# deepspeedai/DeepSpeed

Hardware: AMD Instinct MI355X
Metric: tokens/sec Llama-3-8B ZeRO-3 (higher is better)
Workload: dtype bf16; 1 GPU; model=llama3-8b, global_batch=8, seq_len=4096, parallelism=zero3_dp1, grad_accum=2

## Files before the change

### deepspeed_amd/models/llama.py

```python
from dataclasses import dataclass, field

import torch
import torch.nn as nn
import torch.nn.functional as F

from ..ops.attention import flash_attention
from ..ops.functional import (apply_rope, build_rope_cache,
                              fused_cross_entropy, rms_norm, swiglu)


@dataclass
class LlamaConfig:
    hidden_size: int = 4096
    intermediate_size: int = 14336
    num_hidden_layers: int = 32
    num_attention_heads: int = 32
    num_key_value_heads: int = 8
    vocab_size: int = 128256
    max_position_embeddings: int = 8192
    rope_theta: float = 500000.0
    rms_norm_eps: float = 1e-5
    tie_word_embeddings: bool = False
    initializer_range: float = 0.02
    activation_checkpointing: bool = True
    attention_bias: bool = False

    @property
    def head_dim(self):
        return self.hidden_size // self.num_attention_heads


LLAMA_CONFIGS = {
    "llama3-8b": LlamaConfig(),
    "llama3-70b": LlamaConfig(hidden_size=8192, intermediate_size=28672,
                              num_hidden_layers=80, num_attention_heads=64,
                              num_key_value_heads=8),
    "llama-tiny": LlamaConfig(hidden_size=256, intermediate_size=688,
                              num_hidden_layers=4, num_attention_heads=8,
                              num_key_value_heads=4, vocab_size=2048,
                              max_position_embeddings=512,
                              activation_checkpointing=False),
    "llama-small": LlamaConfig(hidden_size=1024, intermediate_size=2816,
                               num_hidden_layers=8, num_attention_heads=16,
                               num_key_value_heads=4, vocab_size=32000,
                               max_position_embeddings=4096),
    "qwen2-7b": LlamaConfig(hidden_size=3584, intermediate_size=18944,
                            num_hidden_layers=28, num_attention_heads=28,
                            num_key_value_heads=4, vocab_size=152064,
                            max_position_embeddings=32768,
                            rope_theta=1e6, rms_norm_eps=1e-6,
                            attention_bias=True),
    "qwen2-tiny": LlamaConfig(hidden_size=256, intermediate_size=688,
                              num_hidden_layers=4, num_attention_heads=8,
                              num_key_value_heads=4, vocab_size=2048,
                              max_position_embeddings=512,
                              attention_bias=True,
                              tie_word_embeddings=True,
                              activation_checkpointing=False),
}


class LlamaRMSNorm(nn.Module):
    def __init__(self, hidden_size, eps=1e-5):
        super().__init__()
        self.weight = nn.Parameter(torch.ones(hidden_size))
        self.eps = eps

    def forward(self, x):
        return rms_norm(x, self.weight, self.eps)


class LlamaAttention(nn.Module):
    def __init__(self, cfg: LlamaConfig):
        super().__init__()
        self.cfg = cfg
        h, d = cfg.hidden_size, cfg.head_dim
        ab = getattr(cfg, "attention_bias", False)
        self.q_proj = nn.Linear(h, cfg.num_attention_heads * d, bias=ab)
        self.k_proj = nn.Linear(h, cfg.num_key_value_heads * d, bias=ab)
        self.v_proj = nn.Linear(h, cfg.num_key_value_heads * d, bias=ab)
        self.o_proj = nn.Linear(cfg.num_attention_heads * d, h, bias=False)
        self.sp_group = None
        self._dist_attn = None

    def forward(self, x, cos, sin, kv_cache=None):
        B, S, _ = x.shape
        d = self.cfg.head_dim
        q = self.q_proj(x).view(B, S, -1, d)
        k = self.k_proj(x).view(B, S, -1, d)
        v = self.v_proj(x).view(B, S, -1, d)
        if getattr(kv_cache, "fuses_rope", False):
            q, k, v = kv_cache.rope_append(q, k, v)
        else:
            q = apply_rope(q, cos, sin)
            k = apply_rope(k, cos, sin)
            if kv_cache is not None:
                k, v = kv_cache.update(k, v)
        if kv_cache is not None:
            rg = getattr(kv_cache, "ragged", None)
            fb = getattr(kv_cache, "fused", None)
            if getattr(kv_cache, "fp8", False) and (fb is not None
                                                    or rg is not None):
                from ..ops import functional as Fops
                if fb is not None:
                    o = Fops.ragged_prefill_attention_fp8(
                        q[0], kv_cache.k, kv_cache.v, kv_cache.k_scale,
                        kv_cache.v_scale, fb)
                else:
                    o = Fops.ragged_decode_attention_fp8(q, *rg)
            elif fb is not None:
                from ..ops.functional import ragged_prefill_attention
                o = ragged_prefill_attention(q[0], kv_cache.k, kv_cache.v,
                                             fb)
            elif rg is not None:
                from ..ops.loader import get_ext
                o = get_ext(required=True).ragged_decode(
                    q.contiguous(), *rg)
            else:
                mask = getattr(kv_cache, "attn_mask", None)
                causal = S > 1
                o = flash_attention(q, k, v,
                                    causal=causal and mask is None,
                                    attn_mask=mask)
        elif self._dist_attn is not None:
            o = self._dist_attn(q, k, v, causal=True)
        else:
            o = flash_attention(q, k, v, causal=True)
        return self.o_proj(o.reshape(B, S, -1))


class StaticKVCache:

    def __init__(self, batch, max_seq, n_kv, head_dim, dtype, device):
        self.k = torch.zeros(batch, max_seq, n_kv, head_dim, dtype=dtype,
                             device=device)
        self.v = torch.zeros_like(self.k)
        self.max_seq = max_seq

    def prefill(self, k, v):
        S = k.shape[1]
        self.k[:, :S] = k
        self.v[:, :S] = v

    def decode_update(self, k1, v1, pos_idx):
        self.k.index_copy_(1, pos_idx, k1)
        self.v.index_copy_(1, pos_idx, v1)
        return self.k, self.v


def _linear_1t(lin, x):
    if x.is_cuda and x.dtype == torch.bfloat16:
        from ..ops.loader import get_ext
        ext = get_ext(required=False)
        if ext is not None:
            B = x.numel() // x.shape[-1]
            y = ext.gemv_bf16(lin.weight, x.reshape(B, -1).contiguous())
            return y.reshape(*x.shape[:-1], lin.weight.shape[0])
    return lin(x)


def llama_decode_step(model, ids, caches, pos_idx, attn_mask, cos_t, sin_t):
    core = model.model
    x = core.embed_tokens(ids)
    cos = cos_t.index_select(0, pos_idx)
    sin = sin_t.index_select(0, pos_idx)
    for layer, cache in zip(core.layers, caches):
        attn = layer.self_attn
        h = layer.input_layernorm(x)
        B = h.shape[0]
        d = attn.cfg.head_dim
        q = _linear_1t(attn.q_proj, h).view(B, 1, -1, d)
        k = _linear_1t(attn.k_proj, h).view(B, 1, -1, d)
        v = _linear_1t(attn.v_proj, h).view(B, 1, -1, d)
        q = apply_rope(q, cos, sin)
        k = apply_rope(k, cos, sin)
        kf, vf = cache.decode_update(k, v, pos_idx)
        o = F.scaled_dot_product_attention(
            q.transpose(1, 2), kf.transpose(1, 2), vf.transpose(1, 2),
            attn_mask=attn_mask,
            enable_gqa=(kf.shape[2] != q.shape[2]))
        x = x + _linear_1t(attn.o_proj, o.transpose(1, 2).reshape(B, 1, -1))
        h2 = layer.post_attention_layernorm(x)
        mlp = layer.mlp
        x = x + _linear_1t(mlp.down_proj,
                           swiglu(_linear_1t(mlp.gate_proj, h2),
                                  _linear_1t(mlp.up_proj, h2)))
    x = core.norm(x)
    return _linear_1t(model.lm_head, x)


def enable_ulysses(model, sp_group=None):
    from ..sequence.layer import DistributedAttention
    for mod in model.modules():
        if isinstance(mod, LlamaAttention):
            mod.sp_group = sp_group
            mod._dist_attn = DistributedAttention(flash_attention, sp_group)
    return model


class LlamaMLP(nn.Module):
    def __init__(self, cfg: LlamaConfig):
        super().__init__()
        self.gate_proj = nn.Linear(cfg.hidden_size, cfg.intermediate_size,
                                   bias=False)
        self.up_proj = nn.Linear(cfg.hidden_size, cfg.intermediate_size,
                                 bias=False)
        self.down_proj = nn.Linear(cfg.intermediate_size, cfg.hidden_size,
                                   bias=False)

    def forward(self, x):
        return self.down_proj(swiglu(self.gate_proj(x), self.up_proj(x)))


class LlamaDecoderLayer(nn.Module):
    def __init__(self, cfg: LlamaConfig):
        super().__init__()
        self.input_layernorm = LlamaRMSNorm(cfg.hidden_size, cfg.rms_norm_eps)
        self.self_attn = LlamaAttention(cfg)
        self.post_attention_layernorm = LlamaRMSNorm(cfg.hidden_size,
                                                     cfg.rms_norm_eps)
        self.mlp = LlamaMLP(cfg)

    def forward(self, x, cos, sin, kv_cache=None):
        x = x + self.self_attn(self.input_layernorm(x), cos, sin,
                               kv_cache=kv_cache)
        x = x + self.mlp(self.post_attention_layernorm(x))
        return x


class LlamaModel(nn.Module):
    def __init__(self, cfg: LlamaConfig):
        super().__init__()
        self.cfg = cfg
        self.embed_tokens = nn.Embedding(cfg.vocab_size, cfg.hidden_size)
        self.layers = nn.ModuleList(
            [LlamaDecoderLayer(cfg) for _ in range(cfg.num_hidden_layers)])
        self.norm = LlamaRMSNorm(cfg.hidden_size, cfg.rms_norm_eps)
        cos, sin = build_rope_cache(cfg.max_position_embeddings, cfg.head_dim,
                                    cfg.rope_theta)
        dev = self.embed_tokens.weight.device
        if dev.type != "meta":
            cos, sin = cos.to(dev), sin.to(dev)
        self.register_buffer("rope_cos", cos, persistent=False)
        self.register_buffer("rope_sin", sin, persistent=False)

    def forward(self, input_ids, seq_offset=0, kv_caches=None,
                positions=None):
        x = self.embed_tokens(input_ids)
        S = input_ids.shape[1]
        if positions is not None:
            cos = self.rope_cos[positions]
            sin = self.rope_sin[positions]
        else:
            cos = self.rope_cos[seq_offset:seq_offset + S]
            sin = self.rope_sin[seq_offset:seq_offset + S]
        for i, layer in enumerate(self.layers):
            if self.cfg.activation_checkpointing and self.training:
                x = torch.utils.checkpoint.checkpoint(
                    layer, x, cos, sin, use_reentrant=False)
            else:
                x = layer(x, cos, sin,
                          kv_cache=kv_caches[i] if kv_caches else None)
        return self.norm(x)


class LlamaForCausalLM(nn.Module):
    def __init__(self, cfg: LlamaConfig):
        super().__init__()
        self.cfg = cfg
        self.model = LlamaModel(cfg)
        self.lm_head = nn.Linear(cfg.hidden_size, cfg.vocab_size, bias=False)
        if cfg.tie_word_embeddings:
            self.lm_head.weight = self.model.embed_tokens.weight
        self.apply(self._init_weights)

    def _init_weights(self, module):
        std = self.cfg.initializer_range
        if isinstance(module, nn.Linear):
            module.weight.data.normal_(0.0, std)
            if module.bias is not None:
                module.bias.data.zero_()
        elif isinstance(module, nn.Embedding):
            module.weight.data.normal_(0.0, std)

    def forward(self, input_ids, labels=None, seq_offset=0, kv_caches=None,
                positions=None, logits_rows=None):
        h = self.model(input_ids, seq_offset=seq_offset, kv_caches=kv_caches,
                       positions=positions)
        if logits_rows is not None:
            h = h[:, logits_rows]
        logits = self.lm_head(h)
        if labels is None:
            return logits
        return fused_cross_entropy(logits[:, :-1, :], labels[:, 1:])
```

### deepspeed_amd/ops/attention.py

```python
import math
import os

import torch
import torch.nn.functional as F

from .loader import get_ext


class _FlashAttnFn(torch.autograd.Function):
    @staticmethod
    def forward(ctx, q, k, v, causal, scale, kvmask=None):
        ext = get_ext(required=True)
        out, lse = ext.flash_attn_fwd(q, k, v, causal, scale, kvmask)
        ctx.save_for_backward(q, k, v, out, lse,
                              kvmask if kvmask is not None
                              else torch.empty(0))
        ctx.causal = causal
        ctx.scale = scale
        return out

    @staticmethod
    def backward(ctx, dout):
        q, k, v, out, lse, kvmask = ctx.saved_tensors
        if kvmask.numel() == 0:
            kvmask = None
        causal, scale = ctx.causal, ctx.scale
        B, S, Hq, D = q.shape
        Hk = k.shape[2]
        G = Hq // Hk

        if os.environ.get("DSAMD_FLASH_BWD", "1") == "1":
            ext = get_ext(required=True)
            dq, dk, dv = ext.flash_attn_bwd(
                q, k, v, dout.contiguous(), out, lse, causal, scale, kvmask)
            return dq, dk, dv, None, None, None

        qh = q.permute(0, 2, 1, 3)
        kh = k.permute(0, 2, 1, 3)
        vh = v.permute(0, 2, 1, 3)
        doh = dout.permute(0, 2, 1, 3).contiguous()
        oh = out.permute(0, 2, 1, 3)

        drow = (doh.float() * oh.float()).sum(-1)

        qg = qh.reshape(B, Hk, G, S, D)
        dog = doh.reshape(B, Hk, G, S, D)
        lse_g = lse.reshape(B, Hk, G, S)
        drow_g = drow.reshape(B, Hk, G, S)

        dq = torch.zeros(B, Hk, G, S, D, device=q.device, dtype=torch.float32)
        dk = torch.empty_like(kh, dtype=torch.float32)
        dv = torch.empty_like(vh, dtype=torch.float32)

        CHUNK = 1024
        rows = torch.arange(S, device=q.device)
        for c0 in range(0, S, CHUNK):
            c1 = min(c0 + CHUNK, S)
            kc = kh[:, :, c0:c1]
            vc = vh[:, :, c0:c1]
            s_c = torch.einsum("bhgsd,bhcd->bhgsc", qg, kc).float() * scale
            if kvmask is not None:
                s_c = s_c + kvmask[:, c0:c1].view(B, 1, 1, 1, c1 - c0)
            p = torch.exp(s_c - lse_g.unsqueeze(-1))
            if causal:
                mask = rows.view(1, 1, 1, S, 1) >= (c0 + torch.arange(
                    c1 - c0, device=q.device)).view(1, 1, 1, 1, -1)
                p = p * mask
            p16 = p.to(q.dtype)
            dv[:, :, c0:c1] = torch.einsum("bhgsc,bhgsd->bhcd", p16,
                                           dog).float()
            dp = torch.einsum("bhgsd,bhcd->bhgsc", dog, vc).float()
            ds = (p * (dp - drow_g.unsqueeze(-1)) * scale).to(q.dtype)
            dq += torch.einsum("bhgsc,bhcd->bhgsd", ds, kc).float()
            dk[:, :, c0:c1] = torch.einsum("bhgsc,bhgsd->bhcd", ds,
                                           qg).float()

        dq_out = dq.reshape(B, Hq, S, D).permute(0, 2, 1, 3).to(q.dtype)
        dk_out = dk.permute(0, 2, 1, 3).to(k.dtype)
        dv_out = dv.permute(0, 2, 1, 3).to(v.dtype)
        return dq_out.contiguous(), dk_out.contiguous(), \
            dv_out.contiguous(), None, None, None


_USE_HIP_FLASH = os.environ.get("DSAMD_FLASH", "1") == "1"


def _as_kv_padding_mask(attn_mask, B, Sk):
    if attn_mask is None or attn_mask.dtype == torch.bool:
        return None
    m = attn_mask
    if m.dim() == 4 and m.shape[1] == 1 and m.shape[2] == 1:
        m = m[:, 0, 0]
    elif m.dim() == 3 and m.shape[1] == 1:
        m = m[:, 0]
    elif m.dim() != 2:
        return None
    if m.shape[-1] != Sk:
        return None
    if m.shape[0] == 1 and B > 1:
        m = m.expand(B, Sk)
    if m.shape[0] != B:
        return None
    return m.contiguous().float()


def flash_attention(q, k, v, causal=True, attn_mask=None):
    scale = 1.0 / math.sqrt(q.shape[-1])
    hip_ok = _USE_HIP_FLASH and q.is_cuda and q.dtype == torch.bfloat16 \
        and q.shape[-1] in (64, 128) and q.shape[1] == k.shape[1]
    if attn_mask is not None:
        kvm = _as_kv_padding_mask(attn_mask, q.shape[0], k.shape[1]) \
            if hip_ok else None
        if kvm is not None:
            return _FlashAttnFn.apply(q.contiguous(), k.contiguous(),
                                      v.contiguous(), causal, scale, kvm)
        out = F.scaled_dot_product_attention(
            q.transpose(1, 2), k.transpose(1, 2), v.transpose(1, 2),
            attn_mask=attn_mask, is_causal=False,
            enable_gqa=(k.shape[2] != q.shape[2]))
        return out.transpose(1, 2)
    if hip_ok:
        return _FlashAttnFn.apply(q.contiguous(), k.contiguous(),
                                  v.contiguous(), causal, scale)
    qt = q.transpose(1, 2)
    kt = k.transpose(1, 2)
    vt = v.transpose(1, 2)
    out = F.scaled_dot_product_attention(
        qt, kt, vt, is_causal=causal,
        enable_gqa=(k.shape[2] != q.shape[2]))
    return out.transpose(1, 2)
```

### deepspeed_amd/ops/csrc/attention_bwd.hip

```cpp
#include <torch/extension.h>

#include "common.h"

using bf16x8_t = __attribute__((ext_vector_type(8))) short;
using f32x4_t = __attribute__((ext_vector_type(4))) float;
using u32x4_t = __attribute__((ext_vector_type(4))) unsigned int;
using u32x2_t = __attribute__((ext_vector_type(2))) unsigned int;

#define MFMA_BF16_16x16x32 __builtin_amdgcn_mfma_f32_16x16x32_bf16

namespace bwd {

constexpr int BR = 128;
constexpr int WR = 32;
constexpr int KTW1 = 1;
constexpr int TS = 32;
constexpr int PT = 64;

DEV_INLINE unsigned int cvtpk2(float lo, float hi) {
  unsigned short a = __builtin_bit_cast(unsigned short, (__bf16)lo);
  unsigned short b = __builtin_bit_cast(unsigned short, (__bf16)hi);
  return (unsigned int)a | ((unsigned int)b << 16);
}

template <int DH>
__launch_bounds__(256)
__global__ void bwd_preprocess(
    const short* __restrict__ q, const short* __restrict__ k,
    const short* __restrict__ dout, const short* __restrict__ out,
    const float* __restrict__ lse,
    short* __restrict__ qT, short* __restrict__ doT, short* __restrict__ kT,
    float* __restrict__ drowP, float* __restrict__ lseP,
    int B, int S, int Sp, int Hq, int Hk) {
  constexpr int PPR = DH / 8;
  __shared__ unsigned int t[PT][DH / 2 + 1];

  const int z = blockIdx.z;
  const int H = (z == 2) ? Hk : Hq;
  const int bh = blockIdx.y;
  if (bh >= B * H) return;
  const int b = bh / H;
  const int h = bh % H;
  const int s0 = blockIdx.x * PT;
  const short* src = (z == 0) ? q : (z == 1) ? dout : k;
  short* dst = (z == 0) ? qT : (z == 1) ? doT : kT;

  for (int i = threadIdx.x; i < PT * PPR; i += 256) {
    const int row = i / PPR;
    const int c = i % PPR;
    const int s = s0 + row;
    const long long off = (((long long)b * S + s) * H + h) * DH + c * 8;
    u32x4_t x = {0u, 0u, 0u, 0u};
    if (s < S) x = *reinterpret_cast<const u32x4_t*>(src + off);
#pragma unroll
    for (int w = 0; w < 4; ++w) t[row][c * 4 + w] = x[w];
    if (z == 1) {
      u32x4_t o = {0u, 0u, 0u, 0u};
      if (s < S) o = *reinterpret_cast<const u32x4_t*>(out + off);
      float acc = 0.f;
#pragma unroll
      for (int w = 0; w < 4; ++w)
        acc += bf2f((short)(x[w] & 0xffff)) * bf2f((short)(o[w] & 0xffff)) +
               bf2f((short)(x[w] >> 16)) * bf2f((short)(o[w] >> 16));
#pragma unroll
      for (int m = PPR / 2; m > 0; m >>= 1) acc += __shfl_xor(acc, m, WAVE);
      if (c == 0) drowP[((long long)b * Hq + h) * Sp + s] = acc;
    } else if (z == 0 && c == 0) {
      float l = 0.f;
      if (s < S) {
        l = lse[((long long)b * Hq + h) * S + s];
        if (l == -INFINITY) l = INFINITY;
      }
      lseP[((long long)b * Hq + h) * Sp + s] = l;
    }
  }
  __syncthreads();
  for (int i = threadIdx.x; i < DH * (PT / 8); i += 256) {
    const int d = i / (PT / 8);
    const int pc = i % (PT / 8);
    const int sh = (d & 1) * 16;
    unsigned int e[8];
#pragma unroll
    for (int j = 0; j < 8; ++j) e[j] = (t[pc * 8 + j][d >> 1] >> sh) & 0xffffu;
    u32x4_t y = {e[0] | (e[1] << 16), e[2] | (e[3] << 16),
                 e[4] | (e[5] << 16), e[6] | (e[7] << 16)};
    *reinterpret_cast<u32x4_t*>(dst + (((long long)b * H + h) * DH + d) * Sp +
                                s0 + pc * 8) = y;
  }
}

template <int DH>
DEV_INLINE int rmswz(int row, int byte_off) {
  return row * (DH * 2) + (byte_off ^ ((row & 7) << 4));
}

DEV_INLINE void lds_dma16(const short* src, char* lds_wave_base) {
  __builtin_amdgcn_global_load_lds(
      reinterpret_cast<const unsigned int*>(src),
      reinterpret_cast<unsigned int*>(lds_wave_base), 16, 0, 0);
}

template <int DH>
DEV_INLINE void issue_rm(const short* base, long long rs, int r0, int S,
                         char* img, int sseg, int lane) {
  const int linear = sseg * 1024 + lane * 16;
  const int row = linear / (DH * 2);
  const int colbyte = linear % (DH * 2);
  const int src_col = colbyte ^ ((row & 7) << 4);
  const int grow = r0 + row;
  const int srow = grow < S ? grow : S - 1;
  lds_dma16(base + (long long)srow * rs + (src_col >> 1), img + sseg * 1024);
}

template <int DH>
DEV_INLINE void issue_tr(const short* baseT, int Sp, int c0, char* img,
                         int sseg, int lane) {
  const int linear = sseg * 1024 + lane * 16;
  const int d = linear >> 6;
  const int g = ((linear >> 4) & 3) ^ ((d >> 2) & 3);
  lds_dma16(baseT + (long long)d * Sp + c0 + g * 8, img + sseg * 1024);
}

template <int DH>
DEV_INLINE bf16x8_t read_rm(const char* img, int row, int ks, int l4) {
  return *reinterpret_cast<const bf16x8_t*>(
      img + rmswz<DH>(row, (l4 * 8 + 32 * ks) * 2));
}

DEV_INLINE bf16x8_t read_tr(const char* img, int d, int l4) {
  const int sw = (d >> 2) & 3;
  const char* rowp = img + d * 64 + (l4 & 1) * 8;
  u32x2_t lo = *reinterpret_cast<const u32x2_t*>(rowp + (((l4 >> 1) ^ sw) << 4));
  u32x2_t hi =
      *reinterpret_cast<const u32x2_t*>(rowp + (((2 + (l4 >> 1)) ^ sw) << 4));
  u32x4_t w = {lo[0], lo[1], hi[0], hi[1]};
  return __builtin_bit_cast(bf16x8_t, w);
}

DEV_INLINE bf16x8_t pack_pair(const f32x4_t& a, const f32x4_t& b) {
  u32x4_t w = {cvtpk2(a[0], a[1]), cvtpk2(a[2], a[3]), cvtpk2(b[0], b[1]),
               cvtpk2(b[2], b[3])};
  return __builtin_bit_cast(bf16x8_t, w);
}

DEV_INLINE void store4(short* p, const f32x4_t& a) {
  u32x2_t w = {cvtpk2(a[0], a[1]), cvtpk2(a[2], a[3])};
  *reinterpret_cast<u32x2_t*>(p) = w;
}

template <int DH, int KTW>
__launch_bounds__(512 / KTW, 1)
__global__ void flash_bwd_dkv_kernel(
    const short* __restrict__ q,
    const short* __restrict__ k,
    const short* __restrict__ v,
    const short* __restrict__ dout,
    const short* __restrict__ qT,
    const short* __restrict__ doT,
    const float* __restrict__ lseP,
    const float* __restrict__ drowP,
    const float* __restrict__ kvmask,
    short* __restrict__ dk,
    short* __restrict__ dv,
    int B, int S, int Sp, int Hq, int Hk, float scale, int causal) {
  constexpr int NKS = DH / 32;
  constexpr int NDT = DH / 16;
  constexpr int IMG = TS * DH * 2;
  constexpr int SPI = DH / 16;
  constexpr int NW = 8 / KTW;
  constexpr int WRK = 16 * KTW;
  constexpr int LD_OFF = 4 * IMG;
  constexpr int BUF = LD_OFF + 256;
  __shared__ __attribute__((aligned(16))) char smem[2 * BUF];

  const int lane = threadIdx.x & 63;
  const int wave = threadIdx.x >> 6;
  const int l15 = lane & 15;
  const int l4 = lane >> 4;

  const int bh = blockIdx.y;
  const int b = bh / Hk;
  const int hk = bh % Hk;
  const int G = Hq / Hk;
  const int kv_base = blockIdx.x * BR;
  const int wk = kv_base + wave * WRK;

  const long long qrs = (long long)Hq * DH;
  const long long kvrs = (long long)Hk * DH;
  const short* kp = k + ((long long)b * S) * kvrs + hk * DH;
  const short* vp = v + ((long long)b * S) * kvrs + hk * DH;

  bf16x8_t kfrag[KTW][NKS], vfrag[KTW][NKS];
  float maskv[KTW];
#pragma unroll
  for (int kt = 0; kt < KTW; ++kt) {
    const int krow = wk + 16 * kt + l15;
    const int srow = krow < S ? krow : S - 1;
    const short* ks = kp + (long long)srow * kvrs;
    const short* vs = vp + (long long)srow * kvrs;
#pragma unroll
    for (int ks_i = 0; ks_i < NKS; ++ks_i) {
      kfrag[kt][ks_i] =
          *reinterpret_cast<const bf16x8_t*>(ks + ks_i * 32 + l4 * 8);
      vfrag[kt][ks_i] =
          *reinterpret_cast<const bf16x8_t*>(vs + ks_i * 32 + l4 * 8);
    }
    maskv[kt] = (kvmask && krow < S) ? kvmask[(long long)b * S + krow] : 0.f;
  }

  f32x4_t dk_acc[NDT][KTW], dv_acc[NDT][KTW];
#pragma unroll
  for (int dt = 0; dt < NDT; ++dt)
#pragma unroll
    for (int kt = 0; kt < KTW; ++kt) {
      dk_acc[dt][kt] = f32x4_t{0.f, 0.f, 0.f, 0.f};
      dv_acc[dt][kt] = f32x4_t{0.f, 0.f, 0.f, 0.f};
    }

  const int q_start = causal ? kv_base : 0;
  const int nq = (S - q_start + TS - 1) / TS;
  const int total = G * nq;

  auto issue = [&](int g, int qb, int bufi) {
    const int h = hk * G + g;
    char* buf = smem + bufi * BUF;
    const short* qp = q + ((long long)b * S) * qrs + h * DH;
    const short* dop = dout + ((long long)b * S) * qrs + h * DH;
    const long long toff = ((long long)b * Hq + h) * DH * Sp;
    const long long roff = ((long long)b * Hq + h) * Sp;
#pragma unroll
    for (int sseg = wave; sseg < SPI; sseg += NW) {
      issue_rm<DH>(qp, qrs, qb, S, buf, sseg, lane);
      issue_rm<DH>(dop, qrs, qb, S, buf + IMG, sseg, lane);
      issue_tr<DH>(qT + toff, Sp, qb, buf + 2 * IMG, sseg, lane);
      issue_tr<DH>(doT + toff, Sp, qb, buf + 3 * IMG, sseg, lane);
    }
    if (wave == 0) {
      const float* s = (lane < 32 ? lseP : drowP) + roff + qb + (lane & 31);
      __builtin_amdgcn_global_load_lds(
          reinterpret_cast<const unsigned int*>(s),
          reinterpret_cast<unsigned int*>(buf + LD_OFF), 4, 0, 0);
    }
  };

  int g_nx = 0, qb_nx = q_start;
  issue(g_nx, qb_nx, 0);
  for (int it = 0; it < total; ++it) {
    const int qb = qb_nx;
    asm volatile("s_waitcnt vmcnt(0)" ::: "memory");
    __syncthreads();
    qb_nx += TS;
    if (qb_nx >= S) {
      qb_nx = q_start;
      ++g_nx;
    }
    if (it + 1 < total) issue(g_nx, qb_nx, (it + 1) & 1);

    if (wk >= S || (causal && qb + TS - 1 < wk)) continue;
    const bool interior = !kvmask && qb + TS <= S && wk + WRK <= S &&
                          (!causal || qb >= wk + WRK - 1);
    const char* buf = smem + (it & 1) * BUF;
    const float* ld = reinterpret_cast<const float*>(buf + LD_OFF);

    f32x4_t s_acc[2][KTW], dp_acc[2][KTW], lrow[2];
#pragma unroll
    for (int qt = 0; qt < 2; ++qt) {
      lrow[qt] = *reinterpret_cast<const f32x4_t*>(ld + 16 * qt + 4 * l4);
      f32x4_t dr = *reinterpret_cast<const f32x4_t*>(ld + 32 + 16 * qt + 4 * l4);
#pragma unroll
      for (int kt = 0; kt < KTW; ++kt) {
        s_acc[qt][kt] = f32x4_t{0.f, 0.f, 0.f, 0.f};
        dp_acc[qt][kt] = -dr;
      }
    }
    __builtin_amdgcn_s_setprio(1);
#pragma unroll
    for (int qt = 0; qt < 2; ++qt)
#pragma unroll
      for (int ks_i = 0; ks_i < NKS; ++ks_i) {
        bf16x8_t aq = read_rm<DH>(buf, l15 + 16 * qt, ks_i, l4);
        bf16x8_t ad = read_rm<DH>(buf + IMG, l15 + 16 * qt, ks_i, l4);
#pragma unroll
        for (int kt = 0; kt < KTW; ++kt) {
          s_acc[qt][kt] = MFMA_BF16_16x16x32(aq, kfrag[kt][ks_i],
                                             s_acc[qt][kt], 0, 0, 0);
          dp_acc[qt][kt] = MFMA_BF16_16x16x32(ad, vfrag[kt][ks_i],
                                              dp_acc[qt][kt], 0, 0, 0);
        }
      }
    __builtin_amdgcn_s_setprio(0);

    if (interior) {
#pragma unroll
      for (int qt = 0; qt < 2; ++qt)
#pragma unroll
        for (int kt = 0; kt < KTW; ++kt)
#pragma unroll
          for (int r = 0; r < 4; ++r) {
            float p = __expf(s_acc[qt][kt][r] * scale - lrow[qt][r]);
            s_acc[qt][kt][r] = p;
            dp_acc[qt][kt][r] = p * dp_acc[qt][kt][r] * scale;
          }
    } else {
#pragma unroll
      for (int qt = 0; qt < 2; ++qt)
#pragma unroll
        for (int kt = 0; kt < KTW; ++kt) {
          const int gkv = wk + 16 * kt + l15;
#pragma unroll
          for (int r = 0; r < 4; ++r) {
            const int gq = qb + 16 * qt + 4 * l4 + r;
            const bool valid = gq < S && gkv < S && (!causal || gq >= gkv);
            float sval = s_acc[qt][kt][r] * scale + maskv[kt];
            float p = valid ? __expf(sval - lrow[qt][r]) : 0.f;
            s_acc[qt][kt][r] = p;
            dp_acc[qt][kt][r] = p * dp_acc[qt][kt][r] * scale;
          }
        }
    }
    bf16x8_t pb[KTW], dsb[KTW];
#pragma unroll
    for (int kt = 0; kt < KTW; ++kt) {
      pb[kt] = pack_pair(s_acc[0][kt], s_acc[1][kt]);
      dsb[kt] = pack_pair(dp_acc[0][kt], dp_acc[1][kt]);
    }

    __builtin_amdgcn_s_setprio(1);
#pragma unroll
    for (int dt = 0; dt < NDT; ++dt) {
      bf16x8_t aqt = read_tr(buf + 2 * IMG, l15 + 16 * dt, l4);
      bf16x8_t adt = read_tr(buf + 3 * IMG, l15 + 16 * dt, l4);
#pragma unroll
      for (int kt = 0; kt < KTW; ++kt) {
        dv_acc[dt][kt] =
            MFMA_BF16_16x16x32(adt, pb[kt], dv_acc[dt][kt], 0, 0, 0);
        dk_acc[dt][kt] =
            MFMA_BF16_16x16x32(aqt, dsb[kt], dk_acc[dt][kt], 0, 0, 0);
      }
    }
    __builtin_amdgcn_s_setprio(0);
  }

#pragma unroll
  for (int kt = 0; kt < KTW; ++kt) {
    const int gkv = wk + 16 * kt + l15;
    if (gkv >= S) continue;
    short* dkr = dk + ((long long)b * S + gkv) * kvrs + hk * DH + 4 * l4;
    short* dvr = dv + ((long long)b * S + gkv) * kvrs + hk * DH + 4 * l4;
#pragma unroll
    for (int dt = 0; dt < NDT; ++dt) {
      store4(dkr + 16 * dt, dk_acc[dt][kt]);
      store4(dvr + 16 * dt, dv_acc[dt][kt]);
    }
  }
}

template <int DH>
__launch_bounds__(256, 2)
__global__ void flash_bwd_dq_kernel(
    const short* __restrict__ q, const short* __restrict__ k,
    const short* __restrict__ v, const short* __restrict__ dout,
    const short* __restrict__ kT,
    const float* __restrict__ lseP,
    const float* __restrict__ drowP,
    const float* __restrict__ kvmask,
    short* __restrict__ dq,
    int B, int S, int Sp, int Hq, int Hk, float scale, int causal) {
  constexpr int NKS = DH / 32;
  constexpr int NDT = DH / 16;
  constexpr int IMG = TS * DH * 2;
  constexpr int SPI = DH / 16;
  constexpr int IPI = SPI / 4;
  constexpr int BUF = 3 * IMG;
  __shared__ __attribute__((aligned(16))) char smem[2 * BUF];

  const int lane = threadIdx.x & 63;
  const int wave = threadIdx.x >> 6;
  const int l15 = lane & 15;
  const int l4 = lane >> 4;

  const int qtile = gridDim.x - 1 - blockIdx.x;
  const int bh = blockIdx.y;
  const int b = bh / Hq;
  const int h = bh % Hq;
  const int hk = h / (Hq / Hk);
  const int qbase = qtile * BR;
  const int wq = qbase + wave * WR;

  const long long qrs = (long long)Hq * DH;
  const long long kvrs = (long long)Hk * DH;
  const short* qp = q + ((long long)b * S) * qrs + h * DH;
  const short* dop = dout + ((long long)b * S) * qrs + h * DH;
  const short* kp = k + ((long long)b * S) * kvrs + hk * DH;
  const short* vp = v + ((long long)b * S) * kvrs + hk * DH;
  const short* ktp = kT + ((long long)b * Hk + hk) * DH * Sp;
  const float* mp = kvmask ? kvmask + (long long)b * S : nullptr;

  bf16x8_t qfrag[2][NKS], dofrag[2][NKS];
  float lse_l[2], dr_l[2];
#pragma unroll
  for (int qt = 0; qt < 2; ++qt) {
    const int qrow = wq + 16 * qt + l15;
    const int srow = qrow < S ? qrow : S - 1;
    const short* qs = qp + (long long)srow * qrs;
    const short* ds = dop + (long long)srow * qrs;
#pragma unroll
    for (int ks_i = 0; ks_i < NKS; ++ks_i) {
      qfrag[qt][ks_i] =
          *reinterpret_cast<const bf16x8_t*>(qs + ks_i * 32 + l4 * 8);
      dofrag[qt][ks_i] =
          *reinterpret_cast<const bf16x8_t*>(ds + ks_i * 32 + l4 * 8);
    }
    lse_l[qt] = lseP[((long long)b * Hq + h) * Sp + qrow];
    dr_l[qt] = drowP[((long long)b * Hq + h) * Sp + qrow];
  }

  f32x4_t dq_acc[NDT][2];
#pragma unroll
  for (int dt = 0; dt < NDT; ++dt)
#pragma unroll
    for (int qt = 0; qt < 2; ++qt) dq_acc[dt][qt] = f32x4_t{0.f, 0.f, 0.f, 0.f};

  const int kv_end = causal ? min(S, qbase + BR) : S;
  const int n_tiles = (kv_end + TS - 1) / TS;

  auto issue = [&](int kvb, int bufi) {
    char* buf = smem + bufi * BUF;
#pragma unroll
    for (int i = 0; i < IPI; ++i) {
      const int sseg = i * 4 + wave;
      issue_rm<DH>(kp, kvrs, kvb, S, buf, sseg, lane);
      issue_rm<DH>(vp, kvrs, kvb, S, buf + IMG, sseg, lane);
      issue_tr<DH>(ktp, Sp, kvb, buf + 2 * IMG, sseg, lane);
    }
  };

  issue(0, 0);
  for (int t = 0; t < n_tiles; ++t) {
    const int kvb = t * TS;
    asm volatile("s_waitcnt vmcnt(0)" ::: "memory");
    __syncthreads();
    if (t + 1 < n_tiles) issue(kvb + TS, (t + 1) & 1);

    if (wq >= S || (causal && kvb > wq + WR - 1)) continue;
    const bool interior = !mp && kvb + TS <= S && wq + WR <= S &&
                          (!causal || kvb + TS - 1 <= wq);
    const char* buf = smem + (t & 1) * BUF;

    f32x4_t s_acc[2][2], dp_acc[2][2];
#pragma unroll
    for (int kt = 0; kt < 2; ++kt)
#pragma unroll
      for (int qt = 0; qt < 2; ++qt) {
        s_acc[kt][qt] = f32x4_t{0.f, 0.f, 0.f, 0.f};
        dp_acc[kt][qt] =
            f32x4_t{-dr_l[qt], -dr_l[qt], -dr_l[qt], -dr_l[qt]};
      }
    __builtin_amdgcn_s_setprio(1);
#pragma unroll
    for (int kt = 0; kt < 2; ++kt)
#pragma unroll
      for (int ks_i = 0; ks_i < NKS; ++ks_i) {
        bf16x8_t ak = read_rm<DH>(buf, l15 + 16 * kt, ks_i, l4);
        bf16x8_t av = read_rm<DH>(buf + IMG, l15 + 16 * kt, ks_i, l4);
#pragma unroll
        for (int qt = 0; qt < 2; ++qt) {
          s_acc[kt][qt] = MFMA_BF16_16x16x32(ak, qfrag[qt][ks_i],
                                             s_acc[kt][qt], 0, 0, 0);
          dp_acc[kt][qt] = MFMA_BF16_16x16x32(av, dofrag[qt][ks_i],
                                              dp_acc[kt][qt], 0, 0, 0);
        }
      }
    __builtin_amdgcn_s_setprio(0);

    if (interior) {
#pragma unroll
      for (int kt = 0; kt < 2; ++kt)
#pragma unroll
        for (int qt = 0; qt < 2; ++qt)
#pragma unroll
          for (int r = 0; r < 4; ++r) {
            float p = __expf(s_acc[kt][qt][r] * scale - lse_l[qt]);
            dp_acc[kt][qt][r] = p * dp_acc[kt][qt][r] * scale;
          }
    } else {
#pragma unroll
      for (int kt = 0; kt < 2; ++kt)
#pragma unroll
        for (int r = 0; r < 4; ++r) {
          const int gkv = kvb + 16 * kt + 4 * l4 + r;
          const float mv = (mp && gkv < S) ? mp[gkv] : 0.f;
#pragma unroll
          for (int qt = 0; qt < 2; ++qt) {
            const int gq = wq + 16 * qt + l15;
            const bool valid = gq < S && gkv < S && (!causal || gkv <= gq);
            float sval = s_acc[kt][qt][r] * scale + mv;
            float p = valid ? __expf(sval - lse_l[qt]) : 0.f;
            dp_acc[kt][qt][r] = p * dp_acc[kt][qt][r] * scale;
          }
        }
    }
    bf16x8_t dsb[2];
#pragma unroll
    for (int qt = 0; qt < 2; ++qt)
      dsb[qt] = pack_pair(dp_acc[0][qt], dp_acc[1][qt]);

    __builtin_amdgcn_s_setprio(1);
#pragma unroll
    for (int dt = 0; dt < NDT; ++dt) {
      bf16x8_t akt = read_tr(buf + 2 * IMG, l15 + 16 * dt, l4);
#pragma unroll
      for (int qt = 0; qt < 2; ++qt)
        dq_acc[dt][qt] =
            MFMA_BF16_16x16x32(akt, dsb[qt], dq_acc[dt][qt], 0, 0, 0);
    }
    __builtin_amdgcn_s_setprio(0);
  }

#pragma unroll
  for (int qt = 0; qt < 2; ++qt) {
    const int gq = wq + 16 * qt + l15;
    if (gq >= S) continue;
    short* dqr = dq + ((long long)b * S + gq) * qrs + h * DH + 4 * l4;
#pragma unroll
    for (int dt = 0; dt < NDT; ++dt) store4(dqr + 16 * dt, dq_acc[dt][qt]);
  }
}

}

template <int DH>
static void launch_bwd(at::Tensor& q, at::Tensor& k, at::Tensor& v,
                       at::Tensor& dout, at::Tensor& out, at::Tensor& lse,
                       at::Tensor& dq, at::Tensor& dk, at::Tensor& dv,
                       const float* mp, int B, int S, int Hq, int Hk,
                       float scale, int causal) {
  auto stream = c10::hip::getCurrentHIPStream();
  const int Sp = (S + bwd::BR - 1) / bwd::BR * bwd::BR;
  auto qT = at::empty({B, Hq, DH, Sp}, q.options());
  auto doT = at::empty({B, Hq, DH, Sp}, q.options());
  auto kT = at::empty({B, Hk, DH, Sp}, q.options());
  auto drow = at::empty({B, Hq, Sp}, q.options().dtype(at::kFloat));
  auto lseP = at::empty({B, Hq, Sp}, q.options().dtype(at::kFloat));
  auto sp = [](const at::Tensor& t) {
    return reinterpret_cast<const short*>(t.data_ptr());
  };
  auto spm = [](at::Tensor& t) {
    return reinterpret_cast<short*>(t.data_ptr());
  };
  dim3 grid0(Sp / bwd::PT, B * Hq, 3);
  hipLaunchKernelGGL(bwd::bwd_preprocess<DH>, grid0, dim3(256), 0,
                     stream.stream(), sp(q), sp(k), sp(dout), sp(out),
                     lse.data_ptr<float>(), spm(qT), spm(doT), spm(kT),
                     drow.data_ptr<float>(), lseP.data_ptr<float>(), B, S,
                     Sp, Hq, Hk);
  HIP_CHECK_KERNEL();
  dim3 grid1(Sp / bwd::BR, B * Hk);
  hipLaunchKernelGGL((bwd::flash_bwd_dkv_kernel<DH, bwd::KTW1>), grid1,
                     dim3(512 / bwd::KTW1), 0, stream.stream(), sp(q), sp(k),
                     sp(v), sp(dout), sp(qT), sp(doT), lseP.data_ptr<float>(),
                     drow.data_ptr<float>(), mp, spm(dk), spm(dv), B, S, Sp,
                     Hq, Hk, scale, causal);
  HIP_CHECK_KERNEL();
  dim3 grid2(Sp / bwd::BR, B * Hq);
  hipLaunchKernelGGL(bwd::flash_bwd_dq_kernel<DH>, grid2, dim3(256), 0,
                     stream.stream(), sp(q), sp(k), sp(v), sp(dout), sp(kT),
                     lseP.data_ptr<float>(), drow.data_ptr<float>(), mp,
                     spm(dq), B, S, Sp, Hq, Hk, scale, causal);
  HIP_CHECK_KERNEL();
}

void flash_check_qkv(const at::Tensor& q, const at::Tensor& k,
                     const at::Tensor& v, const char* who);
const float* flash_check_kvmask(const c10::optional<at::Tensor>& kvmask,
                                const at::Tensor& q);

std::vector<at::Tensor> flash_attn_bwd(at::Tensor q, at::Tensor k,
                                       at::Tensor v, at::Tensor dout,
                                       at::Tensor out, at::Tensor lse,
                                       bool causal, double scale,
                                       c10::optional<at::Tensor> kvmask) {
  flash_check_qkv(q, k, v, "flash_attn_bwd");
  CHECK_ARG(dout, at::kBFloat16);
  CHECK_ARG(out, at::kBFloat16);
  CHECK_ARG(lse, at::kFloat);
  CHECK_ON(dout, q);
  CHECK_ON(out, q);
  CHECK_ON(lse, q);
  TORCH_CHECK(dout.sizes() == q.sizes() && out.sizes() == q.sizes(),
              "flash_attn_bwd: dout and out must have q's shape");
  int B = q.size(0), S = q.size(1), Hq = q.size(2), D = q.size(3);
  int Hk = k.size(2);
  TORCH_CHECK(lse.dim() == 3 && lse.size(0) == B && lse.size(1) == Hq &&
                  lse.size(2) == S,
              "flash_attn_bwd: lse must be [B,Hq,S]");
  const float* mp = flash_check_kvmask(kvmask, q);
  const float fscale =
      scale == 0.0 ? 1.0f / std::sqrt((float)D) : (float)scale;
  auto dq = at::empty_like(q);
  auto dk = at::empty_like(k);
  auto dv = at::empty_like(v);
  if (D == 128)
    launch_bwd<128>(q, k, v, dout, out, lse, dq, dk, dv, mp, B, S, Hq, Hk,
                    fscale, causal ? 1 : 0);
  else
    launch_bwd<64>(q, k, v, dout, out, lse, dq, dk, dv, mp, B, S, Hq, Hk,
                   fscale, causal ? 1 : 0);
  return {dq, dk, dv};
}
```

### deepspeed_amd/ops/csrc/bindings.cpp

```cpp
#include <torch/extension.h>

void multi_tensor_adam(std::vector<at::Tensor> params,
                       std::vector<at::Tensor> grads,
                       std::vector<at::Tensor> exp_avgs,
                       std::vector<at::Tensor> exp_avg_sqs, double lr,
                       double beta1, double beta2, double eps, long step,
                       long adamw_mode, long bias_correction,
                       double weight_decay, std::vector<at::Tensor> out16,
                       double grad_scale);
void accum_bf16_to_f32(at::Tensor dst, at::Tensor src, double scale);
at::Tensor l2norm_sq(std::vector<at::Tensor> tensors);
at::Tensor fp8_amax(at::Tensor x);
at::Tensor ragged_decode(at::Tensor q, at::Tensor kpool, at::Tensor vpool,
                         at::Tensor rows, at::Tensor lens, long chunk);
at::Tensor ragged_prefill(at::Tensor q, at::Tensor kpool, at::Tensor vpool,
                          at::Tensor desc, long max_qlen, long max_kvlen);
at::Tensor ragged_rope_append(at::Tensor q, at::Tensor k, at::Tensor v,
                              at::Tensor cos, at::Tensor sin,
                              at::Tensor tok_slot, at::Tensor tok_pos,
                              at::Tensor kpool, at::Tensor vpool,
                              c10::optional<at::Tensor> lens);
at::Tensor ragged_decode_fp8(at::Tensor q, at::Tensor kpool, at::Tensor vpool,
                             at::Tensor k_scale, at::Tensor v_scale,
                             at::Tensor rows, at::Tensor lens, long chunk);
at::Tensor ragged_prefill_fp8(at::Tensor q, at::Tensor kpool,
                              at::Tensor vpool, at::Tensor k_scale,
                              at::Tensor v_scale, at::Tensor desc,
                              long max_qlen, long max_kvlen);
at::Tensor ragged_rope_append_fp8(at::Tensor q, at::Tensor k, at::Tensor v,
                                  at::Tensor cos, at::Tensor sin,
                                  at::Tensor tok_slot, at::Tensor tok_pos,
                                  at::Tensor kpool, at::Tensor vpool,
                                  at::Tensor k_scale, at::Tensor v_scale,
                                  c10::optional<at::Tensor> lens);
at::Tensor fp8_cast(at::Tensor x, at::Tensor scale, bool e5m2);
std::vector<at::Tensor> fp8_cast_transpose(at::Tensor x, at::Tensor scale,
                                           bool e5m2);
std::vector<at::Tensor> flash_attn_fwd(at::Tensor q, at::Tensor k,
                                       at::Tensor v, bool causal,
                                       double scale,
                                       c10::optional<at::Tensor> kvmask);
std::vector<at::Tensor> flash_attn_bwd(at::Tensor q, at::Tensor k,
                                       at::Tensor v, at::Tensor dout,
                                       at::Tensor out, at::Tensor lse,
                                       bool causal, double scale,
                                       c10::optional<at::Tensor> kvmask);
void multi_tensor_adagrad(std::vector<at::Tensor> params,
                          std::vector<at::Tensor> grads,
                          std::vector<at::Tensor> sq_accums, double lr,
                          double eps, double weight_decay,
                          std::vector<at::Tensor> out16);
void multi_tensor_lamb(std::vector<at::Tensor> params,
                       std::vector<at::Tensor> grads,
                       std::vector<at::Tensor> updates,
                       std::vector<at::Tensor> exp_avgs,
                       std::vector<at::Tensor> exp_avg_sqs,
                       at::Tensor workspace, double lr, double beta1,
                       double beta2, double eps, long step,
                       long bias_correction, double weight_decay,
                       std::vector<at::Tensor> out16, double grad_scale);
void cpu_lion_step(at::Tensor p, at::Tensor g, at::Tensor m,
                   c10::optional<at::Tensor> out16, double lr, double beta1,
                   double beta2, double wd);
void cpu_adagrad_step(at::Tensor p, at::Tensor g, at::Tensor h,
                      c10::optional<at::Tensor> out16, double lr, double eps,
                      double wd);
void cpu_adam_step(at::Tensor p, at::Tensor g, at::Tensor m, at::Tensor v,
                   c10::optional<at::Tensor> out16, double lr, double beta1,
                   double beta2, double eps, long step, long adamw,
                   long bias_correction, double wd, double grad_scale);
void multi_tensor_lion(std::vector<at::Tensor> params,
                       std::vector<at::Tensor> grads,
                       std::vector<at::Tensor> exp_avgs, double lr,
                       double beta1, double beta2, double weight_decay,
                       std::vector<at::Tensor> out16);
std::vector<at::Tensor> rmsnorm_fwd(at::Tensor x, at::Tensor w, double eps);
std::vector<at::Tensor> rmsnorm_bwd(at::Tensor dy, at::Tensor x, at::Tensor w,
                                    at::Tensor rstd);
std::vector<at::Tensor> layernorm_fwd(at::Tensor x, at::Tensor w,
                                      c10::optional<at::Tensor> b, double eps);
std::vector<at::Tensor> layernorm_bwd(at::Tensor dy, at::Tensor x,
                                      at::Tensor w, at::Tensor mean,
                                      at::Tensor rstd);
void rope(at::Tensor dst, at::Tensor src, at::Tensor cos, at::Tensor sin,
          long pos0, bool backward);
void rope_inplace(at::Tensor t, at::Tensor cos, at::Tensor sin, long pos0,
                  bool backward);
at::Tensor swiglu_fwd(at::Tensor g, at::Tensor u);
std::vector<at::Tensor> swiglu_bwd(at::Tensor dy, at::Tensor g, at::Tensor u);
std::vector<at::Tensor> cross_entropy_fwd(at::Tensor logits,
                                          at::Tensor targets,
                                          long ignore_index);
at::Tensor cross_entropy_bwd(at::Tensor logits, at::Tensor targets,
                             at::Tensor lse, at::Tensor dloss,
                             long ignore_index);

void bind_aio(py::module_& m);
at::Tensor gemv_bf16(at::Tensor W, at::Tensor x);
at::Tensor spatial_bias_add(at::Tensor a, at::Tensor bias,
                            c10::optional<at::Tensor> other);
std::vector<at::Tensor> quantize_int8(at::Tensor x, long group_size);
at::Tensor dequantize_int8(at::Tensor q, at::Tensor scales, long group_size);
std::vector<at::Tensor> quantize_fp8(at::Tensor x, long group_size);
at::Tensor dequantize_fp8(at::Tensor q, at::Tensor scales, long group_size);
std::vector<at::Tensor> quantize_int4(at::Tensor x, long group);
at::Tensor dequantize_int4(at::Tensor q, at::Tensor scales, long group,
                           long numel);
std::vector<at::Tensor> quantize_fp_em(at::Tensor x, long qbits, long group);
at::Tensor dequantize_fp_em(at::Tensor q, at::Tensor scales, long qbits,
                            long group, std::vector<long> shape);

PYBIND11_MODULE(TORCH_EXTENSION_NAME, m) {
  bind_aio(m);
  m.def("multi_tensor_adam", &multi_tensor_adam, "fused AdamW (gfx950)",
        py::arg("params"), py::arg("grads"), py::arg("exp_avgs"),
        py::arg("exp_avg_sqs"), py::arg("lr"), py::arg("beta1"),
        py::arg("beta2"), py::arg("eps"), py::arg("step"),
        py::arg("adamw_mode"), py::arg("bias_correction"),
        py::arg("weight_decay"), py::arg("out16") = std::vector<at::Tensor>(),
        py::arg("grad_scale") = 1.0);
  m.def("accum_bf16_to_f32", &accum_bf16_to_f32, py::arg("dst"),
        py::arg("src"), py::arg("scale") = 1.0);
  m.def("l2norm_sq", &l2norm_sq);
  m.def("fp8_amax", &fp8_amax);
  m.def("ragged_decode", &ragged_decode, py::arg("q"), py::arg("kpool"),
        py::arg("vpool"), py::arg("rows"), py::arg("lens"),
        py::arg("chunk") = 512);
  m.def("ragged_prefill", &ragged_prefill, py::arg("q"), py::arg("kpool"),
        py::arg("vpool"), py::arg("desc"), py::arg("max_qlen"),
        py::arg("max_kvlen"));
  m.def("ragged_rope_append", &ragged_rope_append, py::arg("q"),
        py::arg("k"), py::arg("v"), py::arg("cos"), py::arg("sin"),
        py::arg("tok_slot"), py::arg("tok_pos"), py::arg("kpool"),
        py::arg("vpool"), py::arg("lens") = c10::nullopt);
  m.def("ragged_decode_fp8", &ragged_decode_fp8, py::arg("q"),
        py::arg("kpool"), py::arg("vpool"), py::arg("k_scale"),
        py::arg("v_scale"), py::arg("rows"), py::arg("lens"),
        py::arg("chunk") = 512);
  m.def("ragged_prefill_fp8", &ragged_prefill_fp8, py::arg("q"),
        py::arg("kpool"), py::arg("vpool"), py::arg("k_scale"),
        py::arg("v_scale"), py::arg("desc"), py::arg("max_qlen"),
        py::arg("max_kvlen"));
  m.def("ragged_rope_append_fp8", &ragged_rope_append_fp8, py::arg("q"),
        py::arg("k"), py::arg("v"), py::arg("cos"), py::arg("sin"),
        py::arg("tok_slot"), py::arg("tok_pos"), py::arg("kpool"),
        py::arg("vpool"), py::arg("k_scale"), py::arg("v_scale"),
        py::arg("lens") = c10::nullopt);
  m.def("fp8_cast", &fp8_cast, py::arg("x"), py::arg("scale"),
        py::arg("e5m2") = false);
  m.def("fp8_cast_transpose", &fp8_cast_transpose, py::arg("x"),
        py::arg("scale"), py::arg("e5m2") = false);
  m.def("gemv_bf16", &gemv_bf16);
  m.def("spatial_bias_add", &spatial_bias_add, py::arg("a"), py::arg("bias"),
        py::arg("other") = c10::nullopt);
  m.def("quantize_int8", &quantize_int8);
  m.def("dequantize_int8", &dequantize_int8);
  m.def("quantize_fp8", &quantize_fp8);
  m.def("dequantize_fp8", &dequantize_fp8);
  m.def("quantize_int4", &quantize_int4, py::arg("x"),
        py::arg("group") = 2048);
  m.def("dequantize_int4", &dequantize_int4, py::arg("q"),
        py::arg("scales"), py::arg("group"), py::arg("numel"));
  m.def("quantize_fp_em", &quantize_fp_em, py::arg("x"), py::arg("qbits"),
        py::arg("group") = 512);
  m.def("dequantize_fp_em", &dequantize_fp_em, py::arg("q"),
        py::arg("scales"), py::arg("qbits"), py::arg("group"),
        py::arg("shape"));
  m.def("flash_attn_fwd", &flash_attn_fwd, py::arg("q"), py::arg("k"),
        py::arg("v"), py::arg("causal") = true, py::arg("scale") = 0.0,
        py::arg("kvmask") = c10::nullopt);
  m.def("flash_attn_bwd", &flash_attn_bwd, py::arg("q"), py::arg("k"),
        py::arg("v"), py::arg("dout"), py::arg("out"), py::arg("lse"),
        py::arg("causal") = true, py::arg("scale") = 0.0,
        py::arg("kvmask") = c10::nullopt);
  m.def("multi_tensor_adagrad", &multi_tensor_adagrad, py::arg("params"),
        py::arg("grads"), py::arg("sq_accums"), py::arg("lr"),
        py::arg("eps") = 1e-8, py::arg("weight_decay") = 0.0,
        py::arg("out16") = std::vector<at::Tensor>{});
  m.def("multi_tensor_lamb", &multi_tensor_lamb, py::arg("params"),
        py::arg("grads"), py::arg("updates"), py::arg("exp_avgs"),
        py::arg("exp_avg_sqs"),
        py::arg("workspace"), py::arg("lr"), py::arg("beta1") = 0.9,
        py::arg("beta2") = 0.999, py::arg("eps") = 1e-6, py::arg("step") = 1,
        py::arg("bias_correction") = 1, py::arg("weight_decay") = 0.0,
        py::arg("out16") = std::vector<at::Tensor>{},
        py::arg("grad_scale") = 1.0);
  m.def("cpu_lion_step", &cpu_lion_step, py::arg("p"), py::arg("g"),
        py::arg("m"), py::arg("out16") = c10::nullopt, py::arg("lr") = 1e-4,
        py::arg("beta1") = 0.9, py::arg("beta2") = 0.99, py::arg("wd") = 0.0,
        py::call_guard<py::gil_scoped_release>());
  m.def("cpu_adagrad_step", &cpu_adagrad_step, py::arg("p"), py::arg("g"),
        py::arg("h"), py::arg("out16") = c10::nullopt, py::arg("lr") = 1e-2,
        py::arg("eps") = 1e-8, py::arg("wd") = 0.0,
        py::call_guard<py::gil_scoped_release>());
  m.def("cpu_adam_step", &cpu_adam_step, py::arg("p"), py::arg("g"),
        py::arg("m"), py::arg("v"), py::arg("out16") = c10::nullopt,
        py::arg("lr") = 1e-3, py::arg("beta1") = 0.9, py::arg("beta2") = 0.999,
        py::arg("eps") = 1e-8, py::arg("step") = 1, py::arg("adamw") = 1,
        py::arg("bias_correction") = 1, py::arg("wd") = 0.0,
        py::arg("grad_scale") = 1.0);
  m.def("multi_tensor_lion", &multi_tensor_lion, "fused Lion (gfx950)",
        py::arg("params"), py::arg("grads"), py::arg("exp_avgs"),
        py::arg("lr"), py::arg("beta1"), py::arg("beta2"),
        py::arg("weight_decay"), py::arg("out16") = std::vector<at::Tensor>());
  m.def("rmsnorm_fwd", &rmsnorm_fwd);
  m.def("rmsnorm_bwd", &rmsnorm_bwd);
  m.def("layernorm_fwd", &layernorm_fwd);
  m.def("layernorm_bwd", &layernorm_bwd);
  m.def("rope", &rope);
  m.def("rope_inplace", &rope_inplace);
  m.def("swiglu_fwd", &swiglu_fwd);
  m.def("swiglu_bwd", &swiglu_bwd);
  m.def("cross_entropy_fwd", &cross_entropy_fwd);
  m.def("cross_entropy_bwd", &cross_entropy_bwd);
}
```

### deepspeed_amd/ops/csrc/elementwise.hip

```cpp
#include <torch/extension.h>

#include "common.h"

__global__ void rope_kernel(short* __restrict__ dst,
                            const short* __restrict__ src,
                            const float* __restrict__ cs,
                            const float* __restrict__ sn,
                            long long total_vec, int S, int H, int D,
                            int pos0, int backward) {
  int half = D / 2;
  int half8 = half / 8;
  long long i0 = (long long)blockIdx.x * blockDim.x + threadIdx.x;
  long long stride = (long long)gridDim.x * blockDim.x;
  for (long long i = i0; i < total_vec; i += stride) {
    int d8 = (int)(i % half8);
    long long rem = i / half8;
    int h = (int)(rem % H);
    long long rem2 = rem / H;
    int s = (int)(rem2 % S);
    long long b = rem2 / S;
    long long base = ((b * S + s) * (long long)H + h) * D + d8 * 8;
    const float* crow = cs + (long long)(s + pos0) * half + d8 * 8;
    const float* srow = sn + (long long)(s + pos0) * half + d8 * 8;
    bf16x8 x1 = *reinterpret_cast<const bf16x8*>(src + base);
    bf16x8 x2 = *reinterpret_cast<const bf16x8*>(src + base + half);
    f32x4 c0 = *reinterpret_cast<const f32x4*>(crow);
    f32x4 c1 = *reinterpret_cast<const f32x4*>(crow + 4);
    f32x4 s0 = *reinterpret_cast<const f32x4*>(srow);
    f32x4 s1 = *reinterpret_cast<const f32x4*>(srow + 4);
    float sgn = backward ? -1.f : 1.f;
    bf16x8 o1, o2;
#pragma unroll
    for (int k = 0; k < 8; ++k) {
      float c = (k < 4 ? c0.v[k] : c1.v[k - 4]);
      float sv = (k < 4 ? s0.v[k] : s1.v[k - 4]) * sgn;
      float a = bf2f(x1.v[k]);
      float bb = bf2f(x2.v[k]);
      o1.v[k] = f2bf(a * c - bb * sv);
      o2.v[k] = f2bf(bb * c + a * sv);
    }
    *reinterpret_cast<bf16x8*>(dst + base) = o1;
    *reinterpret_cast<bf16x8*>(dst + base + half) = o2;
  }
}

__global__ void rope_kernel_scalar(short* __restrict__ dst,
                                   const short* __restrict__ src,
                                   const float* __restrict__ cs,
                                   const float* __restrict__ sn,
                                   long long total_pairs, int S, int H,
                                   int D, int pos0, int backward) {
  int half = D / 2;
  long long i0 = (long long)blockIdx.x * blockDim.x + threadIdx.x;
  long long stride = (long long)gridDim.x * blockDim.x;
  for (long long i = i0; i < total_pairs; i += stride) {
    int d = (int)(i % half);
    long long rem = i / half;
    int h = (int)(rem % H);
    long long rem2 = rem / H;
    int s = (int)(rem2 % S);
    long long b = rem2 / S;
    long long base = ((b * S + s) * (long long)H + h) * D;
    float c = cs[(long long)(s + pos0) * half + d];
    float sv = sn[(long long)(s + pos0) * half + d];
    if (backward) sv = -sv;
    float x1 = bf2f(src[base + d]);
    float x2 = bf2f(src[base + d + half]);
    dst[base + d] = f2bf(x1 * c - x2 * sv);
    dst[base + d + half] = f2bf(x2 * c + x1 * sv);
  }
}

void rope(at::Tensor dst, at::Tensor src, at::Tensor cos, at::Tensor sin,
          long pos0, bool backward) {
  CHECK_ARG(src, at::kBFloat16);
  CHECK_ARG(dst, at::kBFloat16);
  CHECK_LIKE(dst, src);
  TORCH_CHECK(src.dim() == 4, "rope expects [B,S,H,D]");
  int B = src.size(0), S = src.size(1), H = src.size(2), D = src.size(3);
  TORCH_CHECK(D % 2 == 0, "rope: D must be even");
  if (src.numel() == 0) return;
  TORCH_CHECK(cos.device() == src.device() && sin.device() == src.device() &&
                  dst.device() == src.device(),
              "rope: cos/sin/dst must be on the same device as src");
  TORCH_CHECK(cos.scalar_type() == at::kFloat && cos.is_contiguous() &&
                  sin.scalar_type() == at::kFloat && sin.is_contiguous(),
              "rope: cos/sin must be contiguous fp32");
  TORCH_CHECK(pos0 >= 0, "rope: pos0 must be >= 0");
  TORCH_CHECK((long long)(pos0 + S) * (D / 2) <= cos.numel() &&
                  (long long)(pos0 + S) * (D / 2) <= sin.numel(),
              "rope: cos/sin table shorter than [pos0 + S, D/2]");
  auto stream = c10::hip::getCurrentHIPStream();
  int block = 256;
  bool vec = (D / 2) % 8 == 0 && ptr_aligned(src.data_ptr(), 16) &&
             ptr_aligned(dst.data_ptr(), 16) &&
             ptr_aligned(cos.data_ptr(), 16) &&
             ptr_aligned(sin.data_ptr(), 16);
  if (vec) {
    long long total_vec = (long long)B * S * H * (D / 16);
    int grid = grid_for(total_vec, block);
    hipLaunchKernelGGL(rope_kernel, dim3(grid), dim3(block), 0,
                       stream.stream(),
                       reinterpret_cast<short*>(dst.data_ptr()),
                       reinterpret_cast<const short*>(src.data_ptr()),
                       cos.data_ptr<float>(), sin.data_ptr<float>(),
                       total_vec, S, H, D, (int)pos0, backward ? 1 : 0);
  } else {
    long long total_pairs = (long long)B * S * H * (D / 2);
    int grid = grid_for(total_pairs, block);
    hipLaunchKernelGGL(rope_kernel_scalar, dim3(grid), dim3(block), 0,
                       stream.stream(),
                       reinterpret_cast<short*>(dst.data_ptr()),
                       reinterpret_cast<const short*>(src.data_ptr()),
                       cos.data_ptr<float>(), sin.data_ptr<float>(),
                       total_pairs, S, H, D, (int)pos0, backward ? 1 : 0);
  }
  HIP_CHECK_KERNEL();
}

void rope_inplace(at::Tensor t, at::Tensor cos, at::Tensor sin, long pos0,
                  bool backward) {
  rope(t, t, cos, sin, pos0, backward);
}

__global__ void swiglu_fwd_kernel(const short* __restrict__ g,
                                  const short* __restrict__ u,
                                  short* __restrict__ y, long long n,
                                  int vec_ok) {
  long long i0 = (long long)blockIdx.x * blockDim.x + threadIdx.x;
  long long stride = (long long)gridDim.x * blockDim.x;
  long long n8 = vec_ok ? n / 8 : 0;
  for (long long i = i0; i < n8; i += stride) {
    bf16x8 gv = reinterpret_cast<const bf16x8*>(g)[i];
    bf16x8 uv = reinterpret_cast<const bf16x8*>(u)[i];
    bf16x8 o;
#pragma unroll
    for (int k = 0; k < 8; ++k) {
      float gf = bf2f(gv.v[k]);
      float s = gf / (1.f + __expf(-gf));
      o.v[k] = f2bf(s * bf2f(uv.v[k]));
    }
    reinterpret_cast<bf16x8*>(y)[i] = o;
  }
  for (long long i = n8 * 8 + i0; i < n; i += stride) {
    float gf = bf2f(g[i]);
    float s = gf / (1.f + __expf(-gf));
    y[i] = f2bf(s * bf2f(u[i]));
  }
}

__global__ void swiglu_bwd_kernel(const short* __restrict__ dy,
                                  const short* __restrict__ g,
                                  const short* __restrict__ u,
                                  short* __restrict__ dg,
                                  short* __restrict__ du, long long n,
                                  int vec_ok) {
  long long i0 = (long long)blockIdx.x * blockDim.x + threadIdx.x;
  long long stride = (long long)gridDim.x * blockDim.x;
  long long n8 = vec_ok ? n / 8 : 0;
  for (long long i = i0; i < n8; i += stride) {
    bf16x8 dv = reinterpret_cast<const bf16x8*>(dy)[i];
    bf16x8 gv = reinterpret_cast<const bf16x8*>(g)[i];
    bf16x8 uv = reinterpret_cast<const bf16x8*>(u)[i];
    bf16x8 og, ou;
#pragma unroll
    for (int k = 0; k < 8; ++k) {
      float gf = bf2f(gv.v[k]);
      float d = bf2f(dv.v[k]);
      float sig = 1.f / (1.f + __expf(-gf));
      float silu = gf * sig;
      og.v[k] = f2bf(d * bf2f(uv.v[k]) * (sig + silu * (1.f - sig)));
      ou.v[k] = f2bf(d * silu);
    }
    reinterpret_cast<bf16x8*>(dg)[i] = og;
    reinterpret_cast<bf16x8*>(du)[i] = ou;
  }
  for (long long i = n8 * 8 + i0; i < n; i += stride) {
    float gf = bf2f(g[i]);
    float d = bf2f(dy[i]);
    float sig = 1.f / (1.f + __expf(-gf));
    float silu = gf * sig;
    dg[i] = f2bf(d * bf2f(u[i]) * (sig + silu * (1.f - sig)));
    du[i] = f2bf(d * silu);
  }
}

at::Tensor swiglu_fwd(at::Tensor g, at::Tensor u) {
  CHECK_ARG(g, at::kBFloat16);
  CHECK_ARG(u, at::kBFloat16);
  CHECK_LIKE(u, g);
  auto y = at::empty_like(g);
  long long n = g.numel();
  if (n == 0) return y;
  int vec_ok = ptr_aligned(g.data_ptr(), 16) && ptr_aligned(u.data_ptr(), 16) &&
               ptr_aligned(y.data_ptr(), 16);
  auto stream = c10::hip::getCurrentHIPStream();
  int block = 256;
  int grid = grid_for(vec_ok ? n / 8 + 1 : n, block);
  hipLaunchKernelGGL(swiglu_fwd_kernel, dim3(grid), dim3(block), 0,
                     stream.stream(),
                     reinterpret_cast<const short*>(g.data_ptr()),
                     reinterpret_cast<const short*>(u.data_ptr()),
                     reinterpret_cast<short*>(y.data_ptr()), n, vec_ok);
  HIP_CHECK_KERNEL();
  return y;
}

std::vector<at::Tensor> swiglu_bwd(at::Tensor dy, at::Tensor g, at::Tensor u) {
  CHECK_ARG(g, at::kBFloat16);
  CHECK_ARG(u, at::kBFloat16);
  CHECK_ARG(dy, at::kBFloat16);
  CHECK_LIKE(u, g);
  CHECK_LIKE(dy, g);
  auto dg = at::empty_like(g);
  auto du = at::empty_like(u);
  long long n = g.numel();
  if (n == 0) return {dg, du};
  int vec_ok = ptr_aligned(dy.data_ptr(), 16) &&
               ptr_aligned(g.data_ptr(), 16) &&
               ptr_aligned(u.data_ptr(), 16) &&
               ptr_aligned(dg.data_ptr(), 16) &&
               ptr_aligned(du.data_ptr(), 16);
  auto stream = c10::hip::getCurrentHIPStream();
  int block = 256;
  int grid = grid_for(vec_ok ? n / 8 + 1 : n, block);
  hipLaunchKernelGGL(swiglu_bwd_kernel, dim3(grid), dim3(block), 0,
                     stream.stream(),
                     reinterpret_cast<const short*>(dy.data_ptr()),
                     reinterpret_cast<const short*>(g.data_ptr()),
                     reinterpret_cast<const short*>(u.data_ptr()),
                     reinterpret_cast<short*>(dg.data_ptr()),
                     reinterpret_cast<short*>(du.data_ptr()), n, vec_ok);
  HIP_CHECK_KERNEL();
  return {dg, du};
}
```

### deepspeed_amd/ops/csrc/misc.hip

```cpp
#include <torch/extension.h>

#include "common.h"

__global__ void accum_bf16_f32_kernel(float* __restrict__ dst,
                                      const short* __restrict__ src,
                                      long long n, float scale,
                                      int vec_ok) {
  long long i0 = (long long)blockIdx.x * blockDim.x + threadIdx.x;
  long long stride = (long long)gridDim.x * blockDim.x;
  long long n4 = vec_ok ? n / 4 : 0;
  for (long long i = i0; i < n4; i += stride) {
    uint2 sv = reinterpret_cast<const uint2*>(src)[i];
    const short* s = reinterpret_cast<const short*>(&sv);
    f32x4 d = reinterpret_cast<f32x4*>(dst)[i];
#pragma unroll
    for (int k = 0; k < 4; ++k) d.v[k] += bf2f(s[k]) * scale;
    reinterpret_cast<f32x4*>(dst)[i] = d;
  }
  for (long long i = n4 * 4 + i0; i < n; i += stride)
    dst[i] += bf2f(src[i]) * scale;
}

void accum_bf16_to_f32(at::Tensor dst, at::Tensor src, double scale) {
  CHECK_ARG(dst, at::kFloat);
  CHECK_ARG(src, at::kBFloat16);
  CHECK_LIKE(src, dst);
  long long n = dst.numel();
  if (n == 0) return;
  int vec_ok = ptr_aligned(dst.data_ptr(), 16) && ptr_aligned(src.data_ptr(), 8);
  auto stream = c10::hip::getCurrentHIPStream();
  int block = 256;
  int grid = grid_for(n / 4 + 1, block);
  hipLaunchKernelGGL(accum_bf16_f32_kernel, dim3(grid), dim3(block), 0,
                     stream.stream(), dst.data_ptr<float>(),
                     reinterpret_cast<const short*>(src.data_ptr()), n,
                     (float)scale, vec_ok);
  HIP_CHECK_KERNEL();
}

template <int BLOCK>
__global__ void l2norm_sq_kernel(const float* __restrict__ x, long long n,
                                 float* __restrict__ out ,
                                 int vec_ok) {
  __shared__ float lds[BLOCK / WAVE];
  long long i0 = (long long)blockIdx.x * blockDim.x + threadIdx.x;
  long long stride = (long long)gridDim.x * blockDim.x;
  float acc = 0.f;
  long long n4 = vec_ok ? n / 4 : 0;
  for (long long i = i0; i < n4; i += stride) {
    f32x4 v = reinterpret_cast<const f32x4*>(x)[i];
#pragma unroll
    for (int k = 0; k < 4; ++k) acc += v.v[k] * v.v[k];
  }
  for (long long i = n4 * 4 + i0; i < n; i += stride) acc += x[i] * x[i];
  acc = block_reduce_sum<BLOCK>(acc, lds);
  if (threadIdx.x == 0) atomicAdd(out, acc);
}

at::Tensor l2norm_sq(std::vector<at::Tensor> tensors) {
  TORCH_CHECK(!tensors.empty());
  for (auto& t : tensors) {
    CHECK_ARG(t, at::kFloat);
    CHECK_ON(t, tensors[0]);
  }
  auto out = at::zeros({1}, tensors[0].options().dtype(at::kFloat));
  auto stream = c10::hip::getCurrentHIPStream();
  constexpr int BLOCK = 256;
  for (auto& t : tensors) {
    long long n = t.numel();
    if (n == 0) continue;
    int vec_ok = ptr_aligned(t.data_ptr(), 16);
    int grid = grid_for(n / 4 + 1, BLOCK);
    hipLaunchKernelGGL(l2norm_sq_kernel<BLOCK>, dim3(grid), dim3(BLOCK), 0,
                       stream.stream(), t.data_ptr<float>(), n,
                       out.data_ptr<float>(), vec_ok);
    HIP_CHECK_KERNEL();
  }
  return out;
}
```

### deepspeed_amd/ops/csrc/norms.hip

```cpp
#include <torch/extension.h>

#include "common.h"

static inline int row_vec_ok(int H, std::initializer_list<const void*> ptrs) {
  if (H % 8 != 0) return 0;
  for (const void* p : ptrs)
    if (!ptr_aligned(p, 16)) return 0;
  return 1;
}

static inline void check_norm_args(const at::Tensor& x, const at::Tensor& w) {
  CHECK_ARG(x, at::kBFloat16);
  CHECK_ARG(w, at::kBFloat16);
  CHECK_ON(w, x);
  TORCH_CHECK(x.dim() >= 1 && x.size(-1) > 0 && w.numel() == x.size(-1),
              "weight must have x.size(-1) elements");
}

template <int BLOCK>
__global__ void rmsnorm_fwd_kernel(const short* __restrict__ x,
                                   const short* __restrict__ w,
                                   short* __restrict__ y,
                                   float* __restrict__ rstd_out, int H,
                                   float eps, int vec) {
  __shared__ float lds[BLOCK / WAVE];
  const long long row = blockIdx.x;
  const short* xr = x + row * (long long)H;
  short* yr = y + row * (long long)H;
  int H8 = vec ? H / 8 : 0;
  float ss = 0.f;
  for (int i = threadIdx.x; i < H8; i += BLOCK) {
    bf16x8 v = reinterpret_cast<const bf16x8*>(xr)[i];
#pragma unroll
    for (int k = 0; k < 8; ++k) {
      float f = bf2f(v.v[k]);
      ss += f * f;
    }
  }
  for (int i = H8 * 8 + threadIdx.x; i < H; i += BLOCK) {
    float f = bf2f(xr[i]);
    ss += f * f;
  }
  ss = block_reduce_sum<BLOCK>(ss, lds);
  float rstd = rsqrtf(ss / H + eps);
  if (threadIdx.x == 0 && rstd_out) rstd_out[row] = rstd;
  for (int i = threadIdx.x; i < H8; i += BLOCK) {
    bf16x8 v = reinterpret_cast<const bf16x8*>(xr)[i];
    bf16x8 wv = reinterpret_cast<const bf16x8*>(w)[i];
    bf16x8 o;
#pragma unroll
    for (int k = 0; k < 8; ++k)
      o.v[k] = f2bf(bf2f(v.v[k]) * rstd * bf2f(wv.v[k]));
    reinterpret_cast<bf16x8*>(yr)[i] = o;
  }
  for (int i = H8 * 8 + threadIdx.x; i < H; i += BLOCK)
    yr[i] = f2bf(bf2f(xr[i]) * rstd * bf2f(w[i]));
}

template <int BLOCK>
__global__ void rmsnorm_bwd_dx_kernel(const short* __restrict__ dy,
                                      const short* __restrict__ x,
                                      const short* __restrict__ w,
                                      const float* __restrict__ rstd,
                                      short* __restrict__ dx, int H,
                                      int vec) {
  __shared__ float lds[BLOCK / WAVE];
  const long long row = blockIdx.x;
  const short* dyr = dy + row * (long long)H;
  const short* xr = x + row * (long long)H;
  short* dxr = dx + row * (long long)H;
  float rs = rstd[row];
  int H8 = vec ? H / 8 : 0;
  float dot = 0.f;
  for (int i = threadIdx.x; i < H8; i += BLOCK) {
    bf16x8 dv = reinterpret_cast<const bf16x8*>(dyr)[i];
    bf16x8 xv = reinterpret_cast<const bf16x8*>(xr)[i];
    bf16x8 wv = reinterpret_cast<const bf16x8*>(w)[i];
#pragma unroll
    for (int k = 0; k < 8; ++k)
      dot += bf2f(dv.v[k]) * bf2f(wv.v[k]) * bf2f(xv.v[k]);
  }
  for (int i = H8 * 8 + threadIdx.x; i < H; i += BLOCK)
    dot += bf2f(dyr[i]) * bf2f(w[i]) * bf2f(xr[i]);
  dot = block_reduce_sum<BLOCK>(dot, lds);
  float c = dot * rs * rs / H;
  for (int i = threadIdx.x; i < H8; i += BLOCK) {
    bf16x8 dv = reinterpret_cast<const bf16x8*>(dyr)[i];
    bf16x8 xv = reinterpret_cast<const bf16x8*>(xr)[i];
    bf16x8 wv = reinterpret_cast<const bf16x8*>(w)[i];
    bf16x8 o;
#pragma unroll
    for (int k = 0; k < 8; ++k)
      o.v[k] = f2bf(rs * (bf2f(dv.v[k]) * bf2f(wv.v[k]) -
                          bf2f(xv.v[k]) * c));
    reinterpret_cast<bf16x8*>(dxr)[i] = o;
  }
  for (int i = H8 * 8 + threadIdx.x; i < H; i += BLOCK)
    dxr[i] = f2bf(rs * (bf2f(dyr[i]) * bf2f(w[i]) - bf2f(xr[i]) * c));
}

__global__ void rmsnorm_bwd_dw_kernel(const short* __restrict__ dy,
                                      const short* __restrict__ x,
                                      const float* __restrict__ rstd,
                                      float* __restrict__ dw, long long rows,
                                      int H) {
  int c = blockIdx.x * blockDim.x + threadIdx.x;
  if (c >= H) return;
  float acc = 0.f;
  for (long long r = blockIdx.y; r < rows; r += gridDim.y) {
    long long idx = r * H + c;
    acc += bf2f(dy[idx]) * bf2f(x[idx]) * rstd[r];
  }
  if (gridDim.y == 1)
    dw[c] = acc;
  else
    atomicAdd(dw + c, acc);
}

std::vector<at::Tensor> rmsnorm_fwd(at::Tensor x, at::Tensor w, double eps) {
  check_norm_args(x, w);
  int H = x.size(-1);
  long long rows = x.numel() / H;
  auto y = at::empty_like(x);
  auto rstd = at::empty({rows}, x.options().dtype(at::kFloat));
  if (rows == 0) return {y, rstd};
  auto stream = c10::hip::getCurrentHIPStream();
  constexpr int BLOCK = 256;
  int vec = row_vec_ok(H, {x.data_ptr(), w.data_ptr(), y.data_ptr()});
  hipLaunchKernelGGL(rmsnorm_fwd_kernel<BLOCK>, dim3(rows), dim3(BLOCK), 0,
                     stream.stream(),
                     reinterpret_cast<const short*>(x.data_ptr()),
                     reinterpret_cast<const short*>(w.data_ptr()),
                     reinterpret_cast<short*>(y.data_ptr()),
                     rstd.data_ptr<float>(), H, (float)eps, vec);
  HIP_CHECK_KERNEL();
  return {y, rstd};
}

std::vector<at::Tensor> rmsnorm_bwd(at::Tensor dy, at::Tensor x, at::Tensor w,
                                    at::Tensor rstd) {
  check_norm_args(x, w);
  CHECK_ARG(dy, at::kBFloat16);
  CHECK_LIKE(dy, x);
  CHECK_ARG(rstd, at::kFloat);
  CHECK_ON(rstd, x);
  int H = x.size(-1);
  long long rows = x.numel() / H;
  TORCH_CHECK(rstd.numel() == rows, "rstd must have one entry per row");
  auto dx = at::empty_like(x);
  auto dw = at::zeros({H}, x.options().dtype(at::kFloat));
  if (rows == 0) return {dx, dw};
  auto stream = c10::hip::getCurrentHIPStream();
  constexpr int BLOCK = 256;
  int vec = row_vec_ok(
      H, {dy.data_ptr(), x.data_ptr(), w.data_ptr(), dx.data_ptr()});
  hipLaunchKernelGGL(rmsnorm_bwd_dx_kernel<BLOCK>, dim3(rows), dim3(BLOCK), 0,
                     stream.stream(),
                     reinterpret_cast<const short*>(dy.data_ptr()),
                     reinterpret_cast<const short*>(x.data_ptr()),
                     reinterpret_cast<const short*>(w.data_ptr()),
                     rstd.data_ptr<float>(),
                     reinterpret_cast<short*>(dx.data_ptr()), H, vec);
  HIP_CHECK_KERNEL();
  int gy = rows > 4096 ? 64 : (rows > 512 ? 16 : 1);
  hipLaunchKernelGGL(rmsnorm_bwd_dw_kernel, dim3((H + 255) / 256, gy),
                     dim3(256), 0, stream.stream(),
                     reinterpret_cast<const short*>(dy.data_ptr()),
                     reinterpret_cast<const short*>(x.data_ptr()),
                     rstd.data_ptr<float>(), dw.data_ptr<float>(), rows, H);
  HIP_CHECK_KERNEL();
  return {dx, dw};
}

template <int BLOCK>
__global__ void layernorm_fwd_kernel(const short* __restrict__ x,
                                     const short* __restrict__ w,
                                     const short* __restrict__ b,
                                     short* __restrict__ y,
                                     float* __restrict__ mean_out,
                                     float* __restrict__ rstd_out, int H,
                                     float eps) {
  __shared__ float lds[BLOCK / WAVE];
  const long long row = blockIdx.x;
  const short* xr = x + row * (long long)H;
  short* yr = y + row * (long long)H;
  float s = 0.f;
  for (int i = threadIdx.x; i < H; i += BLOCK) s += bf2f(xr[i]);
  s = block_reduce_sum<BLOCK>(s, lds);
  float mean = s / H;
  float ss = 0.f;
  for (int i = threadIdx.x; i < H; i += BLOCK) {
    float d = bf2f(xr[i]) - mean;
    ss += d * d;
  }
  ss = block_reduce_sum<BLOCK>(ss, lds);
  float var = ss / H;
  float rstd = rsqrtf(var + eps);
  if (threadIdx.x == 0) {
    if (mean_out) mean_out[row] = mean;
    if (rstd_out) rstd_out[row] = rstd;
  }
  for (int i = threadIdx.x; i < H; i += BLOCK) {
    float xhat = (bf2f(xr[i]) - mean) * rstd;
    float o = xhat * bf2f(w[i]) + (b ? bf2f(b[i]) : 0.f);
    yr[i] = f2bf(o);
  }
}

template <int BLOCK>
__global__ void layernorm_bwd_dx_kernel(
    const short* __restrict__ dy, const short* __restrict__ x,
    const short* __restrict__ w, const float* __restrict__ mean,
    const float* __restrict__ rstd, short* __restrict__ dx, int H) {
  __shared__ float lds[BLOCK / WAVE];
  const long long row = blockIdx.x;
  const short* dyr = dy + row * (long long)H;
  const short* xr = x + row * (long long)H;
  short* dxr = dx + row * (long long)H;
  float mu = mean[row], rs = rstd[row];
  float c1 = 0.f, c2 = 0.f;
  for (int i = threadIdx.x; i < H; i += BLOCK) {
    float g = bf2f(dyr[i]) * bf2f(w[i]);
    float xhat = (bf2f(xr[i]) - mu) * rs;
    c1 += g;
    c2 += g * xhat;
  }
  c1 = block_reduce_sum<BLOCK>(c1, lds) / H;
  c2 = block_reduce_sum<BLOCK>(c2, lds) / H;
  for (int i = threadIdx.x; i < H; i += BLOCK) {
    float g = bf2f(dyr[i]) * bf2f(w[i]);
    float xhat = (bf2f(xr[i]) - mu) * rs;
    dxr[i] = f2bf((g - c1 - xhat * c2) * rs);
  }
}

__global__ void layernorm_bwd_dwdb_kernel(const short* __restrict__ dy,
                                          const short* __restrict__ x,
                                          const float* __restrict__ mean,
                                          const float* __restrict__ rstd,
                                          float* __restrict__ dw,
                                          float* __restrict__ db,
                                          long long rows, int H) {
  int c = blockIdx.x * blockDim.x + threadIdx.x;
  if (c >= H) return;
  float accw = 0.f, accb = 0.f;
  for (long long r = blockIdx.y; r < rows; r += gridDim.y) {
    long long idx = r * H + c;
    float d = bf2f(dy[idx]);
    accw += d * (bf2f(x[idx]) - mean[r]) * rstd[r];
    accb += d;
  }
  if (gridDim.y == 1) {
    dw[c] = accw;
    db[c] = accb;
  } else {
    atomicAdd(dw + c, accw);
    atomicAdd(db + c, accb);
  }
}

std::vector<at::Tensor> layernorm_fwd(at::Tensor x, at::Tensor w,
                                      c10::optional<at::Tensor> b,
                                      double eps) {
  check_norm_args(x, w);
  if (b.has_value()) {
    CHECK_ARG(*b, at::kBFloat16);
    CHECK_LIKE(*b, w);
  }
  int H = x.size(-1);
  long long rows = x.numel() / H;
  auto y = at::empty_like(x);
  auto mean = at::empty({rows}, x.options().dtype(at::kFloat));
  auto rstd = at::empty({rows}, x.options().dtype(at::kFloat));
  if (rows == 0) return {y, mean, rstd};
  auto stream = c10::hip::getCurrentHIPStream();
  constexpr int BLOCK = 256;
  hipLaunchKernelGGL(
      layernorm_fwd_kernel<BLOCK>, dim3(rows), dim3(BLOCK), 0,
      stream.stream(), reinterpret_cast<const short*>(x.data_ptr()),
      reinterpret_cast<const short*>(w.data_ptr()),
      b.has_value() ? reinterpret_cast<const short*>(b->data_ptr()) : nullptr,
      reinterpret_cast<short*>(y.data_ptr()), mean.data_ptr<float>(),
      rstd.data_ptr<float>(), H, (float)eps);
  HIP_CHECK_KERNEL();
  return {y, mean, rstd};
}

std::vector<at::Tensor> layernorm_bwd(at::Tensor dy, at::Tensor x,
                                      at::Tensor w, at::Tensor mean,
                                      at::Tensor rstd) {
  check_norm_args(x, w);
  CHECK_ARG(dy, at::kBFloat16);
  CHECK_LIKE(dy, x);
  CHECK_ARG(mean, at::kFloat);
  CHECK_ARG(rstd, at::kFloat);
  CHECK_ON(mean, x);
  CHECK_ON(rstd, x);
  int H = x.size(-1);
  long long rows = x.numel() / H;
  TORCH_CHECK(mean.numel() == rows && rstd.numel() == rows,
              "mean/rstd must have one entry per row");
  auto dx = at::empty_like(x);
  auto dw = at::zeros({H}, x.options().dtype(at::kFloat));
  auto db = at::zeros({H}, x.options().dtype(at::kFloat));
  if (rows == 0) return {dx, dw, db};
  auto stream = c10::hip::getCurrentHIPStream();
  constexpr int BLOCK = 256;
  hipLaunchKernelGGL(layernorm_bwd_dx_kernel<BLOCK>, dim3(rows), dim3(BLOCK),
                     0, stream.stream(),
                     reinterpret_cast<const short*>(dy.data_ptr()),
                     reinterpret_cast<const short*>(x.data_ptr()),
                     reinterpret_cast<const short*>(w.data_ptr()),
                     mean.data_ptr<float>(), rstd.data_ptr<float>(),
                     reinterpret_cast<short*>(dx.data_ptr()), H);
  HIP_CHECK_KERNEL();
  int gy = rows > 4096 ? 64 : (rows > 512 ? 16 : 1);
  hipLaunchKernelGGL(layernorm_bwd_dwdb_kernel, dim3((H + 255) / 256, gy),
                     dim3(256), 0, stream.stream(),
                     reinterpret_cast<const short*>(dy.data_ptr()),
                     reinterpret_cast<const short*>(x.data_ptr()),
                     mean.data_ptr<float>(), rstd.data_ptr<float>(),
                     dw.data_ptr<float>(), db.data_ptr<float>(), rows, H);
  HIP_CHECK_KERNEL();
  return {dx, dw, db};
}
```

### deepspeed_amd/runtime/zenflow.py

```python
from typing import Optional

import threading

import torch
from pydantic import BaseModel

from .. import comm as dist
from ..utils.logging import log_dist
from .zero.stage_1_and_2 import ZeroStage12Optimizer
from .zero.stage3 import ZeroStage3Optimizer


class ZenFlowConfig(BaseModel):
    topk_ratio: float = 0.01
    update_interval: int = 4
    select_interval: int = 16
    select_strategy: str = "auto"
    full_warm_up_rounds: int = 0
    overlap_step: bool = False


class ZenFlowZeroOptimizer(ZeroStage12Optimizer):
    def __init__(self, init_optimizer, zenflow_config: Optional[dict] = None,
                 **kw):
        super().__init__(init_optimizer, **kw)
        zf = zenflow_config or {}
        self.zf = zf if isinstance(zf, ZenFlowConfig) else ZenFlowConfig(**zf)
        self._zf_step = 0
        pin = torch.cuda.is_available()
        self._zf = []
        for b in self.buckets:
            cpu = b.master32.detach().to("cpu")
            st = dict(master_cpu=cpu.pin_memory() if pin else cpu,
                      acc_steps=0, hot_idx=None, hot_master=None,
                      hot_m=None, hot_v=None)
            st["m_cpu"] = torch.zeros_like(st["master_cpu"])
            st["v_cpu"] = torch.zeros_like(st["master_cpu"])
            st["acc_cpu"] = torch.zeros_like(st["master_cpu"])
            st["acc_snap"] = torch.zeros_like(st["master_cpu"]) \
                if self.zf.overlap_step else None
            st["thread"] = None
            self._zf.append(st)
            b.master32 = None
        for group in self.optimizer.param_groups:
            group["params"] = []
        log_dist(f"ZenFlow: topk={self.zf.topk_ratio}, "
                 f"update_interval={self.zf.update_interval}", ranks=[0])

    def _writeback_hot(self, st):
        if st["hot_idx"] is None:
            return
        idx = st["hot_idx"].cpu()
        st["master_cpu"][idx] = st["hot_master"].cpu()
        st["m_cpu"][idx] = st["hot_m"].cpu()
        st["v_cpu"][idx] = st["hot_v"].cpu()

    def _select_hot(self, st, g):
        k = max(1, int(self.zf.topk_ratio * g.numel()))
        self._writeback_hot(st)
        st["hot_idx"] = g.abs().topk(k).indices
        idx_cpu = st["hot_idx"].cpu()
        dev = g.device
        st["hot_master"] = st["master_cpu"][idx_cpu].to(dev,
                                                        non_blocking=True)
        st["hot_m"] = st["m_cpu"][idx_cpu].to(dev, non_blocking=True)
        st["hot_v"] = st["v_cpu"][idx_cpu].to(dev, non_blocking=True)

    @torch.no_grad()
    def step(self, closure=None):
        assert closure is None, "closure not supported"
        self._sync_comm()
        if self.dtype == torch.float16:
            self.overflow = self.has_overflow()
            self.loss_scaler.update_scale(self.overflow)
            if self.overflow:
                log_dist("ZenFlow: OVERFLOW, skipping step", ranks=[0])
                self._clear_grads()
                return
        self._zf_step += 1
        combined = self._combined_scale()
        group = self.optimizer.param_groups[0]
        lr = group["lr"]
        beta1, beta2 = group.get("betas", (0.9, 0.999))
        eps = group.get("eps", 1e-8)
        wd = group.get("weight_decay", 0.0)
        t = self._zf_step
        bc1 = 1 - beta1 ** t
        bc2 = 1 - beta2 ** t

        lazy = (self._zf_step % self.zf.update_interval) == 0
        for b, st in zip(self.buckets, self._zf):
            if st["thread"] is not None and not st["thread"].is_alive():
                self._publish_cpu_step(b, st)
            g = b.grad32
            if combined != 1.0:
                g.mul_(1.0 / combined)
            if st["hot_idx"] is None or \
                    (self._zf_step % self.zf.select_interval) == 1:
                self._select_hot(st, g)
            idx = st["hot_idx"]
            gh = g[idx]
            st["hot_m"].mul_(beta1).add_(gh, alpha=1 - beta1)
            st["hot_v"].mul_(beta2).addcmul_(gh, gh, value=1 - beta2)
            if wd:
                st["hot_master"].mul_(1 - lr * wd)
            denom = (st["hot_v"] / bc2).sqrt().add_(eps)
            st["hot_master"].addcdiv_(st["hot_m"] / bc1, denom, value=-lr)
            flat_shard = b.shard16.view(-1)
            flat_shard[idx] = st["hot_master"].to(b.shard16.dtype)
            g.index_fill_(0, idx, 0.0)
            st["acc_cpu"].add_(g.to("cpu"))
            st["acc_steps"] += 1
            if lazy:
                if st["thread"] is not None:
                    st["thread"].join()
                    self._publish_cpu_step(b, st)
                self._writeback_hot(st)
                idx_cpu = st["hot_idx"].cpu()
                hot_restore = (idx_cpu, st["master_cpu"][idx_cpu].clone(),
                               st["m_cpu"][idx_cpu].clone(),
                               st["v_cpu"][idx_cpu].clone())
                st["acc_cpu"].div_(max(st["acc_steps"], 1))
                if self.zf.overlap_step:
                    st["acc_cpu"], st["acc_snap"] = (st["acc_snap"],
                                                     st["acc_cpu"])
                    args = (st["master_cpu"], st["acc_snap"], st["m_cpu"],
                            st["v_cpu"], lr, beta1, beta2, eps, t, wd,
                            bc1, bc2) + hot_restore
                    st["thread"] = threading.Thread(
                        target=self._host_adam, args=args, daemon=True)
                    st["thread"].start()
                else:
                    self._host_adam(st["master_cpu"], st["acc_cpu"],
                                    st["m_cpu"], st["v_cpu"], lr, beta1,
                                    beta2, eps, t, wd, bc1, bc2,
                                    *hot_restore)
                    st["acc_cpu"].zero_()
                    self._publish_cpu_step(b, st)
                st["acc_steps"] = 0

        for b in self.buckets:
            dist.all_gather_into_tensor(
                b.flat16, b.shard16,
                group=b.pg if b.pg is not None else self.dp_group)
        self._clear_grads()

    @staticmethod
    def _host_adam(master, grad, m, v, lr, beta1, beta2, eps, t, wd,
                   bc1, bc2, hot_idx=None, hot_master=None, hot_m=None,
                   hot_v=None):
        from ..ops.loader import has_ext, get_ext
        if has_ext():
            get_ext().cpu_adam_step(master, grad, m, v, None, lr, beta1,
                                    beta2, eps, t, 1, 1, wd, 1.0)
        else:
            m.mul_(beta1).add_(grad, alpha=1 - beta1)
            v.mul_(beta2).addcmul_(grad, grad, value=1 - beta2)
            master.mul_(1 - lr * wd)
            master.addcdiv_(m / bc1, (v / bc2).sqrt().add_(eps), value=-lr)
        if hot_idx is not None:
            master[hot_idx] = hot_master
            m[hot_idx] = hot_m
            v[hot_idx] = hot_v

    def _publish_cpu_step(self, b, st):
        st["thread"] = None
        if st["acc_snap"] is not None:
            st["acc_snap"].zero_()
        b.shard16.copy_(
            st["master_cpu"].to(b.shard16.device, non_blocking=True)
            .to(b.shard16.dtype))
        if st["hot_idx"] is not None:
            idx_cpu = st["hot_idx"].cpu()
            dev = b.shard16.device
            st["hot_master"] = st["master_cpu"][idx_cpu].to(dev)
            st["hot_m"] = st["m_cpu"][idx_cpu].to(dev)
            st["hot_v"] = st["v_cpu"][idx_cpu].to(dev)

    def _drain_threads(self):
        for b, st in zip(self.buckets, self._zf):
            if st["thread"] is not None:
                st["thread"].join()
                self._publish_cpu_step(b, st)

    def state_dict(self):
        self._drain_threads()
        return {
            "zf_step": self._zf_step,
            "single_partition_of_fp32_groups":
                [st["master_cpu"] for st in self._zf],
            "m": [st["m_cpu"] for st in self._zf],
            "v": [st["v_cpu"] for st in self._zf],
            "loss_scaler": self.loss_scaler.state_dict()
            if hasattr(self.loss_scaler, "state_dict") else None,
        }

    def load_state_dict(self, sd):
        self._zf_step = sd.get("zf_step", 0)
        for b, st, mc, m, v in zip(self.buckets, self._zf,
                                   sd["single_partition_of_fp32_groups"],
                                   sd["m"], sd["v"]):
            st["master_cpu"].copy_(mc)
            st["m_cpu"].copy_(m)
            st["v_cpu"].copy_(v)
            st["hot_idx"] = None
            b.shard16.copy_(st["master_cpu"].to(b.shard16.device)
                            .to(b.shard16.dtype))
        for b in self.buckets:
            dist.all_gather_into_tensor(
                b.flat16, b.shard16,
                group=b.pg if b.pg is not None else self.dp_group)


class ZenFlowZeroStage3Optimizer(ZeroStage3Optimizer):

    def __init__(self, init_optimizer, zenflow_config=None, **kw):
        super().__init__(init_optimizer, **kw)
        assert self.param_swapper is None, \
            "ZenFlow manages its own host state; combine it with " \
            "offload_param cpu, not the NVMe parameter tier"
        zf = zenflow_config or {}
        self.zf = zf if isinstance(zf, ZenFlowConfig) else ZenFlowConfig(**zf)
        self._zf_step = 0
        pin = torch.cuda.is_available()
        self._zf = []
        for sg in self.sub_groups:
            cpu = sg.master32.detach().to("cpu")
            st = dict(master_cpu=cpu.pin_memory() if pin else cpu,
                      acc_steps=0, hot_idx=None, hot_master=None,
                      hot_m=None, hot_v=None, thread=None)
            st["m_cpu"] = torch.zeros_like(st["master_cpu"])
            st["v_cpu"] = torch.zeros_like(st["master_cpu"])
            st["acc_cpu"] = torch.zeros_like(st["master_cpu"])
            st["acc_snap"] = torch.zeros_like(st["master_cpu"]) \
                if self.zf.overlap_step else None
            self._zf.append(st)
            sg.master32 = st["master_cpu"]
        for group in self.optimizer.param_groups:
            group["params"] = []
        log_dist(f"ZenFlow(stage3): topk={self.zf.topk_ratio}, "
                 f"update_interval={self.zf.update_interval}", ranks=[0])

    @torch.no_grad()
    def step(self, closure=None):
        assert closure is None
        self._flush_ipg()
        self._sync_comm_streams()
        self._drain_inflight()
        self._cached_norm_sq = None
        if self.dtype == torch.float16:
            self.overflow = self.has_overflow()
            self.loss_scaler.update_scale(self.overflow)
            if self.overflow:
                log_dist("ZenFlow(stage3): OVERFLOW, skipping step",
                         ranks=[0])
                self._clear_grads()
                return
        self._zf_step += 1
        combined = self._combined_scale()
        group = self.optimizer.param_groups[0]
        lr = group["lr"]
        beta1, beta2 = group.get("betas", (0.9, 0.999))
        eps = group.get("eps", 1e-8)
        wd = group.get("weight_decay", 0.0)
        t = self._zf_step
        bc1 = 1 - beta1 ** t
        bc2 = 1 - beta2 ** t
        lazy = (self._zf_step % self.zf.update_interval) == 0

        for sg, st in zip(self.sub_groups, self._zf):
            if st["thread"] is not None and not st["thread"].is_alive():
                self._publish_sg(sg, st)
            g = sg.grad32
            if combined != 1.0:
                g.mul_(1.0 / combined)
            if st["hot_idx"] is None or \
                    (self._zf_step % self.zf.select_interval) == 1:
                self._select_hot_sg(sg, st, g)
            idx = st["hot_idx"]
            gh = g[idx]
            st["hot_m"].mul_(beta1).add_(gh, alpha=1 - beta1)
            st["hot_v"].mul_(beta2).addcmul_(gh, gh, value=1 - beta2)
            if wd:
                st["hot_master"].mul_(1 - lr * wd)
            denom = (st["hot_v"] / bc2).sqrt().add_(eps)
            st["hot_master"].addcdiv_(st["hot_m"] / bc1, denom, value=-lr)
            sg.flat16.view(-1)[idx] = st["hot_master"].to(sg.flat16.dtype)
            g.index_fill_(0, idx, 0.0)
            st["acc_cpu"].add_(g.to("cpu"))
            st["acc_steps"] += 1
            if lazy:
                if st["thread"] is not None:
                    st["thread"].join()
                    self._publish_sg(sg, st)
                self._writeback_hot_sg(st)
                idx_cpu = st["hot_idx"].cpu()
                hot_restore = (idx_cpu, st["master_cpu"][idx_cpu].clone(),
                               st["m_cpu"][idx_cpu].clone(),
                               st["v_cpu"][idx_cpu].clone())
                st["acc_cpu"].div_(max(st["acc_steps"], 1))
                if self.zf.overlap_step:
                    st["acc_cpu"], st["acc_snap"] = (st["acc_snap"],
                                                     st["acc_cpu"])
                    args = (st["master_cpu"], st["acc_snap"], st["m_cpu"],
                            st["v_cpu"], lr, beta1, beta2, eps, t, wd,
                            bc1, bc2) + hot_restore
                    st["thread"] = threading.Thread(
                        target=ZenFlowZeroOptimizer._host_adam, args=args,
                        daemon=True)
                    st["thread"].start()
                else:
                    ZenFlowZeroOptimizer._host_adam(
                        st["master_cpu"], st["acc_cpu"], st["m_cpu"],
                        st["v_cpu"], lr, beta1, beta2, eps, t, wd, bc1,
                        bc2, *hot_restore)
                    st["acc_cpu"].zero_()
                    self._publish_sg(sg, st)
                st["acc_steps"] = 0
        self._clear_grads()
        self._refresh_persistent_params()

    def _writeback_hot_sg(self, st):
        if st["hot_idx"] is None:
            return
        idx = st["hot_idx"].cpu()
        st["master_cpu"][idx] = st["hot_master"].cpu()
        st["m_cpu"][idx] = st["hot_m"].cpu()
        st["v_cpu"][idx] = st["hot_v"].cpu()

    def _select_hot_sg(self, sg, st, g):
        k = max(1, int(self.zf.topk_ratio * g.numel()))
        self._writeback_hot_sg(st)
        st["hot_idx"] = g.abs().topk(k).indices
        idx_cpu = st["hot_idx"].cpu()
        dev = g.device
        st["hot_master"] = st["master_cpu"][idx_cpu].to(dev,
                                                        non_blocking=True)
        st["hot_m"] = st["m_cpu"][idx_cpu].to(dev, non_blocking=True)
        st["hot_v"] = st["v_cpu"][idx_cpu].to(dev, non_blocking=True)

    def _publish_sg(self, sg, st):
        st["thread"] = None
        if st["acc_snap"] is not None:
            st["acc_snap"].zero_()
        sg.flat16.copy_(
            st["master_cpu"].to(sg.flat16.device, non_blocking=True)
            .to(sg.flat16.dtype))
        if st["hot_idx"] is not None:
            idx_cpu = st["hot_idx"].cpu()
            dev = sg.flat16.device
            st["hot_master"] = st["master_cpu"][idx_cpu].to(dev)
            st["hot_m"] = st["m_cpu"][idx_cpu].to(dev)
            st["hot_v"] = st["v_cpu"][idx_cpu].to(dev)

    def _drain_threads(self):
        for sg, st in zip(self.sub_groups, self._zf):
            if st["thread"] is not None:
                st["thread"].join()
                self._publish_sg(sg, st)

    def state_dict(self):
        self._drain_threads()
        sd = super().state_dict()
        sd["zf_step"] = self._zf_step
        sd["zf_m"] = [st["m_cpu"] for st in self._zf]
        sd["zf_v"] = [st["v_cpu"] for st in self._zf]
        return sd

    def load_state_dict(self, sd, load_optimizer_states=True):
        super().load_state_dict(sd, load_optimizer_states)
        self._zf_step = sd.get("zf_step", 0)
        if load_optimizer_states and "zf_m" in sd:
            for st, m, v in zip(self._zf, sd["zf_m"], sd["zf_v"]):
                st["m_cpu"].copy_(m)
                st["v_cpu"].copy_(v)
                st["hot_idx"] = None

    def destroy(self):
        self._drain_threads()
        super().destroy()
```

### deepspeed_amd/runtime/zero/stage3.py

```python
from collections import OrderedDict

import torch

from ... import comm as dist
from ...utils.logging import log_dist, logger
from ..loss_scaler import CreateLossScaler
from .stage3_params import (ZeroParamStatus, all_gather_params,
                            convert_to_zero_param, free_param, is_zero_param)

ALIGN = 64


def _pad_to(n, m):
    return (n + m - 1) // m * m


class SubGroup:

    __slots__ = ("params", "offsets", "master32", "grad32", "flat16",
                 "flat16_cpu", "grad_stage", "group_idx", "numel", "offload",
                 "param_offload", "dtype16")

    def __init__(self, params, offsets, numel, group_idx, device,
                 offload=False, param_offload=False, pin_opt=True,
                 pin_param=True):
        self.params = params
        self.offsets = offsets
        self.numel = numel
        self.group_idx = group_idx
        self.offload = offload
        self.param_offload = param_offload
        dtype16 = params[0].ds_tensor.dtype if params else torch.bfloat16
        self.dtype16 = dtype16
        pin = torch.cuda.is_available()
        host = torch.device("cpu")
        state_dev = host if offload else device
        slab_dev = host if param_offload else device
        self.flat16 = torch.empty(numel, dtype=dtype16, device=slab_dev,
                                  pin_memory=pin and param_offload
                                  and pin_param)
        self.master32 = torch.empty(numel, dtype=torch.float32,
                                    device=state_dev,
                                    pin_memory=pin and offload and pin_opt)
        for p in params:
            off = offsets[p]
            n = p.ds_shard_numel
            self.flat16[off:off + n].copy_(p.ds_tensor)
            p.ds_tensor = self.flat16[off:off + n]
            self.master32[off:off + n].copy_(p.ds_tensor.float())
        self.master32 = self.master32.detach().requires_grad_(True)
        self.grad32 = torch.zeros(numel, dtype=torch.float32,
                                  device=state_dev,
                                  pin_memory=pin and offload and pin_opt)
        if offload:
            if param_offload:
                self.flat16_cpu = self.flat16
            else:
                self.flat16_cpu = torch.empty(numel, dtype=dtype16,
                                              device=host,
                                              pin_memory=pin and pin_opt)
            self.grad_stage = torch.empty(numel, dtype=dtype16, device=host,
                                          pin_memory=pin and pin_opt)
        else:
            self.flat16_cpu = None
            self.grad_stage = None

    def grad_shard_view(self, p):
        off = self.offsets[p]
        return self.grad32[off:off + p.ds_shard_numel]

    def accumulate_grad(self, p, shard16_gpu):
        dst = self.grad_shard_view(p)[:shard16_gpu.numel()]
        if self.offload:
            off = self.offsets[p]
            stage = self.grad_stage[off:off + shard16_gpu.numel()]
            stage.copy_(shard16_gpu, non_blocking=True)
            if shard16_gpu.is_cuda:
                torch.cuda.synchronize()
            dst.add_(stage.float())
        elif shard16_gpu.is_cuda and shard16_gpu.dtype == torch.bfloat16:
            from ...ops.loader import get_ext
            get_ext(required=True).accum_bf16_to_f32(dst, shard16_gpu, 1.0)
        else:
            dst.add_(shard16_gpu.float())

    def copy_master_to_shards(self):
        if self.offload:
            self.flat16_cpu.copy_(self.master32.detach().to(self.dtype16)
                                  if self.flat16_cpu.dtype != torch.float32
                                  else self.master32.detach())
            if self.flat16_cpu is not self.flat16:
                self.flat16.copy_(self.flat16_cpu, non_blocking=True)
        else:
            self.flat16.copy_(self.master32.detach())

    def publish_flat16(self):
        if self.flat16_cpu is not self.flat16:
            self.flat16.copy_(self.flat16_cpu, non_blocking=True)


class ZeroStage3Optimizer:
    def __init__(self,
                 init_optimizer,
                 module,
                 engine=None,
                 dp_process_group=None,
                 reduce_bucket_size=int(5e8),
                 prefetch_bucket_size=int(5e7),
                 param_persistence_threshold=int(1e5),
                 model_persistence_threshold=int(1e14),
                 max_live_parameters=int(1e9),
                 max_reuse_distance=int(1e9),
                 sub_group_size=int(1e9),
                 overlap_comm=True,
                 offload_optimizer=None,
                 offload_param=None,
                 zero_quantized_weights=False,
                 zero_quantized_gradients=False,
                 zero_quantized_nontrainable_weights=False,
                 leaf_module_names=None,
                 clip_grad=0.0,
                 static_loss_scale=1.0,
                 dynamic_loss_scale=False,
                 dynamic_loss_args=None,
                 dtype=torch.bfloat16,
                 gradient_accumulation_steps=1,
                 replica_group=None):
        self.optimizer = init_optimizer
        self.module = module
        self.dp_group = dp_process_group
        self.replica_group = replica_group
        self.replica_world = (dist.get_world_size(replica_group)
                              if replica_group is not None else 1)
        self.world = dist.get_world_size(self.dp_group)
        self.rank = dist.get_rank(self.dp_group)
        self.dtype = dtype
        self.clip_grad = clip_grad
        self.reduce_bucket_size = int(reduce_bucket_size)
        self.prefetch_bucket_size = int(prefetch_bucket_size)
        self.persist_threshold = int(param_persistence_threshold)
        self.model_persistence_threshold = int(model_persistence_threshold)
        self.max_live_parameters = int(max_live_parameters)
        self.max_reuse_distance = int(max_reuse_distance)
        self.sub_group_size = int(sub_group_size)
        self.gradient_accumulation_steps = gradient_accumulation_steps
        self.micro_step = 0
        self.overlap_comm = overlap_comm
        self.quantized_weights = bool(zero_quantized_weights)
        self.quantized_gradients = bool(zero_quantized_gradients)
        self.quantized_nontrainable = bool(
            zero_quantized_nontrainable_weights)
        self.leaf_module_names = list(leaf_module_names or [])

        self.device = (torch.device("cuda", torch.cuda.current_device())
                       if torch.cuda.is_available() else torch.device("cpu"))
        self.offload_device = getattr(offload_optimizer, "device", "none") \
            if offload_optimizer is not None else "none"
        self.offload_optimizer = self.offload_device in ("cpu", "nvme")
        self.offload_ratio = float(getattr(offload_optimizer, "ratio",
                                           1.0)) \
            if offload_optimizer is not None else 1.0
        self.param_offload_device = getattr(offload_param, "device", "none") \
            if offload_param is not None else "none"
        self._pin_opt = getattr(offload_optimizer, "pin_memory", True) \
            if offload_optimizer is not None else True
        self._pin_param = getattr(offload_param, "pin_memory", True) \
            if offload_param is not None else True
        self.param_offload = self.param_offload_device in ("cpu", "nvme")
        self.param_swapper = None
        if self.param_offload_device == "nvme":
            from ..swap_tensor.param_swapper import ParamSlabSwapper
            import os as _os
            ppath = getattr(offload_param, "nvme_path", None) \
                or "/tmp/dsamd_nvme_swap"
            ppath = _os.path.join(ppath, f"param_rank{self.rank}")
            self.param_swapper = ParamSlabSwapper(
                ppath,
                max_in_cpu=getattr(offload_param, "max_in_cpu", int(1e9)),
                pin_memory=getattr(offload_param, "pin_memory", True))
        self.nvme_swapper = None
        if self.offload_device == "nvme":
            from ..swap_tensor.optimizer_swapper import OptimizerStateSwapper
            import os as _os
            nvme_path = getattr(offload_optimizer, "nvme_path", None) \
                or "/tmp/dsamd_nvme_swap"
            nvme_path = _os.path.join(nvme_path, f"rank{self.rank}")
            self.nvme_swapper = OptimizerStateSwapper(nvme_path)

        self.loss_scaler = CreateLossScaler(dtype, static_loss_scale,
                                            dynamic_loss_scale,
                                            dynamic_loss_args)
        self.overflow = False

        from ...comm import groups as grp
        self._expert_pg = {}
        for p in module.parameters():
            gn = getattr(p, "group_name", None)
            if gn is None:
                continue
            if gn not in self._expert_pg:
                if gn not in grp.get_expert_parallel_group_dict():
                    try:
                        grp.create_expert_and_data_parallel(
                            int(gn.rsplit("_", 1)[1]))
                    except (ValueError, AssertionError):
                        pass
                try:
                    self._expert_pg[gn] = \
                        grp.get_expert_data_parallel_group(gn)
                except KeyError:
                    self._expert_pg[gn] = None
        if self._expert_pg and self.replica_world > 1:
            raise NotImplementedError("MiCS + expert parallelism")
        self._shard_module_params()
        if self.quantized_nontrainable:
            from .stage3_params import quantize_frozen_param
            nq = 0
            for p in self._all_params:
                if not p.requires_grad and not p.ds_persist \
                        and p.ds_tensor is not None:
                    quantize_frozen_param(p)
                    nq += 1
            log_dist(f"ZeRO-3: {nq} frozen params int8-quantized",
                     ranks=[0])
        self._build_sub_groups()
        if self.param_swapper is not None:
            for i, sg in enumerate(self.sub_groups):
                self.param_swapper.register(i, sg)
                for p in sg.params:
                    p.ds_swap = (self.param_swapper, i)
            self._sg_index = {id(sg): i for i, sg in
                              enumerate(self.sub_groups)}
        if self.nvme_swapper is not None:
            self._init_nvme_state()
        self._gather_persistent_params()
        self._install_module_hooks()
        self._install_grad_hooks()

        import os as _os
        use_streams = torch.cuda.is_available() and self.overlap_comm \
            and (self.world > 1
                 or _os.environ.get("DSAMD_FORCE_STREAMS") == "1")
        self.ag_stream = torch.cuda.Stream() if use_streams else None
        self.rs_stream = torch.cuda.Stream() if use_streams else None
        self._rs_refs = []

        self._ipg_params = []
        self._ipg_numel = 0
        self._reduce_works = []

        self._trace = []
        self._trace_complete = False
        self._trace_pos = 0
        self._inflight = {}
        self._hooks_paused = False
        self._partition_stats = {"fetches": 0, "prefetch_hits": 0,
                                 "demand_gathers": 0, "gathered_numel": 0,
                                 "releases": 0}

        self._global_grad_norm = 0.0
        self._cached_norm_sq = None
        self._sanity = _os.environ.get("DSAMD_SANITY") == "1"
        log_dist(
            f"ZeRO-3: {sum(p.ds_numel for p in self._all_params)/1e9:.2f}B "
            f"params, {len(self.sub_groups)} sub-groups, world {self.world}",
            ranks=[0])

    def _shard_module_params(self):
        params = list(self.module.parameters())
        bcast_group = None if self.replica_world > 1 else self.dp_group
        bcast_world = dist.get_world_size(bcast_group) \
            if dist.is_initialized() else 1
        src = (dist.get_global_rank(bcast_group, 0)
               if bcast_group is not None and bcast_world > 1 else 0)
        shard_dev = torch.device("cpu") if self.param_offload else self.device
        for p in params:
            if not is_zero_param(p):
                p.data = p.data.to(self.device, self.dtype)
                gn = getattr(p, "group_name", None)
                pg = self._expert_pg.get(gn) if gn is not None else None
                if pg is not None:
                    if dist.get_world_size(pg) > 1:
                        dist.broadcast(p.data,
                                       dist.get_global_rank(pg, 0),
                                       group=pg)
                    convert_to_zero_param(p, pg, shard_dev, self.dtype,
                                          self.persist_threshold)
                    continue
                if bcast_world > 1:
                    dist.broadcast(p.data, src, group=bcast_group)
                convert_to_zero_param(p, self.dp_group, shard_dev,
                                      self.dtype, self.persist_threshold)
        for b in self.module.buffers():
            b.data = b.data.to(self.device)
        self._all_params = [p for p in self.module.parameters()]
        for i, p in enumerate(self._all_params):
            p.ds_param_index = i
        budget = self.model_persistence_threshold // max(self.world, 1)
        persisted = 0
        for p in self._all_params:
            if p.ds_persist:
                if persisted + p.ds_numel > budget:
                    p.ds_persist = False
                else:
                    persisted += p.ds_numel

    def _build_sub_groups(self):
        param_to_group = {}
        for gi, g in enumerate(self.optimizer.param_groups):
            for p in g["params"]:
                param_to_group[p] = gi
        self.sub_groups = []
        for gi in range(len(self.optimizer.param_groups)):
            gparams = [p for p in self._all_params
                       if param_to_group.get(p, 0) == gi and p.requires_grad]
            cur, offsets, numel = [], OrderedDict(), 0
            for p in gparams:
                if numel >= self.sub_group_size and cur:
                    self.sub_groups.append(
                        SubGroup(cur, offsets, numel, gi, self.device,
                                 offload=self._sg_offload(numel),
                                 param_offload=self.param_offload,
                                 pin_opt=self._pin_opt,
                                 pin_param=self._pin_param))
                    cur, offsets, numel = [], OrderedDict(), 0
                offsets[p] = numel
                cur.append(p)
                numel += p.ds_shard_numel
            if cur:
                self.sub_groups.append(
                    SubGroup(cur, offsets, numel, gi, self.device,
                             offload=self._sg_offload(numel),
                             param_offload=self.param_offload,
                             pin_opt=self._pin_opt,
                             pin_param=self._pin_param))
        self.param_to_subgroup = {}
        for sg in self.sub_groups:
            for p in sg.params:
                self.param_to_subgroup[p] = sg
        for gi, g in enumerate(self.optimizer.param_groups):
            g["params"] = [sg.master32 for sg in self.sub_groups
                           if sg.group_idx == gi]

    def _sg_offload(self, numel):
        if not self.offload_optimizer:
            return False
        if self.offload_ratio >= 1.0:
            return True
        if self.offload_ratio <= 0.0:
            return False
        if not hasattr(self, "_off_elems"):
            self._off_elems = 0
            self._tot_elems = 0
        behind = self._off_elems <= self.offload_ratio * self._tot_elems
        self._tot_elems += numel
        if behind:
            self._off_elems += numel
            return True
        return False

    def _init_nvme_state(self):
        for i, sg in enumerate(self.sub_groups):
            buf = self.nvme_swapper._buffer(i, "master", sg.numel)
            buf.copy_(sg.master32.detach().cpu())
            self.nvme_swapper._buffer(i, "exp_avg", sg.numel)
            self.nvme_swapper._buffer(i, "exp_avg_sq", sg.numel)
            self.nvme_swapper.swap_out(i)
            self.nvme_swapper.release_buffers(i)
            sg.master32 = None
        for g in self.optimizer.param_groups:
            g["params"] = []

    def _nvme_step(self, combined_scale):
        from ...ops.loader import get_ext
        ext = get_ext(required=False)
        for g in self.optimizer.param_groups:
            g["step"] = g.get("step", 0) + 1
        for i, sg in enumerate(self.sub_groups):
            if self.param_swapper is not None:
                self.param_swapper.ensure_resident(i)
            group = self.optimizer.param_groups[sg.group_idx]
            beta1, beta2 = group.get("betas", (0.9, 0.999))
            master, ea, eas = self.nvme_swapper.swap_in(i, sg.numel)
            grad = sg.grad32 if not sg.grad32.is_cuda else sg.grad32.cpu()
            if ext is not None:
                ext.cpu_adam_step(master, grad, ea, eas,
                                  sg.flat16_cpu, group["lr"], beta1, beta2,
                                  group.get("eps", 1e-8), group["step"], 1, 1,
                                  group.get("weight_decay", 0.0),
                                  1.0 / combined_scale)
            else:
                g32 = grad * (1.0 / combined_scale)
                step = group["step"]
                bc1 = 1 - beta1**step
                bc2 = 1 - beta2**step
                master.mul_(1.0 - group["lr"] *
                            group.get("weight_decay", 0.0))
                ea.mul_(beta1).add_(g32, alpha=1 - beta1)
                eas.mul_(beta2).addcmul_(g32, g32, value=1 - beta2)
                denom = (eas / bc2).sqrt().add_(group.get("eps", 1e-8))
                master.addcdiv_(ea, denom, value=-group["lr"] / bc1)
                sg.flat16_cpu.copy_(master.to(sg.flat16_cpu.dtype))
            self.nvme_swapper.swap_out(i)
            self.nvme_swapper.release_buffers(i)
            sg.publish_flat16()
            if self.param_swapper is not None:
                self.param_swapper.mark_dirty(i)
                self.param_swapper.evict_to_budget()

    def _flush_ipg_quant(self, params, world, pg):
        from .stage3_params import dequantize_gathered, quantize_shard
        for p in params:
            sn = p.ds_shard_numel
            if sn * world == p.ds_numel:
                padded = p.grad.reshape(-1)
            else:
                padded = torch.empty(sn * world, dtype=p.grad.dtype,
                                     device=p.grad.device)
                padded[:p.ds_numel].copy_(p.grad.reshape(-1))
                padded[p.ds_numel:].zero_()
            q, sc = quantize_shard(padded)
            qr = torch.empty_like(q)
            sr = torch.empty_like(sc)
            dist.all_to_all_single(qr, q, group=pg)
            dist.all_to_all_single(sr, sc, group=pg)
            deq = dequantize_gathered(qr, sr, world, torch.float32)
            shard = deq.view(world, sn).sum(0).div_(world)
            sg = self.param_to_subgroup[p]
            if self.replica_world > 1:
                from .stage_1_and_2 import _avg_op
                op = _avg_op(self.replica_world, shard)
                dist.all_reduce(shard, op=op, group=self.replica_group)
            sg.accumulate_grad(p, shard.to(p.grad.dtype))
            p.grad = None

    def _partial_offload_step(self, combined):
        if not hasattr(self, "_gpu_adam"):
            from ...ops.adam import FusedAdam
            g0 = self.optimizer.param_groups[0]
            dev_masters = [sg.master32 for sg in self.sub_groups
                           if not sg.offload]
            self._gpu_adam = FusedAdam(
                dev_masters, lr=g0["lr"],
                betas=g0.get("betas", (0.9, 0.999)),
                eps=g0.get("eps", 1e-8),
                weight_decay=g0.get("weight_decay", 0.0)) \
                if dev_masters else None
        if self._gpu_adam is not None:
            self._gpu_adam.param_groups[0]["lr"] = \
                self.optimizer.param_groups[0]["lr"]
        for which, opt in (("host", self.optimizer),
                           ("dev", self._gpu_adam)):
            if opt is None:
                continue
            fused = hasattr(opt, "set_grad_scale")
            sel = [sg for sg in self.sub_groups
                   if sg.offload == (which == "host")]
            if not sel:
                continue
            if fused:
                opt.set_grad_scale(1.0 / combined)
                opt.set_fused_out16(
                    {sg.master32: (sg.flat16_cpu if sg.offload
                                   else sg.flat16) for sg in sel})
            elif combined != 1.0:
                for sg in sel:
                    sg.grad32.mul_(1.0 / combined)
            for sg in sel:
                sg.master32.grad = sg.grad32
            opt.step()
            for sg in sel:
                sg.master32.grad = None
                if not fused:
                    sg.copy_master_to_shards()
                elif sg.offload:
                    sg.publish_flat16()
            if fused:
                opt.set_grad_scale(1.0)
                opt.set_fused_out16({})

    def _param_offload_step(self, combined, fused):
        bases = [g.get("step", 0) for g in self.optimizer.param_groups]
        if fused:
            self.optimizer.set_grad_scale(1.0 / combined)
        for i, sg in enumerate(self.sub_groups):
            self.param_swapper.ensure_resident(i)
            for g, b in zip(self.optimizer.param_groups, bases):
                g["step"] = b
            if fused:
                self.optimizer.set_fused_out16(
                    {sg.master32: (sg.flat16_cpu if sg.offload
                                   else sg.flat16)})
            elif combined != 1.0:
                sg.grad32.mul_(1.0 / combined)
            sg.master32.grad = sg.grad32
            self.optimizer.step()
            sg.master32.grad = None
            if not fused:
                sg.copy_master_to_shards()
            elif sg.offload:
                sg.publish_flat16()
            self.param_swapper.mark_dirty(i)
            self.param_swapper.evict_to_budget()
        if fused:
            self.optimizer.set_grad_scale(1.0)
            self.optimizer.set_fused_out16({})

    @torch.no_grad()
    def _muon_step(self, combined):
        from ...ops.muon import zeropower_via_newtonschulz5
        inv = 1.0 / combined
        if not hasattr(self, "_muon_state"):
            self._muon_state = {}
        for sg in self.sub_groups:
            group = self.optimizer.param_groups[sg.group_idx]
            group["step"] = group.get("step", 0) + 1
            mom = group["momentum"]
            for p in sg.params:
                sn = p.ds_shard_numel
                off = sg.offsets[p]
                gs = sg.grad32[off:off + sn]
                master = sg.master32[off:off + sn]
                st = self._muon_state.setdefault(p.ds_id, {})
                use_muon = len(p.ds_shape) == 2 and min(p.ds_shape) > 1
                if use_muon:
                    g = gs * inv
                    buf = st.setdefault("momentum_buffer",
                                        torch.zeros_like(gs))
                    buf.mul_(mom).add_(g)
                    eff = g.add(buf, alpha=mom) if group["nesterov"]                         else buf.clone()
                    pg = self._param_pg(p)
                    world = dist.get_world_size(pg)
                    eff_dev = eff.to(self.device)
                    if world > 1:
                        full = torch.empty(world * sn, dtype=eff_dev.dtype,
                                           device=eff_dev.device)
                        dist.all_gather_into_tensor(full, eff_dev, group=pg)
                    else:
                        full = eff_dev
                    mat = full[:p.ds_numel].view(p.ds_shape)
                    u = zeropower_via_newtonschulz5(
                        mat, group["ns_steps"]).reshape(-1)
                    rank = dist.get_rank(pg)
                    start = rank * sn
                    end = min(start + sn, p.ds_numel)
                    scale = max(1.0, p.ds_shape[0] / p.ds_shape[1]) ** 0.5
                    if group["weight_decay"]:
                        master.mul_(1 - group["lr"] *
                                    group["weight_decay"])
                    if end > start:
                        master[:end - start].add_(
                            u[start:end].to(master.device),
                            alpha=-group["lr"] * scale)
                else:
                    g = gs * inv
                    if "exp_avg" not in st:
                        st["exp_avg"] = torch.zeros_like(g)
                        st["exp_avg_sq"] = torch.zeros_like(g)
                    b1, b2 = group["adamw_betas"]
                    t = group["step"]
                    m, v = st["exp_avg"], st["exp_avg_sq"]
                    m.mul_(b1).add_(g, alpha=1 - b1)
                    v.mul_(b2).addcmul_(g, g, value=1 - b2)
                    denom = (v / (1 - b2 ** t)).sqrt_()                         .add_(group["adamw_eps"])
                    master.addcdiv_(m, denom,
                                    value=-group["adamw_lr"] /
                                    (1 - b1 ** t))
            if self.param_swapper is not None:
                i = self._sg_index[id(sg)]
                self.param_swapper.ensure_resident(i)
                sg.copy_master_to_shards()
                self.param_swapper.mark_dirty(i)
                self.param_swapper.evict_to_budget()
            else:
                sg.copy_master_to_shards()

    def _param_pg(self, p):
        return getattr(p, "ds_group", None) or self.dp_group

    def _gather_grouped(self, params, async_op=True, stream=None):
        if self.param_swapper is not None:
            need_ids = []
            for pm in params:
                sg = self.param_to_subgroup.get(pm)
                if sg is not None and self._sg_index[id(sg)] not in need_ids:
                    need_ids.append(self._sg_index[id(sg)])
            for i in need_ids:
                self.param_swapper.ensure_resident(i, exclude=need_ids)
        by_pg = {}
        for p in params:
            by_pg.setdefault(id(self._param_pg(p)), []).append(p)
        handles = [all_gather_params(ps, self._param_pg(ps[0]),
                                     async_op=async_op, stream=stream,
                                     quantized=self.quantized_weights)
                   for ps in by_pg.values()]
        if len(handles) == 1:
            return handles[0]

        class _Multi:
            def __init__(self, hs):
                self._hs = hs
                self.params = [p for h in hs for p in h.params]

            def wait(self):
                for h in self._hs:
                    h.wait()
        return _Multi(handles)

    def _gather_persistent_params(self):
        persist = [p for p in self._all_params if p.ds_persist]
        if persist:
            self._gather_grouped(persist, async_op=False).wait()

    def _leaf_module_classes(self):
        return set(getattr(self, "leaf_module_names", []) or [])

    def _install_module_hooks(self):
        self._module_hooks = []
        leaf_names = self._leaf_module_classes()
        leaf_descendants = set()
        for mod in self.module.modules():
            if type(mod).__name__ in leaf_names:
                for sub in mod.modules():
                    if sub is not mod:
                        leaf_descendants.add(id(sub))
        for mod in self.module.modules():
            if id(mod) in leaf_descendants:
                continue
            if type(mod).__name__ in leaf_names:
                direct = [p for p in mod.parameters(recurse=True)
                          if is_zero_param(p)]
            else:
                direct = [p for p in mod.parameters(recurse=False)
                          if is_zero_param(p)]
            external = [p for p in getattr(mod, "_ds_external_params", [])
                        if is_zero_param(p)]
            if not direct and not external:
                continue
            mod._ds_direct_params = direct + external
            self._module_hooks.append(mod.register_forward_pre_hook(
                self._pre_forward_hook))
            self._module_hooks.append(mod.register_forward_hook(
                self._post_forward_hook))
            self._module_hooks.append(mod.register_full_backward_pre_hook(
                self._pre_backward_hook))
            self._module_hooks.append(mod.register_full_backward_hook(
                self._post_backward_hook))
        self._module_hooks.append(self.module.register_forward_pre_hook(
            self._root_pre_forward))

    def _root_pre_forward(self, mod, inputs):
        self._trace_pos = 0
        if self._trace and not self._trace_complete:
            self._trace_complete = True
            self._compute_reuse_keep()

    def _compute_reuse_keep(self):
        sizes = [sum(p.ds_numel for p in m._ds_direct_params)
                 for m in self._trace]
        suffix = 0
        for i in range(len(self._trace) - 1, -1, -1):
            self._trace[i]._ds_keep_for_backward =                 2 * suffix < self.max_reuse_distance
            suffix += sizes[i]

    def _pre_forward_hook(self, mod, inputs):
        if self._hooks_paused:
            return
        self.fetch_sub_module(mod, forward=True)

    def _post_forward_hook(self, mod, inputs, output):
        if self._hooks_paused:
            return
        self.release_sub_module(mod)

    def _pre_backward_hook(self, mod, grad_output):
        self.fetch_sub_module(mod, forward=False)

    def _post_backward_hook(self, mod, grad_input, grad_output):
        for p in mod._ds_direct_params:
            p.ds_active_sub_modules.discard(id(mod))

    def fetch_sub_module(self, mod, forward=True):
        params = mod._ds_direct_params
        st = self._partition_stats
        st["fetches"] += 1
        for p in params:
            p.ds_active_sub_modules.add(id(mod))
        if forward and not self._trace_complete:
            self._trace.append(mod)
        h = self._inflight.pop(mod, None)
        if h is not None:
            st["prefetch_hits"] += 1
            h.wait()
        need = [p for p in params
                if p.ds_status == ZeroParamStatus.NOT_AVAILABLE]
        if need:
            st["demand_gathers"] += 1
            st["gathered_numel"] += sum(p.ds_numel for p in need)
            self._gather_grouped(need,
                              stream=self.ag_stream).wait()
        pending = [p for p in params
                   if p.ds_status == ZeroParamStatus.INFLIGHT]
        if pending:
            for key, handle in list(self._inflight.items()):
                if any(p in handle.params for p in pending):
                    handle.wait()
                    self._inflight.pop(key, None)
        for p in params:
            assert p.ds_status == ZeroParamStatus.AVAILABLE, \
                f"param {p.ds_id} not available after fetch"
        if self._trace_complete:
            self._prefetch(forward=forward, current_mod=mod)

    def _prefetch(self, forward=True, current_mod=None):
        budget = self.prefetch_bucket_size
        live = sum(p.ds_numel for p in self._all_params
                   if p.ds_status != ZeroParamStatus.NOT_AVAILABLE
                   and not p.ds_persist)
        budget = min(budget, max(0, self.max_live_parameters - live))
        n = len(self._trace)
        launched = 0
        if forward:
            pos = self._trace_pos
            step = 1
        else:
            if not hasattr(self, "_trace_index"):
                self._trace_index = {id(m): i
                                     for i, m in enumerate(self._trace)}
            pos = self._trace_index.get(id(current_mod), 0) - 1
            step = -1
        while 0 <= pos < n and budget > 0:
            mod = self._trace[pos]
            pos += step
            if mod in self._inflight:
                continue
            need = [p for p in mod._ds_direct_params
                    if p.ds_status == ZeroParamStatus.NOT_AVAILABLE]
            if not need:
                continue
            budget -= sum(p.ds_numel for p in need)
            self._inflight[mod] = self._gather_grouped(need,
                                                    stream=self.ag_stream)
            launched += 1
            if launched >= 8:
                break
        if forward:
            self._trace_pos = min(max(pos, 0), n)

    def release_sub_module(self, mod):
        keep = getattr(mod, "_ds_keep_for_backward", False)
        for p in mod._ds_direct_params:
            p.ds_active_sub_modules.discard(id(mod))
            if not keep and not p.ds_active_sub_modules \
                    and not p.ds_persist:
                self._partition_stats["releases"] += 1
                free_param(p)

    def partition_stats(self):
        return dict(self._partition_stats)

    def _install_grad_hooks(self):
        self._grad_hooks = []
        for p in self._all_params:
            if p.requires_grad:
                self._grad_hooks.append(
                    p.register_post_accumulate_grad_hook(self._on_grad_ready))

    def _on_grad_ready(self, p):
        self._ipg_params.append(p)
        self._ipg_numel += p.ds_numel
        if not p.ds_active_sub_modules and not p.ds_persist:
            free_param(p)
        if self._ipg_numel >= self.reduce_bucket_size:
            self._flush_ipg()

    def _flush_ipg(self):
        if not self._ipg_params:
            return
        params = self._ipg_params
        self._ipg_params = []
        self._ipg_numel = 0
        if self._sanity:
            from ..utils import assert_ints_same_as_other_ranks
            assert_ints_same_as_other_ranks(
                [p.ds_id for p in params], group=self.dp_group,
                tag="ipg_flush")
        by_pg = {}
        for p in params:
            by_pg.setdefault(id(self._param_pg(p)), []).append(p)
        if self.rs_stream is not None:
            self.rs_stream.wait_stream(torch.cuda.current_stream())
            for p in params:
                if p.grad is not None:
                    p.grad.record_stream(self.rs_stream)
            with torch.cuda.stream(self.rs_stream):
                for ps in by_pg.values():
                    pg = self._param_pg(ps[0])
                    self._flush_ipg_body(ps, dist.get_world_size(pg), pg)
            return
        for ps in by_pg.values():
            pg = self._param_pg(ps[0])
            self._flush_ipg_body(ps, dist.get_world_size(pg), pg)

    def _flush_ipg_body(self, params, world, pg=None):
        if pg is None:
            pg = self.dp_group
        use_coalescing = (torch.cuda.is_available() and world > 1
                          and len(params) > 1)
        shards = []
        if world == 1:
            for p in params:
                sg = self.param_to_subgroup[p]
                g = p.grad.reshape(-1)
                if self.replica_world > 1:
                    from .stage_1_and_2 import _avg_op
                    op = _avg_op(self.replica_world, g)
                    dist.all_reduce(g, op=op, group=self.replica_group)
                sg.accumulate_grad(p, g)
                p.grad = None
            return
        if self.quantized_gradients:
            self._flush_ipg_quant(params, world, pg)
            return
        from .stage_1_and_2 import _avg_op
        inputs = []
        for p in params:
            shard_numel = p.ds_shard_numel
            if shard_numel * world == p.ds_numel:
                padded = p.grad.reshape(-1)
            else:
                padded = torch.empty(shard_numel * world, dtype=p.grad.dtype,
                                     device=p.grad.device)
                padded[:p.ds_numel].copy_(p.grad.reshape(-1))
                padded[p.ds_numel:].zero_()
            inputs.append(padded)
            shards.append(torch.empty(shard_numel, dtype=p.grad.dtype,
                                      device=p.grad.device))
            p.grad = None
        if use_coalescing:
            try:
                from torch.distributed.distributed_c10d import \
                    _coalescing_manager
                from .stage_1_and_2 import _premul_avg_op
                op = _premul_avg_op(world) if inputs[0].is_cuda else None
                if op is None:
                    if world > 1:
                        for inp in inputs:
                            inp.div_(world)
                    op = dist.ReduceOp.SUM
                with _coalescing_manager(pg, self.device,
                                         async_ops=True) as cm:
                    for out, inp in zip(shards, inputs):
                        dist.reduce_scatter_tensor(out, inp, op=op,
                                                   group=pg)
                cm.wait()
            except Exception as e:
                from .stage3_params import _COALESCE_OK
                import deepspeed_amd.runtime.zero.stage3_params as s3p
                s3p._COALESCE_OK = False
                logger.warning(f"coalesced reduce-scatter failed ({e}); "
                               "falling back to per-param calls")
                use_coalescing = False
        if not use_coalescing:
            for out, inp in zip(shards, inputs):
                op = _avg_op(world, inp)
                dist.reduce_scatter_tensor(out, inp, op=op,
                                           group=pg)
        if self.replica_world > 1:
            from .stage_1_and_2 import _avg_op
            for shard in shards:
                op = _avg_op(self.replica_world, shard)
                dist.all_reduce(shard, op=op, group=self.replica_group)
        for p, shard in zip(params, shards):
            sg = self.param_to_subgroup[p]
            sg.accumulate_grad(p, shard)

    def backward(self, loss, retain_graph=False):
        self.micro_step += 1
        self.loss_scaler.backward(loss.float(), retain_graph=retain_graph)
        self._flush_ipg()

    def is_gradient_accumulation_boundary(self):
        return self.micro_step % self.gradient_accumulation_steps == 0

    def _grad_norm_sq(self):
        grads = [sg.grad32 for sg in self.sub_groups]
        if grads and grads[0].is_cuda:
            from ...ops.loader import get_ext
            total_sq = get_ext(required=True).l2norm_sq(grads).double()
        else:
            total_sq = torch.zeros(1, dtype=torch.float64)
            for g in grads:
                s = g.double()
                total_sq += torch.dot(s, s)
        total_sq = total_sq.reshape(1)
        if dist.is_initialized():
            total_sq = total_sq.to(self.device)
            dist.all_reduce(total_sq, group=self.dp_group)
        return total_sq

    def has_overflow(self):
        total_sq = self._cached_norm_sq if self._cached_norm_sq is not None \
            else self._grad_norm_sq()
        self._cached_norm_sq = total_sq
        return not bool(torch.isfinite(total_sq).item())

    def _combined_scale(self):
        scale = self.loss_scaler.loss_scale
        combined = scale
        if self.clip_grad > 0.0:
            total_sq = self._cached_norm_sq \
                if self._cached_norm_sq is not None else self._grad_norm_sq()
            norm = total_sq.sqrt().item() / scale
            self._global_grad_norm = norm
            clip = norm / self.clip_grad
            if clip > 1.0:
                combined = scale * clip
        return combined

    def _sync_comm_streams(self):
        if self.rs_stream is not None:
            torch.cuda.current_stream().wait_stream(self.rs_stream)
        if self.ag_stream is not None:
            torch.cuda.current_stream().wait_stream(self.ag_stream)
        self._rs_refs = []

    def _drain_inflight(self):
        for mod, h in list(self._inflight.items()):
            h.wait()
            for p in h.params:
                if not p.ds_persist:
                    free_param(p)
        self._inflight.clear()

    def step(self, closure=None):
        assert closure is None
        self._flush_ipg()
        self._sync_comm_streams()
        self._drain_inflight()
        self._cached_norm_sq = None

        if self.dtype == torch.float16:
            self.overflow = self.has_overflow()
            self.loss_scaler.update_scale(self.overflow)
            if self.overflow:
                log_dist("OVERFLOW: skipping step, new scale "
                         f"{self.loss_scaler.loss_scale}", ranks=[0])
                self._clear_grads()
                return

        combined = self._combined_scale()

        if self.nvme_swapper is not None:
            self._nvme_step(combined)
            self._clear_grads()
            self._refresh_persistent_params()
            return

        from ...ops.muon import Muon as _Muon
        if isinstance(self.optimizer, _Muon):
            self._muon_step(combined)
            self._clear_grads()
            self._refresh_persistent_params()
            return

        fused = hasattr(self.optimizer, "set_grad_scale")
        if getattr(self, "offload_ratio", 1.0) < 1.0 \
                and self.offload_optimizer:
            if self.param_swapper is not None:
                raise NotImplementedError(
                    "offload_optimizer.ratio < 1 with offload_param nvme "
                    "is unsupported: use ratio 1.0 (full offload) with "
                    "the NVMe parameter tier")
            self._partial_offload_step(combined)
            self._clear_grads()
            self._refresh_persistent_params()
            return
        if self.param_swapper is not None:
            self._param_offload_step(combined, fused)
            self._clear_grads()
            self._refresh_persistent_params()
            return
        if fused:
            self.optimizer.set_grad_scale(1.0 / combined)
            self.optimizer.set_fused_out16(
                {sg.master32: (sg.flat16_cpu if sg.offload else sg.flat16)
                 for sg in self.sub_groups})
        elif combined != 1.0:
            for sg in self.sub_groups:
                sg.grad32.mul_(1.0 / combined)

        for sg in self.sub_groups:
            sg.master32.grad = sg.grad32
        self.optimizer.step()
        for sg in self.sub_groups:
            sg.master32.grad = None
            if not fused:
                sg.copy_master_to_shards()
            elif sg.offload:
                sg.publish_flat16()
        if fused:
            self.optimizer.set_grad_scale(1.0)
            self.optimizer.set_fused_out16({})
        self._clear_grads()
        self._refresh_persistent_params()

    def _refresh_persistent_params(self):
        persist = [p for p in self._all_params if p.ds_persist]
        for p in persist:
            p.ds_status = ZeroParamStatus.NOT_AVAILABLE
        if persist:
            self._gather_grouped(persist, async_op=False).wait()

    def _clear_grads(self):
        for sg in self.sub_groups:
            sg.grad32.zero_()

    def zero_grad(self, set_to_none=True):
        pass

    @property
    def loss_scale(self):
        return self.loss_scaler.loss_scale

    def get_global_grad_norm(self):
        return self._global_grad_norm

    @property
    def param_groups(self):
        return self.optimizer.param_groups

    def shard_layout(self):
        names = {id(p): n for n, p in self.module.named_parameters()}
        subgroups = []
        for i, sg in enumerate(self.sub_groups):
            subgroups.append({
                "group_idx": sg.group_idx,
                "numel": sg.numel,
                "params": [(names.get(id(p), f"param_{p.ds_id}"),
                            sg.offsets[p], p.ds_shard_numel, p.ds_numel,
                            list(p.ds_shape),
                            dist.get_world_size(p.ds_group))
                           for p in sg.params],
            })
        return {"stage": 3, "world": self.world, "kind": "subgroup",
                "subgroups": subgroups}

    def state_dict(self):
        if self.nvme_swapper is not None:
            masters, eas, eass = [], [], []
            for i, sg in enumerate(self.sub_groups):
                m, ea, eas_ = self.nvme_swapper.swap_in(i, sg.numel)
                masters.append(m.clone())
                eas.append(ea.clone())
                eass.append(eas_.clone())
                self.nvme_swapper.release_buffers(i)
            return {
                "loss_scaler": self.loss_scaler,
                "base_optimizer_state": self.optimizer.state_dict(),
                "fp32_flat_groups": masters,
                "nvme_exp_avg": eas,
                "nvme_exp_avg_sq": eass,
                "param_shapes": self._param_shapes(),
                "zero_stage": 3,
                "partition_count": self.world,
                "shard_layout": self.shard_layout(),
            }
        sd = {
            "loss_scaler": self.loss_scaler,
            "base_optimizer_state": self.optimizer.state_dict(),
            "fp32_flat_groups": [sg.master32 for sg in self.sub_groups],
            "param_shapes": self._param_shapes(),
            "zero_stage": 3,
            "partition_count": self.world,
            "shard_layout": self.shard_layout(),
        }
        if getattr(self, "_muon_state", None):
            sd["muon_state"] = {
                k: {n: v for n, v in st.items()}
                for k, st in self._muon_state.items()}
        return sd

    def _param_shapes(self):
        shapes = OrderedDict()
        pmap = {id(p): n for n, p in self.module.named_parameters()}
        for sg in self.sub_groups:
            for p in sg.params:
                shapes[pmap.get(id(p), f"param_{p.ds_id}")] = {
                    "shape": p.ds_shape, "numel": p.ds_numel,
                    "shard_numel": p.ds_shard_numel,
                    "subgroup_offset": sg.offsets[p]}
        return shapes

    def load_state_dict(self, sd, load_optimizer_states=True):
        if "loss_scaler" in sd:
            self.loss_scaler = sd["loss_scaler"]
        if load_optimizer_states and "base_optimizer_state" in sd:
            self.optimizer.load_state_dict(sd["base_optimizer_state"])
        if load_optimizer_states and "muon_state" in sd:
            self._muon_state = {k: dict(st)
                                for k, st in sd["muon_state"].items()}
        saved = sd.get("fp32_flat_groups", [])
        assert len(saved) == len(self.sub_groups)
        if self.nvme_swapper is not None:
            eas = sd.get("nvme_exp_avg")
            eass = sd.get("nvme_exp_avg_sq")
            for i, (sg, m) in enumerate(zip(self.sub_groups, saved)):
                if self.param_swapper is not None:
                    self.param_swapper.ensure_resident(i)
                mb, eab, easb = self.nvme_swapper.swap_in(i, sg.numel)
                mb.copy_(m.cpu())
                if eas is not None:
                    eab.copy_(eas[i].cpu())
                    easb.copy_(eass[i].cpu())
                sg.flat16_cpu.copy_(mb.to(sg.flat16_cpu.dtype))
                self.nvme_swapper.swap_out(i)
                self.nvme_swapper.release_buffers(i)
                sg.publish_flat16()
                if self.param_swapper is not None:
                    self.param_swapper.mark_dirty(i)
                    self.param_swapper.evict_to_budget()
            self._refresh_persistent_params()
            return
        for i, (sg, s) in enumerate(zip(self.sub_groups, saved)):
            if self.param_swapper is not None:
                self.param_swapper.ensure_resident(i)
            sg.master32.data.copy_(s.data.to(sg.master32.device))
            sg.copy_master_to_shards()
            if self.param_swapper is not None:
                self.param_swapper.mark_dirty(i)
                self.param_swapper.evict_to_budget()
        self._refresh_persistent_params()

    @torch.no_grad()
    def offload_states(self, include=None, device="cpu",
                       pin_memory=False, non_blocking=False):
        inc = set(include or ("lp_params", "hp_params", "lp_grads",
                              "optim_states"))
        dev = torch.device(device)

        def _move(t):
            if t is None or t.device == dev:
                return t
            new = torch.empty_like(t, device=dev,
                                   pin_memory=pin_memory and
                                   dev.type == "cpu")
            new.copy_(t, non_blocking=non_blocking)
            return new

        for sg in self.sub_groups:
            if "lp_params" in inc and sg.flat16 is not None:
                sg.flat16 = _move(sg.flat16)
                for p in sg.params:
                    off = sg.offsets[p]
                    p.ds_tensor = sg.flat16[off:off + p.ds_shard_numel]
            if "hp_params" in inc:
                sg.master32.data = _move(sg.master32.data)
            if "lp_grads" in inc:
                sg.grad32 = _move(sg.grad32)
        if "optim_states" in inc:
            for st in self.optimizer.state.values():
                for k, v in list(st.items()):
                    if torch.is_tensor(v):
                        st[k] = _move(v)
        if torch.cuda.is_available():
            torch.cuda.empty_cache()

    def reload_states(self, non_blocking=False):
        self.offload_states(device=self.device,
                            non_blocking=non_blocking)

    def empty_partition_cache(self):
        self._drain_inflight()
        for p in self._all_params:
            if not p.ds_persist:
                free_param(p)
        if torch.cuda.is_available():
            torch.cuda.empty_cache()

    def destroy(self):
        for h in self._grad_hooks + self._module_hooks:
            h.remove()
        self._grad_hooks, self._module_hooks = [], []
```

### deepspeed_amd/utils/tensor_fragment.py

```python
import torch

from .. import comm as dist


def _find_owner(optimizer, param):
    if hasattr(optimizer, "param_to_bucket"):
        b = optimizer.param_to_bucket.get(param)
        if b is not None:
            return "bucket", b, b.offsets[param], None
    if hasattr(optimizer, "param_to_subgroup"):
        sg = optimizer.param_to_subgroup.get(param)
        if sg is not None:
            return "subgroup", sg, sg.offsets[param], param.ds_shard_numel
    return None, None, None, None


def _gather_flat(optimizer, kind, container, source32):
    pg = getattr(container, "pg", None) or optimizer.dp_group
    world = dist.get_world_size(pg)
    if world == 1:
        return source32.detach().float()
    out = torch.empty(source32.numel() * world, dtype=torch.float32,
                      device=source32.device)
    dist.all_gather_into_tensor(out, source32.detach().float().contiguous(),
                                group=pg)
    return out


def safe_get_full_fp32_param(param, optimizer=None):
    opt = optimizer
    if opt is None:
        return None
    kind, container, off, shard_numel = _find_owner(opt, param)
    if kind == "bucket":
        full = _gather_flat(opt, kind, container, container.master32)
        return full[off:off + param.numel()].reshape(param.shape)
    if kind == "subgroup":
        if container.master32 is None:
            return None
        pg = opt.dp_group
        world = dist.get_world_size(pg)
        shard = container.master32.detach().float()[off:off + shard_numel]
        if world == 1:
            return shard[:param.ds_numel].reshape(param.ds_shape)
        out = torch.empty(shard_numel * world, dtype=torch.float32,
                          device=shard.device)
        dist.all_gather_into_tensor(out, shard.contiguous(), group=pg)
        return out[:param.ds_numel].reshape(param.ds_shape)
    return None


def safe_set_full_fp32_param(param, value, optimizer=None):
    opt = optimizer
    if opt is None:
        return False
    kind, container, off, shard_numel = _find_owner(opt, param)
    flat = value.reshape(-1).float()
    if kind == "bucket":
        pg = getattr(container, "pg", None) or opt.dp_group
        rank = dist.get_rank(pg)
        lo = rank * container.shard_numel
        hi = lo + container.shard_numel
        s = max(lo, off)
        e = min(hi, off + param.numel())
        if e > s:
            container.master32.data[s - lo:e - lo].copy_(
                flat[s - off:e - off])
            container.shard16[s - lo:e - lo].copy_(
                flat[s - off:e - off].to(container.shard16.dtype))
        dist.all_gather_into_tensor(container.flat16, container.shard16,
                                    group=pg)
        return True
    if kind == "subgroup":
        pg = opt.dp_group
        rank = dist.get_rank(pg)
        lo = rank * shard_numel
        hi = min(lo + shard_numel, param.ds_numel)
        if hi > lo and container.master32 is not None:
            container.master32.data[off:off + hi - lo].copy_(flat[lo:hi])
            container.flat16[off:off + hi - lo].copy_(
                flat[lo:hi].to(container.flat16.dtype))
        return True
    return False


def safe_get_full_optimizer_state(param, optim_state_key, optimizer=None):
    opt = optimizer
    if opt is None:
        return None
    kind, container, off, shard_numel = _find_owner(opt, param)
    if container is None:
        return None
    base = opt.optimizer
    st = base.state.get(container.master32)
    if not st or optim_state_key not in st:
        return None
    state32 = st[optim_state_key]
    if kind == "bucket":
        full = _gather_flat(opt, kind, container, state32)
        return full[off:off + param.numel()].reshape(param.shape)
    pg = opt.dp_group
    world = dist.get_world_size(pg)
    shard = state32.detach().float()[off:off + shard_numel]
    if world == 1:
        return shard[:param.ds_numel].reshape(param.ds_shape)
    out = torch.empty(shard_numel * world, dtype=torch.float32,
                      device=shard.device)
    dist.all_gather_into_tensor(out, shard.contiguous(), group=pg)
    return out[:param.ds_numel].reshape(param.ds_shape)


def safe_get_full_grad(param, optimizer=None):
    opt = optimizer
    if opt is None:
        return None
    kind, container, off, shard_numel = _find_owner(opt, param)
    if kind == "bucket":
        if container.grad32 is None:
            return None
        full = _gather_flat(opt, kind, container, container.grad32)
        return full[off:off + param.numel()].reshape(param.shape)
    if kind == "subgroup":
        pg = opt.dp_group
        world = dist.get_world_size(pg)
        shard = container.grad32.detach().float()[off:off + shard_numel]
        if world == 1:
            return shard[:param.ds_numel].reshape(param.ds_shape)
        out = torch.empty(shard_numel * world, dtype=torch.float32,
                          device=shard.device)
        dist.all_gather_into_tensor(out, shard.contiguous(), group=pg)
        return out[:param.ds_numel].reshape(param.ds_shape)
    return None
```

Measured before the change: 16860 tokens/s.

## Fuse RoPE into flash attention, fuse RMSNorm backward, store-first grad accumulation

Adds a rope_flash_attention path that applies RoPE to q/k in one kernel and un-rotates dq/dk inside the flash backward kernels, removing the separate RoPE passes. RMSNorm backward becomes a fused dx+dw-partial kernel followed by a column-sum reduction. ZeRO-3 gradient accumulation now overwrites on the first write instead of zeroing grad32 every step, with lazy zeroing of stale entries. These are separate ideas that carry correctness risk around grad completion and rope table alignment.

```diff
diff --git a/deepspeed_amd/models/llama.py b/deepspeed_amd/models/llama.py
--- a/deepspeed_amd/models/llama.py
+++ b/deepspeed_amd/models/llama.py
@@ -4,7 +4,7 @@
 import torch.nn as nn
 import torch.nn.functional as F
 
-from ..ops.attention import flash_attention
+from ..ops.attention import flash_attention, rope_flash_attention
 from ..ops.functional import (apply_rope, build_rope_cache,
                               fused_cross_entropy, rms_norm, swiglu)
 
@@ -92,6 +92,10 @@
         if getattr(kv_cache, "fuses_rope", False):
             q, k, v = kv_cache.rope_append(q, k, v)
         else:
+            if kv_cache is None and self._dist_attn is None:
+                o = rope_flash_attention(q, k, v, cos, sin, causal=True)
+                if o is not None:
+                    return self.o_proj(o.reshape(B, S, -1))
             q = apply_rope(q, cos, sin)
             k = apply_rope(k, cos, sin)
             if kv_cache is not None:
diff --git a/deepspeed_amd/ops/attention.py b/deepspeed_amd/ops/attention.py
--- a/deepspeed_amd/ops/attention.py
+++ b/deepspeed_amd/ops/attention.py
@@ -24,62 +24,94 @@
         q, k, v, out, lse, kvmask = ctx.saved_tensors
         if kvmask.numel() == 0:
             kvmask = None
-        causal, scale = ctx.causal, ctx.scale
-        B, S, Hq, D = q.shape
-        Hk = k.shape[2]
-        G = Hq // Hk
+        dq, dk, dv = _flash_backward(q, k, v, out, lse, kvmask, ctx.causal,
+                                     ctx.scale, dout)
+        return dq, dk, dv, None, None, None
 
-        if os.environ.get("DSAMD_FLASH_BWD", "1") == "1":
-            ext = get_ext(required=True)
-            dq, dk, dv = ext.flash_attn_bwd(
-                q, k, v, dout.contiguous(), out, lse, causal, scale, kvmask)
-            return dq, dk, dv, None, None, None
 
-        qh = q.permute(0, 2, 1, 3)
-        kh = k.permute(0, 2, 1, 3)
-        vh = v.permute(0, 2, 1, 3)
-        doh = dout.permute(0, 2, 1, 3).contiguous()
-        oh = out.permute(0, 2, 1, 3)
+def _flash_backward(q, k, v, out, lse, kvmask, causal, scale, dout,
+                    cos=None, sin=None):
+    B, S, Hq, D = q.shape
+    Hk = k.shape[2]
+    G = Hq // Hk
 
-        drow = (doh.float() * oh.float()).sum(-1)
+    if os.environ.get("DSAMD_FLASH_BWD", "1") == "1":
+        ext = get_ext(required=True)
+        dq, dk, dv = ext.flash_attn_bwd(
+            q, k, v, dout.contiguous(), out, lse, causal, scale, kvmask,
+            cos, sin)
+        return dq, dk, dv
 
-        qg = qh.reshape(B, Hk, G, S, D)
-        dog = doh.reshape(B, Hk, G, S, D)
-        lse_g = lse.reshape(B, Hk, G, S)
-        drow_g = drow.reshape(B, Hk, G, S)
+    qh = q.permute(0, 2, 1, 3)
+    kh = k.permute(0, 2, 1, 3)
+    vh = v.permute(0, 2, 1, 3)
+    doh = dout.permute(0, 2, 1, 3).contiguous()
+    oh = out.permute(0, 2, 1, 3)
 
-        dq = torch.zeros(B, Hk, G, S, D, device=q.device, dtype=torch.float32)
-        dk = torch.empty_like(kh, dtype=torch.float32)
-        dv = torch.empty_like(vh, dtype=torch.float32)
+    drow = (doh.float() * oh.float()).sum(-1)
 
-        CHUNK = 1024
-        rows = torch.arange(S, device=q.device)
-        for c0 in range(0, S, CHUNK):
-            c1 = min(c0 + CHUNK, S)
-            kc = kh[:, :, c0:c1]
-            vc = vh[:, :, c0:c1]
-            s_c = torch.einsum("bhgsd,bhcd->bhgsc", qg, kc).float() * scale
-            if kvmask is not None:
-                s_c = s_c + kvmask[:, c0:c1].view(B, 1, 1, 1, c1 - c0)
-            p = torch.exp(s_c - lse_g.unsqueeze(-1))
-            if causal:
-                mask = rows.view(1, 1, 1, S, 1) >= (c0 + torch.arange(
-                    c1 - c0, device=q.device)).view(1, 1, 1, 1, -1)
-                p = p * mask
-            p16 = p.to(q.dtype)
-            dv[:, :, c0:c1] = torch.einsum("bhgsc,bhgsd->bhcd", p16,
-                                           dog).float()
-            dp = torch.einsum("bhgsd,bhcd->bhgsc", dog, vc).float()
-            ds = (p * (dp - drow_g.unsqueeze(-1)) * scale).to(q.dtype)
-            dq += torch.einsum("bhgsc,bhcd->bhgsd", ds, kc).float()
-            dk[:, :, c0:c1] = torch.einsum("bhgsc,bhgsd->bhcd", ds,
-                                           qg).float()
+    qg = qh.reshape(B, Hk, G, S, D)
+    dog = doh.reshape(B, Hk, G, S, D)
+    lse_g = lse.reshape(B, Hk, G, S)
+    drow_g = drow.reshape(B, Hk, G, S)
 
-        dq_out = dq.reshape(B, Hq, S, D).permute(0, 2, 1, 3).to(q.dtype)
-        dk_out = dk.permute(0, 2, 1, 3).to(k.dtype)
-        dv_out = dv.permute(0, 2, 1, 3).to(v.dtype)
-        return dq_out.contiguous(), dk_out.contiguous(), \
-            dv_out.contiguous(), None, None, None
+    dq = torch.zeros(B, Hk, G, S, D, device=q.device, dtype=torch.float32)
+    dk = torch.empty_like(kh, dtype=torch.float32)
+    dv = torch.empty_like(vh, dtype=torch.float32)
+
+    CHUNK = 1024
+    rows = torch.arange(S, device=q.device)
+    for c0 in range(0, S, CHUNK):
+        c1 = min(c0 + CHUNK, S)
+        kc = kh[:, :, c0:c1]
+        vc = vh[:, :, c0:c1]
+        s_c = torch.einsum("bhgsd,bhcd->bhgsc", qg, kc).float() * scale
+        if kvmask is not None:
+            s_c = s_c + kvmask[:, c0:c1].view(B, 1, 1, 1, c1 - c0)
+        p = torch.exp(s_c - lse_g.unsqueeze(-1))
+        if causal:
+            mask = rows.view(1, 1, 1, S, 1) >= (c0 + torch.arange(
+                c1 - c0, device=q.device)).view(1, 1, 1, 1, -1)
+            p = p * mask
+        p16 = p.to(q.dtype)
+        dv[:, :, c0:c1] = torch.einsum("bhgsc,bhgsd->bhcd", p16,
+                                       dog).float()
+        dp = torch.einsum("bhgsd,bhcd->bhgsc", dog, vc).float()
+        ds = (p * (dp - drow_g.unsqueeze(-1)) * scale).to(q.dtype)
+        dq += torch.einsum("bhgsc,bhcd->bhgsd", ds, kc).float()
+        dk[:, :, c0:c1] = torch.einsum("bhgsc,bhgsd->bhcd", ds,
+                                       qg).float()
+
+    dq_out = dq.reshape(B, Hq, S, D).permute(0, 2, 1, 3).to(q.dtype)
+    dk_out = dk.permute(0, 2, 1, 3).to(k.dtype)
+    dv_out = dv.permute(0, 2, 1, 3).to(v.dtype)
+    dq_out, dk_out = dq_out.contiguous(), dk_out.contiguous()
+    if cos is not None:
+        ext = get_ext(required=True)
+        ext.rope_inplace(dq_out, cos, sin, 0, True)
+        ext.rope_inplace(dk_out, cos, sin, 0, True)
+    return dq_out, dk_out, dv_out.contiguous()
+
+
+class _RopeFlashAttnFn(torch.autograd.Function):
+
+    @staticmethod
+    def forward(ctx, q, k, v, cos, sin, causal, scale):
+        ext = get_ext(required=True)
+        qr, kr = ext.rope_qk(q.contiguous(), k.contiguous(), cos, sin)
+        v = v.contiguous()
+        out, lse = ext.flash_attn_fwd(qr, kr, v, causal, scale, None)
+        ctx.save_for_backward(qr, kr, v, out, lse, cos, sin)
+        ctx.causal = causal
+        ctx.scale = scale
+        return out
+
+    @staticmethod
+    def backward(ctx, dout):
+        qr, kr, v, out, lse, cos, sin = ctx.saved_tensors
+        dq, dk, dv = _flash_backward(qr, kr, v, out, lse, None, ctx.causal,
+                                     ctx.scale, dout, cos, sin)
+        return dq, dk, dv, None, None, None, None
 
 
 _USE_HIP_FLASH = os.environ.get("DSAMD_FLASH", "1") == "1"
@@ -102,6 +134,22 @@
     if m.shape[0] != B:
         return None
     return m.contiguous().float()
+
+
+def rope_flash_attention(q, k, v, cos, sin, causal=True):
+    D = q.shape[-1]
+    if not (_USE_HIP_FLASH and q.is_cuda and q.dtype == torch.bfloat16
+            and D in (64, 128) and q.shape[1] == k.shape[1]
+            and cos.dim() == 2 and cos.is_cuda
+            and cos.shape[0] >= q.shape[1] and cos.shape[1] == D // 2
+            and os.environ.get("DSAMD_FLASH_BWD", "1") == "1"):
+        return None
+    cos = cos.float().contiguous()
+    sin = sin.float().contiguous()
+    if cos.data_ptr() % 16 or sin.data_ptr() % 16:
+        return None
+    return _RopeFlashAttnFn.apply(q, k, v, cos, sin, causal,
+                                  1.0 / math.sqrt(D))
 
 
 def flash_attention(q, k, v, causal=True, attn_mask=None):
diff --git a/deepspeed_amd/ops/csrc/attention_bwd.hip b/deepspeed_amd/ops/csrc/attention_bwd.hip
--- a/deepspeed_amd/ops/csrc/attention_bwd.hip
+++ b/deepspeed_amd/ops/csrc/attention_bwd.hip
@@ -148,7 +148,22 @@
   *reinterpret_cast<u32x2_t*>(p) = w;
 }
 
-template <int DH, int KTW>
+template <int NDT, int STRIDE>
+DEV_INLINE void unrotate_row(f32x4_t* acc ,
+                             const float* __restrict__ cr,
+                             const float* __restrict__ sr) {
+#pragma unroll
+  for (int dt = 0; dt < NDT / 2; ++dt) {
+    const f32x4_t c = *reinterpret_cast<const f32x4_t*>(cr + 16 * dt);
+    const f32x4_t sn = *reinterpret_cast<const f32x4_t*>(sr + 16 * dt);
+    const f32x4_t d1 = acc[dt * STRIDE];
+    const f32x4_t d2 = acc[(dt + NDT / 2) * STRIDE];
+    acc[dt * STRIDE] = d1 * c + d2 * sn;
+    acc[(dt + NDT / 2) * STRIDE] = d2 * c - d1 * sn;
+  }
+}
+
+template <int DH, int KTW, bool ROPE>
 __launch_bounds__(512 / KTW, 1)
 __global__ void flash_bwd_dkv_kernel(
     const short* __restrict__ q,
@@ -162,6 +177,8 @@
     const float* __restrict__ kvmask,
     short* __restrict__ dk,
     short* __restrict__ dv,
+    const float* __restrict__ rope_cos,
+    const float* __restrict__ rope_sin,
     int B, int S, int Sp, int Hq, int Hk, float scale, int causal) {
   constexpr int NKS = DH / 32;
   constexpr int NDT = DH / 16;
@@ -347,6 +364,10 @@
     if (gkv >= S) continue;
     short* dkr = dk + ((long long)b * S + gkv) * kvrs + hk * DH + 4 * l4;
     short* dvr = dv + ((long long)b * S + gkv) * kvrs + hk * DH + 4 * l4;
+    if (ROPE)
+      unrotate_row<NDT, KTW>(&dk_acc[0][kt],
+                             rope_cos + (long long)gkv * (DH / 2) + 4 * l4,
+                             rope_sin + (long long)gkv * (DH / 2) + 4 * l4);
 #pragma unroll
     for (int dt = 0; dt < NDT; ++dt) {
       store4(dkr + 16 * dt, dk_acc[dt][kt]);
@@ -355,7 +376,7 @@
   }
 }
 
-template <int DH>
+template <int DH, bool ROPE>
 __launch_bounds__(256, 2)
 __global__ void flash_bwd_dq_kernel(
     const short* __restrict__ q, const short* __restrict__ k,
@@ -365,6 +386,8 @@
     const float* __restrict__ drowP,
     const float* __restrict__ kvmask,
     short* __restrict__ dq,
+    const float* __restrict__ rope_cos,
+    const float* __restrict__ rope_sin,
     int B, int S, int Sp, int Hq, int Hk, float scale, int causal) {
   constexpr int NKS = DH / 32;
   constexpr int NDT = DH / 16;
@@ -522,6 +545,10 @@
     const int gq = wq + 16 * qt + l15;
     if (gq >= S) continue;
     short* dqr = dq + ((long long)b * S + gq) * qrs + h * DH + 4 * l4;
+    if (ROPE)
+      unrotate_row<NDT, 2>(&dq_acc[0][qt],
+                           rope_cos + (long long)gq * (DH / 2) + 4 * l4,
+                           rope_sin + (long long)gq * (DH / 2) + 4 * l4);
 #pragma unroll
     for (int dt = 0; dt < NDT; ++dt) store4(dqr + 16 * dt, dq_acc[dt][qt]);
   }
@@ -529,12 +556,13 @@
 
 }
 
-template <int DH>
+template <int DH, bool ROPE>
 static void launch_bwd(at::Tensor& q, at::Tensor& k, at::Tensor& v,
                        at::Tensor& dout, at::Tensor& out, at::Tensor& lse,
                        at::Tensor& dq, at::Tensor& dk, at::Tensor& dv,
-                       const float* mp, int B, int S, int Hq, int Hk,
-                       float scale, int causal) {
+                       const float* mp, const float* cosp, const float* sinp,
+                       int B, int S, int Hq, int Hk, float scale,
+                       int causal) {
   auto stream = c10::hip::getCurrentHIPStream();
   const int Sp = (S + bwd::BR - 1) / bwd::BR * bwd::BR;
   auto qT = at::empty({B, Hq, DH, Sp}, q.options());
@@ -556,17 +584,17 @@
                      Sp, Hq, Hk);
   HIP_CHECK_KERNEL();
   dim3 grid1(Sp / bwd::BR, B * Hk);
-  hipLaunchKernelGGL((bwd::flash_bwd_dkv_kernel<DH, bwd::KTW1>), grid1,
+  hipLaunchKernelGGL((bwd::flash_bwd_dkv_kernel<DH, bwd::KTW1, ROPE>), grid1,
                      dim3(512 / bwd::KTW1), 0, stream.stream(), sp(q), sp(k),
                      sp(v), sp(dout), sp(qT), sp(doT), lseP.data_ptr<float>(),
-                     drow.data_ptr<float>(), mp, spm(dk), spm(dv), B, S, Sp,
-                     Hq, Hk, scale, causal);
+                     drow.data_ptr<float>(), mp, spm(dk), spm(dv), cosp, sinp,
+                     B, S, Sp, Hq, Hk, scale, causal);
   HIP_CHECK_KERNEL();
   dim3 grid2(Sp / bwd::BR, B * Hq);
-  hipLaunchKernelGGL(bwd::flash_bwd_dq_kernel<DH>, grid2, dim3(256), 0,
+  hipLaunchKernelGGL((bwd::flash_bwd_dq_kernel<DH, ROPE>), grid2, dim3(256), 0,
                      stream.stream(), sp(q), sp(k), sp(v), sp(dout), sp(kT),
                      lseP.data_ptr<float>(), drow.data_ptr<float>(), mp,
-                     spm(dq), B, S, Sp, Hq, Hk, scale, causal);
+                     spm(dq), cosp, sinp, B, S, Sp, Hq, Hk, scale, causal);
   HIP_CHECK_KERNEL();
 }
 
@@ -574,12 +602,17 @@
                      const at::Tensor& v, const char* who);
 const float* flash_check_kvmask(const c10::optional<at::Tensor>& kvmask,
                                 const at::Tensor& q);
+void check_rope_table(const at::Tensor& cos, const at::Tensor& sin,
+                      const at::Tensor& ref, long long S, int D,
+                      const char* who);
 
 std::vector<at::Tensor> flash_attn_bwd(at::Tensor q, at::Tensor k,
                                        at::Tensor v, at::Tensor dout,
                                        at::Tensor out, at::Tensor lse,
                                        bool causal, double scale,
-                                       c10::optional<at::Tensor> kvmask) {
+                                       c10::optional<at::Tensor> kvmask,
+                                       c10::optional<at::Tensor> cos,
+                                       c10::optional<at::Tensor> sin) {
   flash_check_qkv(q, k, v, "flash_attn_bwd");
   CHECK_ARG(dout, at::kBFloat16);
   CHECK_ARG(out, at::kBFloat16);
@@ -600,11 +633,25 @@
   auto dq = at::empty_like(q);
   auto dk = at::empty_like(k);
   auto dv = at::empty_like(v);
-  if (D == 128)
-    launch_bwd<128>(q, k, v, dout, out, lse, dq, dk, dv, mp, B, S, Hq, Hk,
-                    fscale, causal ? 1 : 0);
-  else
-    launch_bwd<64>(q, k, v, dout, out, lse, dq, dk, dv, mp, B, S, Hq, Hk,
-                   fscale, causal ? 1 : 0);
+  TORCH_CHECK(cos.has_value() == sin.has_value(),
+              "flash_attn_bwd: cos and sin must be given together");
+  const bool rope = cos.has_value();
+  const float* cosp = nullptr;
+  const float* sinp = nullptr;
+  if (rope) {
+    check_rope_table(*cos, *sin, q, S, D, "flash_attn_bwd");
+    cosp = cos->data_ptr<float>();
+    sinp = sin->data_ptr<float>();
+  }
+  const int ic = causal ? 1 : 0;
+#define DSAMD_LAUNCH_BWD(DH_, ROPE_)                                        \
+  launch_bwd<DH_, ROPE_>(q, k, v, dout, out, lse, dq, dk, dv, mp, cosp, sinp, \
+                         B, S, Hq, Hk, fscale, ic)
+  if (D == 128) {
+    if (rope) DSAMD_LAUNCH_BWD(128, true); else DSAMD_LAUNCH_BWD(128, false);
+  } else {
+    if (rope) DSAMD_LAUNCH_BWD(64, true); else DSAMD_LAUNCH_BWD(64, false);
+  }
+#undef DSAMD_LAUNCH_BWD
   return {dq, dk, dv};
 }
diff --git a/deepspeed_amd/ops/csrc/bindings.cpp b/deepspeed_amd/ops/csrc/bindings.cpp
--- a/deepspeed_amd/ops/csrc/bindings.cpp
+++ b/deepspeed_amd/ops/csrc/bindings.cpp
@@ -8,7 +8,8 @@
                        long adamw_mode, long bias_correction,
                        double weight_decay, std::vector<at::Tensor> out16,
                        double grad_scale);
-void accum_bf16_to_f32(at::Tensor dst, at::Tensor src, double scale);
+void accum_bf16_to_f32(at::Tensor dst, at::Tensor src, double scale,
+                       bool overwrite);
 at::Tensor l2norm_sq(std::vector<at::Tensor> tensors);
 at::Tensor fp8_amax(at::Tensor x);
 at::Tensor ragged_decode(at::Tensor q, at::Tensor kpool, at::Tensor vpool,
@@ -44,7 +45,9 @@
                                        at::Tensor v, at::Tensor dout,
                                        at::Tensor out, at::Tensor lse,
                                        bool causal, double scale,
-                                       c10::optional<at::Tensor> kvmask);
+                                       c10::optional<at::Tensor> kvmask,
+                                       c10::optional<at::Tensor> cos,
+                                       c10::optional<at::Tensor> sin);
 void multi_tensor_adagrad(std::vector<at::Tensor> params,
                           std::vector<at::Tensor> grads,
                           std::vector<at::Tensor> sq_accums, double lr,
@@ -86,6 +89,8 @@
           long pos0, bool backward);
 void rope_inplace(at::Tensor t, at::Tensor cos, at::Tensor sin, long pos0,
                   bool backward);
+std::vector<at::Tensor> rope_qk(at::Tensor q, at::Tensor k, at::Tensor cos,
+                                at::Tensor sin);
 at::Tensor swiglu_fwd(at::Tensor g, at::Tensor u);
 std::vector<at::Tensor> swiglu_bwd(at::Tensor dy, at::Tensor g, at::Tensor u);
 std::vector<at::Tensor> cross_entropy_fwd(at::Tensor logits,
@@ -120,7 +125,8 @@
         py::arg("weight_decay"), py::arg("out16") = std::vector<at::Tensor>(),
         py::arg("grad_scale") = 1.0);
   m.def("accum_bf16_to_f32", &accum_bf16_to_f32, py::arg("dst"),
-        py::arg("src"), py::arg("scale") = 1.0);
+        py::arg("src"), py::arg("scale") = 1.0,
+        py::arg("overwrite") = false);
   m.def("l2norm_sq", &l2norm_sq);
   m.def("fp8_amax", &fp8_amax);
   m.def("ragged_decode", &ragged_decode, py::arg("q"), py::arg("kpool"),
@@ -172,7 +178,8 @@
   m.def("flash_attn_bwd", &flash_attn_bwd, py::arg("q"), py::arg("k"),
         py::arg("v"), py::arg("dout"), py::arg("out"), py::arg("lse"),
         py::arg("causal") = true, py::arg("scale") = 0.0,
-        py::arg("kvmask") = c10::nullopt);
+        py::arg("kvmask") = c10::nullopt, py::arg("cos") = c10::nullopt,
+        py::arg("sin") = c10::nullopt);
   m.def("multi_tensor_adagrad", &multi_tensor_adagrad, py::arg("params"),
         py::arg("grads"), py::arg("sq_accums"), py::arg("lr"),
         py::arg("eps") = 1e-8, py::arg("weight_decay") = 0.0,
@@ -209,6 +216,7 @@
   m.def("layernorm_bwd", &layernorm_bwd);
   m.def("rope", &rope);
   m.def("rope_inplace", &rope_inplace);
+  m.def("rope_qk", &rope_qk);
   m.def("swiglu_fwd", &swiglu_fwd);
   m.def("swiglu_bwd", &swiglu_bwd);
   m.def("cross_entropy_fwd", &cross_entropy_fwd);
diff --git a/deepspeed_amd/ops/csrc/elementwise.hip b/deepspeed_amd/ops/csrc/elementwise.hip
--- a/deepspeed_amd/ops/csrc/elementwise.hip
+++ b/deepspeed_amd/ops/csrc/elementwise.hip
@@ -1,6 +1,30 @@
 #include <torch/extension.h>
 
 #include "common.h"
+
+DEV_INLINE void rope_vec8(short* __restrict__ dst,
+                          const short* __restrict__ src, long long base,
+                          int half, const float* __restrict__ crow,
+                          const float* __restrict__ srow, float sgn) {
+  bf16x8 x1 = *reinterpret_cast<const bf16x8*>(src + base);
+  bf16x8 x2 = *reinterpret_cast<const bf16x8*>(src + base + half);
+  f32x4 c0 = *reinterpret_cast<const f32x4*>(crow);
+  f32x4 c1 = *reinterpret_cast<const f32x4*>(crow + 4);
+  f32x4 s0 = *reinterpret_cast<const f32x4*>(srow);
+  f32x4 s1 = *reinterpret_cast<const f32x4*>(srow + 4);
+  bf16x8 o1, o2;
+#pragma unroll
+  for (int k = 0; k < 8; ++k) {
+    float c = (k < 4 ? c0.v[k] : c1.v[k - 4]);
+    float sv = (k < 4 ? s0.v[k] : s1.v[k - 4]) * sgn;
+    float a = bf2f(x1.v[k]);
+    float bb = bf2f(x2.v[k]);
+    o1.v[k] = f2bf(a * c - bb * sv);
+    o2.v[k] = f2bf(bb * c + a * sv);
+  }
+  *reinterpret_cast<bf16x8*>(dst + base) = o1;
+  *reinterpret_cast<bf16x8*>(dst + base + half) = o2;
+}
 
 __global__ void rope_kernel(short* __restrict__ dst,
                             const short* __restrict__ src,
@@ -20,27 +44,39 @@
     int s = (int)(rem2 % S);
     long long b = rem2 / S;
     long long base = ((b * S + s) * (long long)H + h) * D + d8 * 8;
-    const float* crow = cs + (long long)(s + pos0) * half + d8 * 8;
-    const float* srow = sn + (long long)(s + pos0) * half + d8 * 8;
-    bf16x8 x1 = *reinterpret_cast<const bf16x8*>(src + base);
-    bf16x8 x2 = *reinterpret_cast<const bf16x8*>(src + base + half);
-    f32x4 c0 = *reinterpret_cast<const f32x4*>(crow);
-    f32x4 c1 = *reinterpret_cast<const f32x4*>(crow + 4);
-    f32x4 s0 = *reinterpret_cast<const f32x4*>(srow);
-    f32x4 s1 = *reinterpret_cast<const f32x4*>(srow + 4);
-    float sgn = backward ? -1.f : 1.f;
-    bf16x8 o1, o2;
-#pragma unroll
-    for (int k = 0; k < 8; ++k) {
-      float c = (k < 4 ? c0.v[k] : c1.v[k - 4]);
-      float sv = (k < 4 ? s0.v[k] : s1.v[k - 4]) * sgn;
-      float a = bf2f(x1.v[k]);
-      float bb = bf2f(x2.v[k]);
-      o1.v[k] = f2bf(a * c - bb * sv);
-      o2.v[k] = f2bf(bb * c + a * sv);
-    }
-    *reinterpret_cast<bf16x8*>(dst + base) = o1;
-    *reinterpret_cast<bf16x8*>(dst + base + half) = o2;
+    rope_vec8(dst, src, base, half,
+              cs + (long long)(s + pos0) * half + d8 * 8,
+              sn + (long long)(s + pos0) * half + d8 * 8,
+              backward ? -1.f : 1.f);
+  }
+}
+
+__global__ void rope_qk_kernel(short* __restrict__ qd,
+                               const short* __restrict__ qs,
+                               short* __restrict__ kd,
+                               const short* __restrict__ ks,
+                               const float* __restrict__ cs,
+                               const float* __restrict__ sn,
+                               long long total_vec, int S, int Hq, int Hk,
+                               int D) {
+  int half = D / 2;
+  int half8 = half / 8;
+  int HT = Hq + Hk;
+  long long i0 = (long long)blockIdx.x * blockDim.x + threadIdx.x;
+  long long stride = (long long)gridDim.x * blockDim.x;
+  for (long long i = i0; i < total_vec; i += stride) {
+    int d8 = (int)(i % half8);
+    long long rem = i / half8;
+    int h = (int)(rem % HT);
+    long long tok = rem / HT;
+    int s = (int)(tok % S);
+    const float* crow = cs + (long long)s * half + d8 * 8;
+    const float* srow = sn + (long long)s * half + d8 * 8;
+    if (h < Hq)
+      rope_vec8(qd, qs, (tok * Hq + h) * D + d8 * 8, half, crow, srow, 1.f);
+    else
+      rope_vec8(kd, ks, (tok * Hk + (h - Hq)) * D + d8 * 8, half, crow, srow,
+                1.f);
   }
 }
 
@@ -118,6 +154,56 @@
   HIP_CHECK_KERNEL();
 }
 
+void check_rope_table(const at::Tensor& cos, const at::Tensor& sin,
+                      const at::Tensor& ref, long long S, int D,
+                      const char* who) {
+  TORCH_CHECK(cos.defined() && sin.defined() &&
+                  cos.device() == ref.device() && sin.device() == ref.device(),
+              who, ": cos/sin must be on the same device as q");
+  TORCH_CHECK(cos.scalar_type() == at::kFloat && cos.is_contiguous() &&
+                  sin.scalar_type() == at::kFloat && sin.is_contiguous(),
+              who, ": cos/sin must be contiguous fp32");
+  TORCH_CHECK(S * (D / 2) <= cos.numel() && S * (D / 2) <= sin.numel(),
+              who, ": cos/sin table shorter than [S, D/2]");
+  TORCH_CHECK(ptr_aligned(cos.data_ptr(), 16) &&
+                  ptr_aligned(sin.data_ptr(), 16),
+              who, ": cos/sin must be 16-byte aligned");
+}
+
+std::vector<at::Tensor> rope_qk(at::Tensor q, at::Tensor k, at::Tensor cos,
+                                at::Tensor sin) {
+  CHECK_ARG(q, at::kBFloat16);
+  CHECK_ARG(k, at::kBFloat16);
+  CHECK_ON(k, q);
+  TORCH_CHECK(q.dim() == 4 && k.dim() == 4 && q.size(0) == k.size(0) &&
+                  q.size(1) == k.size(1) && q.size(3) == k.size(3),
+              "rope_qk expects q [B,S,Hq,D] and k [B,S,Hk,D]");
+  int B = q.size(0), S = q.size(1), Hq = q.size(2), D = q.size(3);
+  int Hk = k.size(2);
+  TORCH_CHECK(D % 16 == 0, "rope_qk: D must be a multiple of 16");
+  auto qo = at::empty_like(q);
+  auto ko = at::empty_like(k);
+  if (q.numel() + k.numel() == 0) return {qo, ko};
+  check_rope_table(cos, sin, q, S, D, "rope_qk");
+  TORCH_CHECK(ptr_aligned(q.data_ptr(), 16) && ptr_aligned(k.data_ptr(), 16) &&
+                  ptr_aligned(qo.data_ptr(), 16) &&
+                  ptr_aligned(ko.data_ptr(), 16),
+              "rope_qk: q/k must be 16-byte aligned");
+  auto stream = c10::hip::getCurrentHIPStream();
+  int block = 256;
+  long long total_vec = (long long)B * S * (Hq + Hk) * (D / 16);
+  int grid = grid_for(total_vec, block);
+  hipLaunchKernelGGL(rope_qk_kernel, dim3(grid), dim3(block), 0,
+                     stream.stream(), reinterpret_cast<short*>(qo.data_ptr()),
+                     reinterpret_cast<const short*>(q.data_ptr()),
+                     reinterpret_cast<short*>(ko.data_ptr()),
+                     reinterpret_cast<const short*>(k.data_ptr()),
+                     cos.data_ptr<float>(), sin.data_ptr<float>(), total_vec,
+                     S, Hq, Hk, D);
+  HIP_CHECK_KERNEL();
+  return {qo, ko};
+}
+
 void rope_inplace(at::Tensor t, at::Tensor cos, at::Tensor sin, long pos0,
                   bool backward) {
   rope(t, t, cos, sin, pos0, backward);
diff --git a/deepspeed_amd/ops/csrc/misc.hip b/deepspeed_amd/ops/csrc/misc.hip
--- a/deepspeed_amd/ops/csrc/misc.hip
+++ b/deepspeed_amd/ops/csrc/misc.hip
@@ -2,6 +2,7 @@
 
 #include "common.h"
 
+template <bool OVERWRITE>
 __global__ void accum_bf16_f32_kernel(float* __restrict__ dst,
                                       const short* __restrict__ src,
                                       long long n, float scale,
@@ -12,16 +13,27 @@
   for (long long i = i0; i < n4; i += stride) {
     uint2 sv = reinterpret_cast<const uint2*>(src)[i];
     const short* s = reinterpret_cast<const short*>(&sv);
-    f32x4 d = reinterpret_cast<f32x4*>(dst)[i];
+    f32x4 d;
+    if (OVERWRITE) {
 #pragma unroll
-    for (int k = 0; k < 4; ++k) d.v[k] += bf2f(s[k]) * scale;
+      for (int k = 0; k < 4; ++k) d.v[k] = bf2f(s[k]) * scale;
+    } else {
+      d = reinterpret_cast<f32x4*>(dst)[i];
+#pragma unroll
+      for (int k = 0; k < 4; ++k) d.v[k] += bf2f(s[k]) * scale;
+    }
     reinterpret_cast<f32x4*>(dst)[i] = d;
   }
-  for (long long i = n4 * 4 + i0; i < n; i += stride)
-    dst[i] += bf2f(src[i]) * scale;
+  for (long long i = n4 * 4 + i0; i < n; i += stride) {
+    if (OVERWRITE)
+      dst[i] = bf2f(src[i]) * scale;
+    else
+      dst[i] += bf2f(src[i]) * scale;
+  }
 }
 
-void accum_bf16_to_f32(at::Tensor dst, at::Tensor src, double scale) {
+void accum_bf16_to_f32(at::Tensor dst, at::Tensor src, double scale,
+                       bool overwrite) {
   CHECK_ARG(dst, at::kFloat);
   CHECK_ARG(src, at::kBFloat16);
   CHECK_LIKE(src, dst);
@@ -31,8 +43,10 @@
   auto stream = c10::hip::getCurrentHIPStream();
   int block = 256;
   int grid = grid_for(n / 4 + 1, block);
-  hipLaunchKernelGGL(accum_bf16_f32_kernel, dim3(grid), dim3(block), 0,
-                     stream.stream(), dst.data_ptr<float>(),
+  auto kern = overwrite ? accum_bf16_f32_kernel<true>
+                        : accum_bf16_f32_kernel<false>;
+  hipLaunchKernelGGL(kern, dim3(grid), dim3(block), 0, stream.stream(),
+                     dst.data_ptr<float>(),
                      reinterpret_cast<const short*>(src.data_ptr()), n,
                      (float)scale, vec_ok);
   HIP_CHECK_KERNEL();
diff --git a/deepspeed_amd/ops/csrc/norms.hip b/deepspeed_amd/ops/csrc/norms.hip
--- a/deepspeed_amd/ops/csrc/norms.hip
+++ b/deepspeed_amd/ops/csrc/norms.hip
@@ -99,11 +99,96 @@
     dxr[i] = f2bf(rs * (bf2f(dyr[i]) * bf2f(w[i]) - bf2f(xr[i]) * c));
 }
 
-__global__ void rmsnorm_bwd_dw_kernel(const short* __restrict__ dy,
-                                      const short* __restrict__ x,
-                                      const float* __restrict__ rstd,
-                                      float* __restrict__ dw, long long rows,
-                                      int H) {
+constexpr int kRmsBwdMaxV = 4;
+
+template <int BLOCK, int NV>
+__launch_bounds__(BLOCK)
+__global__ void rmsnorm_bwd_fused_kernel(const short* __restrict__ dy,
+                                         const short* __restrict__ x,
+                                         const short* __restrict__ w,
+                                         const float* __restrict__ rstd,
+                                         short* __restrict__ dx,
+                                         float* __restrict__ part,
+                                         long long rows, long long per,
+                                         int H) {
+  __shared__ float lds[BLOCK / WAVE];
+  const int H8 = H / 8;
+  const long long r0 = blockIdx.x * per;
+  const long long r1 = r0 + per < rows ? r0 + per : rows;
+  bf16x8 wv[NV], dv[NV], xv[NV];
+  float acc[NV][8];
+#pragma unroll
+  for (int j = 0; j < NV; ++j) {
+    const int i = threadIdx.x + j * BLOCK;
+#pragma unroll
+    for (int k = 0; k < 8; ++k) acc[j][k] = 0.f;
+    if (i < H8) {
+      wv[j] = reinterpret_cast<const bf16x8*>(w)[i];
+      if (r0 < r1) {
+        dv[j] = reinterpret_cast<const bf16x8*>(dy + r0 * H)[i];
+        xv[j] = reinterpret_cast<const bf16x8*>(x + r0 * H)[i];
+      }
+    }
+  }
+  for (long long r = r0; r < r1; ++r) {
+    const float rs = rstd[r];
+    bf16x8 ndv[NV], nxv[NV];
+    const bool more = r + 1 < r1;
+    float dot = 0.f;
+#pragma unroll
+    for (int j = 0; j < NV; ++j) {
+      const int i = threadIdx.x + j * BLOCK;
+      if (i < H8) {
+        if (more) {
+          ndv[j] = reinterpret_cast<const bf16x8*>(dy + (r + 1) * H)[i];
+          nxv[j] = reinterpret_cast<const bf16x8*>(x + (r + 1) * H)[i];
+        }
+#pragma unroll
+        for (int k = 0; k < 8; ++k)
+          dot += bf2f(dv[j].v[k]) * bf2f(wv[j].v[k]) * bf2f(xv[j].v[k]);
+      }
+    }
+    dot = block_reduce_sum<BLOCK>(dot, lds);
+    const float c = dot * rs * rs / H;
+    short* dxr = dx + r * H;
+#pragma unroll
+    for (int j = 0; j < NV; ++j) {
+      const int i = threadIdx.x + j * BLOCK;
+      if (i < H8) {
+        bf16x8 o;
+#pragma unroll
+        for (int k = 0; k < 8; ++k) {
+          const float d = bf2f(dv[j].v[k]);
+          const float xf = bf2f(xv[j].v[k]);
+          o.v[k] = f2bf(rs * (d * bf2f(wv[j].v[k]) - xf * c));
+          acc[j][k] += d * xf * rs;
+        }
+        reinterpret_cast<bf16x8*>(dxr)[i] = o;
+        if (more) {
+          dv[j] = ndv[j];
+          xv[j] = nxv[j];
+        }
+      }
+    }
+  }
+  float* pr = part + (long long)blockIdx.x * H;
+#pragma unroll
+  for (int j = 0; j < NV; ++j) {
+    const int i = threadIdx.x + j * BLOCK;
+    if (i < H8) {
+      f32x4 lo = {{acc[j][0], acc[j][1], acc[j][2], acc[j][3]}};
+      f32x4 hi = {{acc[j][4], acc[j][5], acc[j][6], acc[j][7]}};
+      reinterpret_cast<f32x4*>(pr)[2 * i] = lo;
+      reinterpret_cast<f32x4*>(pr)[2 * i + 1] = hi;
+    }
+  }
+}
+
+__global__ void rmsnorm_bwd_dw_partial_kernel(const short* __restrict__ dy,
+                                              const short* __restrict__ x,
+                                              const float* __restrict__ rstd,
+                                              float* __restrict__ part,
+                                              long long rows, int H) {
   int c = blockIdx.x * blockDim.x + threadIdx.x;
   if (c >= H) return;
   float acc = 0.f;
@@ -111,10 +196,48 @@
     long long idx = r * H + c;
     acc += bf2f(dy[idx]) * bf2f(x[idx]) * rstd[r];
   }
-  if (gridDim.y == 1)
-    dw[c] = acc;
-  else
-    atomicAdd(dw + c, acc);
+  part[(long long)blockIdx.y * H + c] = acc;
+}
+
+template <int BLOCK>
+__launch_bounds__(BLOCK)
+__global__ void colsum_partials_kernel(const float* __restrict__ part,
+                                       int nparts, int H,
+                                       float* __restrict__ dw) {
+  constexpr int COLS = 32;
+  constexpr int NG = BLOCK / COLS;
+  __shared__ float lds[BLOCK];
+  const int cx = threadIdx.x % COLS;
+  const int g = threadIdx.x / COLS;
+  const int c = blockIdx.x * COLS + cx;
+  float acc = 0.f;
+  if (c < H) {
+#pragma unroll 8
+    for (int p = g; p < nparts; p += NG) acc += part[(long long)p * H + c];
+  }
+  lds[threadIdx.x] = acc;
+  __syncthreads();
+  if (g == 0 && c < H) {
+    float s = 0.f;
+#pragma unroll
+    for (int k = 0; k < NG; ++k) s += lds[k * COLS + cx];
+    dw[c] = s;
+  }
+}
+
+static int rms_bwd_max_blocks() {
+  static int cached[64] = {0};
+  int dev = 0;
+  TORCH_CHECK(hipGetDevice(&dev) == hipSuccess, "hipGetDevice failed");
+  if (dev < 0 || dev >= 64) return 1024;
+  if (cached[dev] == 0) {
+    int cus = 0;
+    if (hipDeviceGetAttribute(&cus, hipDeviceAttributeMultiprocessorCount,
+                              dev) != hipSuccess || cus <= 0)
+      cus = 256;
+    cached[dev] = 4 * cus;
+  }
+  return cached[dev];
 }
 
 std::vector<at::Tensor> rmsnorm_fwd(at::Tensor x, at::Tensor w, double eps) {
@@ -148,26 +271,49 @@
   long long rows = x.numel() / H;
   TORCH_CHECK(rstd.numel() == rows, "rstd must have one entry per row");
   auto dx = at::empty_like(x);
-  auto dw = at::zeros({H}, x.options().dtype(at::kFloat));
-  if (rows == 0) return {dx, dw};
+  auto fopt = x.options().dtype(at::kFloat);
+  if (rows == 0) return {dx, at::zeros({H}, fopt)};
+  auto dw = at::empty({H}, fopt);
   auto stream = c10::hip::getCurrentHIPStream();
   constexpr int BLOCK = 256;
   int vec = row_vec_ok(
       H, {dy.data_ptr(), x.data_ptr(), w.data_ptr(), dx.data_ptr()});
-  hipLaunchKernelGGL(rmsnorm_bwd_dx_kernel<BLOCK>, dim3(rows), dim3(BLOCK), 0,
-                     stream.stream(),
-                     reinterpret_cast<const short*>(dy.data_ptr()),
-                     reinterpret_cast<const short*>(x.data_ptr()),
-                     reinterpret_cast<const short*>(w.data_ptr()),
-                     rstd.data_ptr<float>(),
-                     reinterpret_cast<short*>(dx.data_ptr()), H, vec);
-  HIP_CHECK_KERNEL();
-  int gy = rows > 4096 ? 64 : (rows > 512 ? 16 : 1);
-  hipLaunchKernelGGL(rmsnorm_bwd_dw_kernel, dim3((H + 255) / 256, gy),
-                     dim3(256), 0, stream.stream(),
-                     reinterpret_cast<const short*>(dy.data_ptr()),
-                     reinterpret_cast<const short*>(x.data_ptr()),
-                     rstd.data_ptr<float>(), dw.data_ptr<float>(), rows, H);
+  const short* dyp = reinterpret_cast<const short*>(dy.data_ptr());
+  const short* xp = reinterpret_cast<const short*>(x.data_ptr());
+  const short* wp = reinterpret_cast<const short*>(w.data_ptr());
+  short* dxp = reinterpret_cast<short*>(dx.data_ptr());
+  const int nv = (H / 8 + BLOCK - 1) / BLOCK;
+  at::Tensor part;
+  int nparts;
+  if (vec && nv <= kRmsBwdMaxV) {
+    const long long maxb = rms_bwd_max_blocks();
+    const long long per = (rows + maxb - 1) / maxb;
+    nparts = (int)((rows + per - 1) / per);
+    part = at::empty({nparts, H}, fopt);
+    auto kern = nv == 1   ? rmsnorm_bwd_fused_kernel<BLOCK, 1>
+                : nv == 2 ? rmsnorm_bwd_fused_kernel<BLOCK, 2>
+                          : rmsnorm_bwd_fused_kernel<BLOCK, 4>;
+    hipLaunchKernelGGL(kern, dim3(nparts), dim3(BLOCK), 0, stream.stream(),
+                       dyp, xp, wp, rstd.data_ptr<float>(), dxp,
+                       part.data_ptr<float>(), rows, per, H);
+    HIP_CHECK_KERNEL();
+  } else {
+    hipLaunchKernelGGL(rmsnorm_bwd_dx_kernel<BLOCK>, dim3(rows), dim3(BLOCK),
+                       0, stream.stream(), dyp, xp, wp,
+                       rstd.data_ptr<float>(), dxp, H, vec);
+    HIP_CHECK_KERNEL();
+    nparts = rows > 4096 ? 64 : (rows > 512 ? 16 : 1);
+    part = at::empty({nparts, H}, fopt);
+    hipLaunchKernelGGL(rmsnorm_bwd_dw_partial_kernel,
+                       dim3((H + 255) / 256, nparts), dim3(256), 0,
+                       stream.stream(), dyp, xp, rstd.data_ptr<float>(),
+                       part.data_ptr<float>(), rows, H);
+    HIP_CHECK_KERNEL();
+  }
+  constexpr int RB = 1024;
+  hipLaunchKernelGGL(colsum_partials_kernel<RB>, dim3((H + 31) / 32),
+                     dim3(RB), 0, stream.stream(), part.data_ptr<float>(),
+                     nparts, H, dw.data_ptr<float>());
   HIP_CHECK_KERNEL();
   return {dx, dw};
 }
diff --git a/deepspeed_amd/runtime/zenflow.py b/deepspeed_amd/runtime/zenflow.py
--- a/deepspeed_amd/runtime/zenflow.py
+++ b/deepspeed_amd/runtime/zenflow.py
@@ -247,6 +247,7 @@
         self._flush_ipg()
         self._sync_comm_streams()
         self._drain_inflight()
+        self._complete_grads()
         self._cached_norm_sq = None
         if self.dtype == torch.float16:
             self.overflow = self.has_overflow()
diff --git a/deepspeed_amd/runtime/zero/stage3.py b/deepspeed_amd/runtime/zero/stage3.py
--- a/deepspeed_amd/runtime/zero/stage3.py
+++ b/deepspeed_amd/runtime/zero/stage3.py
@@ -19,7 +19,8 @@
 
     __slots__ = ("params", "offsets", "master32", "grad32", "flat16",
                  "flat16_cpu", "grad_stage", "group_idx", "numel", "offload",
-                 "param_offload", "dtype16")
+                 "param_offload", "dtype16", "store_first", "_written",
+                 "_stale")
 
     def __init__(self, params, offsets, numel, group_idx, device,
                  offload=False, param_offload=False, pin_opt=True,
@@ -64,6 +65,9 @@
         else:
             self.flat16_cpu = None
             self.grad_stage = None
+        self.store_first = not offload
+        self._written = set()
+        self._stale = set()
 
     def grad_shard_view(self, p):
         off = self.offsets[p]
@@ -78,11 +82,31 @@
             if shard16_gpu.is_cuda:
                 torch.cuda.synchronize()
             dst.add_(stage.float())
-        elif shard16_gpu.is_cuda and shard16_gpu.dtype == torch.bfloat16:
+            return
+        overwrite = self.store_first and p not in self._written
+        self._written.add(p)
+        if shard16_gpu.is_cuda and shard16_gpu.dtype == torch.bfloat16:
             from ...ops.loader import get_ext
-            get_ext(required=True).accum_bf16_to_f32(dst, shard16_gpu, 1.0)
+            get_ext(required=True).accum_bf16_to_f32(dst, shard16_gpu, 1.0,
+                                                     overwrite)
+        elif overwrite:
+            dst.copy_(shard16_gpu)
         else:
             dst.add_(shard16_gpu.float())
+
+    def complete_grads(self):
+        for p in self._stale:
+            if p not in self._written:
+                self.grad_shard_view(p).zero_()
+        self._stale.clear()
+
+    def clear_grads(self):
+        if self.store_first:
+            self._stale |= self._written
+        else:
+            self.grad32.zero_()
+            self._stale.clear()
+        self._written.clear()
 
     def copy_master_to_shards(self):
         if self.offload:
@@ -884,6 +908,7 @@
         return self.micro_step % self.gradient_accumulation_steps == 0
 
     def _grad_norm_sq(self):
+        self._complete_grads()
         grads = [sg.grad32 for sg in self.sub_groups]
         if grads and grads[0].is_cuda:
             from ...ops.loader import get_ext
@@ -938,6 +963,7 @@
         self._flush_ipg()
         self._sync_comm_streams()
         self._drain_inflight()
+        self._complete_grads()
         self._cached_norm_sq = None
 
         if self.dtype == torch.float16:
@@ -1014,7 +1040,16 @@
 
     def _clear_grads(self):
         for sg in self.sub_groups:
-            sg.grad32.zero_()
+            sg.clear_grads()
+
+    def _set_store_first(self, enabled):
+        self._complete_grads()
+        for sg in self.sub_groups:
+            sg.store_first = bool(enabled) and not sg.offload
+
+    def _complete_grads(self):
+        for sg in self.sub_groups:
+            sg.complete_grads()
 
     def zero_grad(self, set_to_none=True):
         pass
diff --git a/deepspeed_amd/utils/tensor_fragment.py b/deepspeed_amd/utils/tensor_fragment.py
--- a/deepspeed_amd/utils/tensor_fragment.py
+++ b/deepspeed_amd/utils/tensor_fragment.py
@@ -123,6 +123,7 @@
     if kind == "subgroup":
         pg = opt.dp_group
         world = dist.get_world_size(pg)
+        container.complete_grads()
         shard = container.grad32.detach().float()[off:off + shard_numel]
         if world == 1:
             return shard[:param.ds_numel].reshape(param.ds_shape)
```

Result: faster. 17120 tokens/s (median of 6 runs) (+1.5%).
